# rookiepig/CrossScalePatchMatch

Hardware: AMD Instinct MI355X
Metric: Mpix/s disparity (GRD, use_cs=true) (higher is better)
Workload: dtype f64; 1 GPU; C3: 1242x375 max_dis=128 GRD scale_num=5 reg_lambda=0.3 wnd=35 iters=3 (BASELINE.json configs[2] when C3); cc_name=GRD, schedule=raster, sweep_cells=as cost_source, raster_sweep=persistent, rb_rounds=1, sweep_workgroups_per_cu=2, sweep_workgroup_waves=levels - 1 (coarsest level folded, CSPM_OPT_SWEEP_FOLD), early_exit=True, pairs_per_gpu=22, distinct_pairs_per_gpu=22, pairs_in_flight_per_gpu=2, use_pp=False, parallelism=1 rank(s), one per GPU, 2 independent pair stream(s) each, dispatch=every rank generates its own pairs (no collective in the timed region)

## Files before the change

crossscalepatchmatch_amd/capi.py:

```python
import ctypes as C
import os
import subprocess

import numpy as np

_HERE = os.path.dirname(os.path.abspath(__file__))
_SO = os.environ.get("CSPM_LIB") or os.path.join(_HERE, "libcspm_hip.so")

SCHED_RASTER, SCHED_REDBLACK = 0, 1
RNG_PER_PIXEL, RNG_ROW_SHARED = 0, 1
K_GRD, K_INIT, K_SPATIAL, K_VIEW, K_REFINE, K_MISC, K_POST = range(7)
K_NAMES = ["grd", "init", "spatial", "view", "refine", "misc", "post"]
MAX_LEVELS = 8
OPT_GRD_VOLUMES = 1
OPT_RASTER_LAUNCHES = 2
OPT_SWEEP_TIMEOUT_MS = 3
OPT_SWEEP_FALLBACKS = 4
OPT_SWEEP_PAIRS = 5
OPT_SWEEP_PAIRS_ACTIVE = 6
OPT_TABLE_VOLUMES = 7
OPT_TABLE_VOLUMES_ACTIVE = 8
OPT_SWEEP_PACKED = 10
OPT_SWEEP_PACKED_ACTIVE = 11
OPT_SWEEP_PACKED_BAD = 12
OPT_SWEEP_FLOW = 13
OPT_SWEEP_WG = 14
OPT_VOLUME_FALLBACKS = 9
OPT_VOLUME_RETRY_PAIRS = 15
OPT_VIEW_SORT = 17
OPT_SWEEP_FOLD = 18
OPT_FAULT_VOLUME_ALLOC = 16
CA_BOX, CA_GF, CA_BF = 0, 1, 2

SYMBOLS = [
    "cspm_device_count", "cspm_create", "cspm_destroy", "cspm_last_error", "cspm_set_stream", "cspm_get_stream", "cspm_synchronize",
    "cspm_set_images", "cspm_set_images_device", "cspm_build_cost_grd", "cspm_build_cost_cen", "cspm_build_cost_img", "cspm_cen_build_cv_host", "cspm_set_option", "cspm_get_option", "cspm_begin_cost", "cspm_upload_cost_slab",
    "cspm_finish_cost", "cspm_get_levels", "cspm_get_level_dims", "cspm_get_level_image", "cspm_get_cost_slab",
    "cspm_get_max_cost", "cspm_get_scale_weights", "cspm_grd_build_cv_host", "cspm_plane_cost_batch",
    "cspm_pm_default_params", "cspm_patchmatch", "cspm_pm_init", "cspm_pm_spatial", "cspm_pm_view", "cspm_pm_refine",
    "cspm_get_planes", "cspm_set_planes", "cspm_get_disparity_u8", "cspm_get_disparity_f64",
    "cspm_disparity_u8_device", "cspm_postprocess", "cspm_postprocess_device", "cspm_enable_timing", "cspm_reset_timing", "cspm_get_timing",
    "cspm_taps_per_view_pass", "cspm_row_engine_taps_per_view_pass", "cspm_fpm_begin", "cspm_fpm_candidates", "cspm_fpm_commit",
    "cspm_aggregate_cv_host", "cspm_local_stereo", "cspm_rescore_planes", "cspm_patchmatch_warm", "cspm_upsample_planes",
]


class CspmError(RuntimeError):
    pass


class PmParams(C.Structure):
    _fields_ = [("seed", C.c_uint64), ("schedule", C.c_int), ("rb_rounds", C.c_int), ("rb_neighbours", C.c_int),
                ("rng_mode", C.c_int), ("early_exit", C.c_int)]


def library_path():
    return _SO


def build_library(force=False):
    src_dir = os.path.join(_HERE, "csrc")
    srcs = [os.path.join(src_dir, f) for f in os.listdir(src_dir)] + [os.path.join(_HERE, "..", "include", "cspm.h")]
    if force or not os.path.exists(_SO) or os.path.getmtime(_SO) < max(os.path.getmtime(s) for s in srcs):
        subprocess.check_call(["make", "-C", src_dir, "-B"], stdout=subprocess.DEVNULL)
    return _SO


_lib = None


def load_library():
    global _lib
    if _lib is not None:
        return _lib
    if not os.path.exists(_SO):
        raise CspmError(f"{_SO} is missing: build it with `python -c 'import __graft_entry__ as g; g.build()'` "
                        "(hipcc --offload-arch=gfx950). There is no CPU fallback.")
    L = C.CDLL(_SO)
    vp, dp, ip, u8p = C.c_void_p, C.POINTER(C.c_double), C.POINTER(C.c_int), C.POINTER(C.c_uint8)
    llp = C.POINTER(C.c_longlong)
    pp = C.POINTER(PmParams)
    sig = {
        "cspm_device_count": (C.c_int, []),
        "cspm_create": (C.c_int, [C.POINTER(vp), C.c_int]),
        "cspm_destroy": (None, [vp]),
        "cspm_last_error": (C.c_char_p, [vp]),
        "cspm_set_stream": (C.c_int, [vp, vp]),
        "cspm_get_stream": (C.c_int, [vp, C.POINTER(vp)]),
        "cspm_synchronize": (C.c_int, [vp]),
        "cspm_set_images": (C.c_int, [vp, u8p, u8p, C.c_int, C.c_int, C.c_size_t]),
        "cspm_set_images_device": (C.c_int, [vp, vp, vp, C.c_int, C.c_int, C.c_size_t]),
        "cspm_build_cost_grd": (C.c_int, [vp, C.c_int, C.c_int, C.c_int, C.c_double]),
        "cspm_set_option": (C.c_int, [vp, C.c_int, C.c_longlong]),
        "cspm_get_option": (C.c_int, [vp, C.c_int, llp]),
        "cspm_build_cost_cen": (C.c_int, [vp, C.c_int, C.c_int, C.c_int, C.c_double]),
        "cspm_build_cost_img": (C.c_int, [vp, C.c_int, C.c_int, C.c_int, C.c_double]),
        "cspm_cen_build_cv_host": (C.c_int, [C.c_int, dp, dp, C.c_int, C.c_int, C.c_int, C.c_int, dp]),
        "cspm_begin_cost": (C.c_int, [vp, C.c_int, C.c_int, C.c_int, C.c_double]),
        "cspm_upload_cost_slab": (C.c_int, [vp, C.c_int, C.c_int, C.c_int, dp, C.c_size_t]),
        "cspm_finish_cost": (C.c_int, [vp]),
        "cspm_get_levels": (C.c_int, [vp]),
        "cspm_get_level_dims": (C.c_int, [vp, C.c_int, ip, ip, ip]),
        "cspm_get_level_image": (C.c_int, [vp, C.c_int, C.c_int, u8p]),
        "cspm_get_cost_slab": (C.c_int, [vp, C.c_int, C.c_int, C.c_int, dp]),
        "cspm_get_max_cost": (C.c_int, [vp, C.c_int, C.c_int, dp]),
        "cspm_get_scale_weights": (C.c_int, [vp, dp]),
        "cspm_grd_build_cv_host": (C.c_int, [C.c_int, dp, dp, C.c_int, C.c_int, C.c_int, C.c_int, dp]),
        "cspm_plane_cost_batch": (C.c_int, [vp, C.c_int, C.c_int, ip, dp, dp]),
        "cspm_pm_default_params": (C.c_int, [pp]),
        "cspm_patchmatch": (C.c_int, [vp, C.c_int, pp]),
        "cspm_pm_init": (C.c_int, [vp, pp]),
        "cspm_pm_spatial": (C.c_int, [vp, C.c_int, pp]),
        "cspm_pm_view": (C.c_int, [vp, C.c_int, pp]),
        "cspm_pm_refine": (C.c_int, [vp, C.c_int, pp]),
        "cspm_get_planes": (C.c_int, [vp, C.c_int, dp, dp]),
        "cspm_set_planes": (C.c_int, [vp, C.c_int, dp, dp]),
        "cspm_get_disparity_u8": (C.c_int, [vp, C.c_int, C.c_int, u8p, C.c_size_t]),
        "cspm_get_disparity_f64": (C.c_int, [vp, C.c_int, dp]),
        "cspm_disparity_u8_device": (C.c_int, [vp, C.c_int, C.c_int, vp]),
        "cspm_postprocess": (C.c_int, [vp, C.c_int, u8p, u8p, C.c_size_t]),
        "cspm_postprocess_device": (C.c_int, [vp, C.c_int, vp, vp]),
        "cspm_enable_timing": (C.c_int, [vp, C.c_int]),
        "cspm_reset_timing": (C.c_int, [vp]),
        "cspm_get_timing": (C.c_int, [vp, C.c_int, llp, dp, llp]),
        "cspm_fpm_begin": (C.c_int, [vp, C.c_int, C.c_int, C.c_int]),
        "cspm_fpm_candidates": (C.c_int, [vp, C.c_int, C.c_int, C.c_int, pp, ip, ip, ip, dp]),
        "cspm_fpm_commit": (C.c_int, [vp, dp]),
        "cspm_taps_per_view_pass": (C.c_longlong, [vp]),
        "cspm_row_engine_taps_per_view_pass": (C.c_longlong, [vp]),
        "cspm_aggregate_cv_host": (C.c_int, [C.c_int, C.c_int, dp, C.c_int, C.c_int, C.c_int, dp]),
        "cspm_local_stereo": (C.c_int, [vp, C.c_int]),
        "cspm_rescore_planes": (C.c_int, [vp]),
        "cspm_patchmatch_warm": (C.c_int, [vp, C.c_int, pp]),
        "cspm_upsample_planes": (C.c_int, [vp, vp]),
    }
    assert sorted(sig) == sorted(SYMBOLS)
    for name, (res, args) in sig.items():
        f = getattr(L, name)
        f.restype, f.argtypes = res, args
    _lib = L
    return L


def _dp(a):
    return a.ctypes.data_as(C.POINTER(C.c_double))


def _u8(a):
    return a.ctypes.data_as(C.POINTER(C.c_uint8))


class StereoContext:

    def __init__(self, device=0):
        self.L = load_library()
        self.p = C.c_void_p()
        rc = self.L.cspm_create(C.byref(self.p), device)
        if rc != 0:
            raise CspmError(f"cspm_create failed ({rc}): {self.L.cspm_last_error(None).decode()}")
        self.w = self.h = 0

    def close(self):
        if getattr(self, "p", None) and self.p:
            self.L.cspm_destroy(self.p)
            self.p = C.c_void_p()

    def __del__(self):
        try:
            self.close()
        except Exception:
            pass

    def _chk(self, rc):
        if rc != 0:
            raise CspmError(f"cspm error {rc}: {self.L.cspm_last_error(self.p).decode()}")

    def set_images(self, l_bgr, r_bgr):
        l = np.ascontiguousarray(l_bgr, dtype=np.uint8)
        r = np.ascontiguousarray(r_bgr, dtype=np.uint8)
        assert l.ndim == 3 and l.shape[2] == 3 and l.shape == r.shape
        self.h, self.w = l.shape[:2]
        self._chk(self.L.cspm_set_images(self.p, _u8(l), _u8(r), self.w, self.h, self.w * 3))

    def set_images_device(self, d_l_ptr, d_r_ptr, w, h, stride=None):
# ... 226 lines not shown
```

crossscalepatchmatch_amd/csrc/cspm_api.hip:

```cpp
#include <hip/hip_runtime.h>

#include <cfloat>
#include <cmath>
#include <cstdio>
#include <cstring>
#include <string>
#include <vector>

#include "cspm_kernels.h"
#include "cspm_ca.h"

using namespace cspm;

namespace {

thread_local std::string g_create_error;

struct TimingRec {
  int kclass;
  hipEvent_t a, b;
  long long evals;
};

}

struct DevGuard {
  int prev = -1;
  bool ok = true;
  explicit DevGuard(int dev) {
    if (hipGetDevice(&prev) != hipSuccess) prev = -1;
    if (prev != dev) ok = hipSetDevice(dev) == hipSuccess;
    else prev = -1;
  }
  ~DevGuard() {
    if (prev >= 0) (void)hipSetDevice(prev);
  }
};

struct CostKey {
  int W = 0, H = 0, max_dis = 0, wnd = 0, scale_num = -1, with_vol = 0, kind = -1, with_pairs = 0, with_cvol = 0, with_px8 = 0;
  bool operator==(const CostKey &o) const {
    return W == o.W && H == o.H && max_dis == o.max_dis && wnd == o.wnd && scale_num == o.scale_num && with_vol == o.with_vol && kind == o.kind &&
           with_pairs == o.with_pairs && with_cvol == o.with_cvol && with_px8 == o.with_px8;
  }
};
enum { kKindForeign = 0, kKindGrd = 1, kKindCen = 2, kKindImg = 3 };

struct cspm_ctx {
  int device = 0, ncu = 256;
  int sweep_wg_per_cu = 0;
  int sweep_bands = 1;
  int sweep_bands_built = 0;
  int refine_chunk = 64;
  hipStream_t own_stream = nullptr, stream = nullptr;
  std::string err;
  int W = 0, H = 0;
  uint32_t *img0[2] = {nullptr, nullptr};
  uint8_t *stage = nullptr;
  size_t stage_bytes = 0;
  bool cost_alloc = false, cost_ready = false;
  Cost cost{};
  int max_dis = 0, wnd = 0;
  double scale_wgt[CSPM_MAX_LEVELS] = {0};
  double host_max_cost[2 * CSPM_MAX_LEVELS] = {0};
  std::vector<void *> cost_allocs;
  CostKey cost_key;
  bool max_cost_fetched = false;
  int *d_early_ok = nullptr;
  uint8_t *cen_gray[2][CSPM_MAX_LEVELS] = {{nullptr}};
  double *d_lut = nullptr, *d_lut_a = nullptr, *d_maxcost = nullptr;
  bool is_grd = false;
  bool is_cen = false;
  bool is_img = false;
  const uint32_t *cen_code[2][CSPM_MAX_LEVELS] = {{nullptr}};
  long long opt_grd_volumes = 0;
  long long opt_sweep_pairs = 0;
  long long sweep_pairs_limit = 4LL << 30;
  bool sweep_pairs = false;
  long long opt_table_volumes = 1;
  long long table_volumes_limit = 48LL << 30;
  long long opt_sweep_packed = 0;
  bool sweep_packed = false;
  unsigned int *d_px8_bad = nullptr;
  double volumes_mem_fraction = 0.5;
  long long optional_volume_fallbacks = 0;
  bool optional_missing = false;
  long long optional_reuses = 0;
  long long volume_retry_pairs = 16;
  int fault_volume_alloc = 0;
  unsigned long long *d_maxkeys = nullptr;
  int row_claim = -1;
  unsigned int *d_rowq = nullptr;
  bool field_alloc = false;
  bool field_consistent = false;
  double *field_mem = nullptr;
  Field f[2]{};
  ViewCand vc{nullptr, nullptr, nullptr, nullptr};
  long long opt_sweep_fold = 0;
  long long opt_view_sort = 1;
  uint8_t *d_dis[2] = {nullptr, nullptr};
  uint8_t *d_valid[2] = {nullptr, nullptr};
  unsigned int *d_todo = nullptr;
  unsigned int *d_sweep_ctrl = nullptr, *d_sweep_start = nullptr;
  unsigned long long *d_sweep_gran = nullptr;
  unsigned int *d_sweep_ready = nullptr, *d_sweep_qctl = nullptr;
  unsigned long long *d_sweep_queue = nullptr;
  long long opt_sweep_flow = 0;
  unsigned int sweep_epoch = 0;
  long long opt_raster_launches = 0;
  long long sweep_timeout_ms = 3000;
  bool sweep_pending = false;
  int pm_runs_unchecked = 0;
  bool phases_unchecked = false;
  int last_iters = 0;
  cspm_pm_params last_params{};
  bool last_warm = false;
  double *warm_snap = nullptr;
  long long sweep_fallbacks = 0;
  struct OutReq { int post, view, dis_scale; void *o0, *o1; };
  std::vector<OutReq> out_reqs;
  void remember_output(const OutReq &q) {
    for (auto it = out_reqs.begin(); it != out_reqs.end(); ++it)
      if (it->post == q.post && it->o0 == q.o0 && it->o1 == q.o1 && (q.post || it->view == q.view)) { out_reqs.erase(it); break; }
    out_reqs.push_back(q);
  }
  FpmCand fpm{nullptr, nullptr, nullptr, nullptr};
  long long fpm_cap = 0;
  int fpm_phase = -1, fpm_iter = 0, fpm_step = 0, fpm_inc = 1;
  long long fpm_count = 0;
  cspm_pm_params fpm_params{};
  std::vector<void *> ca_allocs;
  long long ca_key[4] = {0, 0, 0, 0};
  double *ca_gn = nullptr, *ca_t = nullptr, *ca_s = nullptr, *ca_raw = nullptr, *ca_out = nullptr, *ca_best = nullptr;
  int *ca_bestd = nullptr;
  double *ca_vol[CSPM_MAX_LEVELS] = {nullptr};
  unsigned long long *ca_keys = nullptr;
  CaGuideT ca_gt{nullptr, nullptr, nullptr, nullptr};
  int ca_nb = 0;
  bool timing = false;
  std::vector<TimingRec> recs;
  std::vector<hipEvent_t> pool;
  double acc_ms[CSPM_K_COUNT] = {0};
  long long acc_launch[CSPM_K_COUNT] = {0}, acc_evals[CSPM_K_COUNT] = {0};
};

namespace {

int fail(cspm_ctx *c, int code, const std::string &msg) {
  if (c) c->err = msg;
  else g_create_error = msg;
  return code;
}

#define HIPCHK(ctx, expr)                                                                            \
  do {                                                                                               \
    hipError_t e_ = (expr);                                                                          \
    if (e_ != hipSuccess)                                                                            \
      return fail(ctx, CSPM_ERR_HIP, std::string(#expr) + ": " + hipGetErrorString(e_));             \
  } while (0)

template <class T>
int dalloc(cspm_ctx *c, T **p, size_t n, std::vector<void *> *track) {
  void *q = nullptr;
  hipError_t e = hipMalloc(&q, n * sizeof(T) ? n * sizeof(T) : sizeof(T));
  if (e != hipSuccess) return fail(c, CSPM_ERR_HIP, std::string("hipMalloc: ") + hipGetErrorString(e));
  *p = (T *)q;
  if (track) track->push_back(q);
  return CSPM_OK;
}

hipEvent_t get_event(cspm_ctx *c) {
  if (!c->pool.empty()) {
    hipEvent_t e = c->pool.back();
    c->pool.pop_back();
    return e;
  }
  hipEvent_t e;
  (void)hipEventCreate(&e);
  return e;
}

struct Timed {
  cspm_ctx *c;
  TimingRec r{};
  bool on;
  Timed(cspm_ctx *ctx, int kclass, long long evals) : c(ctx), on(ctx->timing) {
    if (!on) return;
    r.kclass = kclass;
    r.evals = evals;
    r.a = get_event(c);
    r.b = get_event(c);
    (void)hipEventRecord(r.a, c->stream);
  }
  ~Timed() {
    if (!on) return;
    (void)hipEventRecord(r.b, c->stream);
    c->recs.push_back(r);
  }
};

int drain_timing(cspm_ctx *c) {
  if (c->recs.empty()) return CSPM_OK;
  HIPCHK(c, hipStreamSynchronize(c->stream));
  for (auto &r : c->recs) {
    float ms = 0.f;
    (void)hipEventElapsedTime(&ms, r.a, r.b);
    c->acc_ms[r.kclass] += ms;
    c->acc_launch[r.kclass] += 1;
    c->acc_evals[r.kclass] += r.evals;
    c->pool.push_back(r.a);
    c->pool.push_back(r.b);
  }
  c->recs.clear();
  return CSPM_OK;
}

inline bool row_claimed_w(const cspm_ctx *c, int W, int views) {
  const long long items = row_items(W, c->H, views);
  if (items >= (1LL << 31)) return false;
  if (c->row_claim >= 0) return c->row_claim != 0;
  return items >= 2LL * c->ncu * 12;
}
inline unsigned row_grid_w(const cspm_ctx *c, int W, int views) {
  const bool claimed = row_claimed_w(c, W, views);
  long long per_xcd = (row_items_per_xcd(W, c->H, views, claimed) + kRowWaves - 1) / kRowWaves;
  if (claimed) per_xcd += per_xcd / 4 + 1;
  return (unsigned)(per_xcd * 8);
}
inline bool row_claimed(const cspm_ctx *c, int views) { return row_claimed_w(c, c->W, views); }
inline unsigned row_grid(const cspm_ctx *c, int views) { return row_grid_w(c, c->W, views); }
inline int row_cap(const cspm_ctx *c) { return strip_capacity(c->max_dis, c->cost.half); }
inline int row_ocap(const cspm_ctx *c) { return own_capacity(c->cost.half); }
inline size_t row_shmem(const cspm_ctx *c) { return sizeof(LutMem) + (size_t)kRowWaves * wave_lds_bytes(row_cap(c), row_ocap(c)); }

inline RowQueue next_row_queue(cspm_ctx *c, int views) {
  if (!row_claimed(c, views)) return RowQueue{nullptr};
  (void)hipMemsetAsync(c->d_rowq, 0, 8 * sizeof(unsigned int), c->stream);
  return RowQueue{c->d_rowq};
}

inline unsigned eval_grid(long long items) {
  long long nb = (items + (kEvalBlock / kWave) - 1) / (kEvalBlock / kWave);
  nb = (nb + 7) / 8 * 8;
  if (nb < 8) nb = 8;
  return (unsigned)nb;
}
inline unsigned ew_grid(long long n, int block = 256) { return (unsigned)((n + block - 1) / block); }
inline unsigned stride_grid(long long n, int block = 256) { return (unsigned)std::min<long long>((n + block - 1) / block, 256 * 16); }

void free_cost(cspm_ctx *c) {
  for (void *p : c->cost_allocs) (void)hipFree(p);
  c->cost_allocs.clear();
  c->cost_alloc = c->cost_ready = false;
  c->cost_key = CostKey{};
  memset(&c->cost, 0, sizeof c->cost);
}
void free_field(cspm_ctx *c) {
  if (c->field_mem) (void)hipFree(c->field_mem);
  if (c->warm_snap) (void)hipFree(c->warm_snap);
  c->warm_snap = nullptr;
  if (c->vc.cost) (void)hipFree(c->vc.cost);
  if (c->vc.c) (void)hipFree(c->vc.c);
  if (c->vc.cx) (void)hipFree(c->vc.cx);
  if (c->vc.perm) (void)hipFree(c->vc.perm);
  for (int v = 0; v < 2; ++v) {
    if (c->d_dis[v]) (void)hipFree(c->d_dis[v]);
    if (c->d_valid[v]) (void)hipFree(c->d_valid[v]);
    c->d_dis[v] = nullptr;
    c->d_valid[v] = nullptr;
  }
  if (c->d_todo) (void)hipFree(c->d_todo);
  c->d_todo = nullptr;
  if (c->d_rowq) (void)hipFree(c->d_rowq);
  c->d_rowq = nullptr;
  if (c->fpm.xy) (void)hipFree(c->fpm.xy);
  if (c->fpm.view) (void)hipFree(c->fpm.view);
  if (c->fpm.plane) (void)hipFree(c->fpm.plane);
  if (c->fpm.cost) (void)hipFree(c->fpm.cost);
  c->fpm = FpmCand{nullptr, nullptr, nullptr, nullptr};
  c->fpm_cap = 0;
  c->fpm_phase = -1;
  if (c->d_sweep_ctrl) (void)hipFree(c->d_sweep_ctrl);
  if (c->d_sweep_gran) (void)hipFree(c->d_sweep_gran);
  if (c->d_sweep_start) (void)hipFree(c->d_sweep_start);
  if (c->d_sweep_ready) (void)hipFree(c->d_sweep_ready);
  if (c->d_sweep_qctl) (void)hipFree(c->d_sweep_qctl);
  if (c->d_sweep_queue) (void)hipFree(c->d_sweep_queue);
  c->d_sweep_ready = c->d_sweep_qctl = nullptr;
  c->d_sweep_queue = nullptr;
  c->d_sweep_ctrl = c->d_sweep_start = nullptr;
  c->d_sweep_gran = nullptr;
  c->field_mem = nullptr;
  c->vc = ViewCand{nullptr, nullptr, nullptr, nullptr};
  c->field_alloc = false;
}
void free_images(cspm_ctx *c) {
  for (int v = 0; v < 2; ++v) {
    if (c->img0[v]) (void)hipFree(c->img0[v]);
    c->img0[v] = nullptr;
  }
  if (c->stage) (void)hipFree(c->stage);
  c->stage = nullptr;
  c->stage_bytes = 0;
  c->W = c->H = 0;
}

void small_inverse_row0(int S, const double A[CSPM_MAX_LEVELS][CSPM_MAX_LEVELS], double *w);
int scale_weights(int S, double lambda, double *w) {
  if (S < 1 || S > CSPM_MAX_LEVELS) return -1;
  double A[CSPM_MAX_LEVELS][CSPM_MAX_LEVELS] = {{0}}, B[CSPM_MAX_LEVELS][CSPM_MAX_LEVELS] = {{0}};
  for (int s = 0; s < S; ++s) {
    B[s][s] = 1.0;
    if (S == 1) { A[0][0] = 1 + lambda; break; }
    if (s == 0) { A[s][s] = 1 + lambda; A[s][s + 1] = -lambda; }
    else if (s == S - 1) { A[s][s] = 1 + lambda; A[s][s - 1] = -lambda; }
    else { A[s][s] = 1 + 2 * lambda; A[s][s - 1] = -lambda; A[s][s + 1] = -lambda; }
  }
  if (S <= 3) {
    small_inverse_row0(S, A, w);
    return 0;
  }
  const double eps = DBL_EPSILON * 100;
  for (int i = 0; i < S; ++i) {
    int k = i;
    for (int j = i + 1; j < S; ++j)
      if (std::fabs(A[j][i]) > std::fabs(A[k][i])) k = j;
    if (std::fabs(A[k][i]) < eps) return -2;
    if (k != i) {
      for (int j = i; j < S; ++j) std::swap(A[i][j], A[k][j]);
      for (int j = 0; j < S; ++j) std::swap(B[i][j], B[k][j]);
    }
    const double d = -1 / A[i][i];
    for (int j = i + 1; j < S; ++j) {
      const double alpha = A[j][i] * d;
      for (int q = i + 1; q < S; ++q) A[j][q] += alpha * A[i][q];
      for (int q = 0; q < S; ++q) B[j][q] += alpha * B[i][q];
    }
    A[i][i] = -d;
  }
  for (int i = S - 1; i >= 0; --i)
    for (int j = 0; j < S; ++j) {
      double s = B[i][j];
      for (int q = i + 1; q < S; ++q) s -= A[i][q] * B[q][j];
      B[i][j] = s * A[i][i];
    }
  for (int s = 0; s < S; ++s) w[s] = B[0][s];
  return 0;
}

void small_inverse_row0(int S, const double A[CSPM_MAX_LEVELS][CSPM_MAX_LEVELS], double *w) {
  if (S == 1) {
    w[0] = 1. / A[0][0];
  } else if (S == 2) {
    double d = A[0][0] * A[1][1] - A[0][1] * A[1][0];
    d = 1. / d;
    w[0] = A[1][1] * d;
    w[1] = -A[0][1] * d;
  } else {
    double d = A[0][0] * (A[1][1] * A[2][2] - A[1][2] * A[2][1]) - A[0][1] * (A[1][0] * A[2][2] - A[1][2] * A[2][0]) +
               A[0][2] * (A[1][0] * A[2][1] - A[1][1] * A[2][0]);
    d = 1. / d;
    w[0] = (A[1][1] * A[2][2] - A[1][2] * A[2][1]) * d;
    w[1] = (A[0][2] * A[2][1] - A[0][1] * A[2][2]) * d;
    w[2] = (A[0][1] * A[1][2] - A[0][2] * A[1][1]) * d;
  }
}

void launch_pyramid(cspm_ctx *c) {
  Cost &cd = c->cost;
  for (int s = 0; s < cd.levels; ++s) {
    Level &L = cd.lv[s];
    for (int v = 0; v < 2; ++v) {
      Timed t(c, CSPM_K_MISC, 0);
      uint32_t *img = const_cast<uint32_t *>(L.pix[v]);
      if (s == 0) {
        hipLaunchKernelGGL(k_pad_u32, dim3(ew_grid((long long)L.Wp * L.H)), dim3(256), 0, c->stream, c->img0[v], L.W, L.H, L.Wp, L.pad, img);
      } else {
        const Level &P = cd.lv[s - 1];
        hipLaunchKernelGGL(k_pyrdown, dim3(ew_grid((long long)L.Wp * L.H)), dim3(256), 0, c->stream, P.pix[v], P.W, P.H, P.Wp, P.pad,
                           img, L.W, L.H, L.Wp, L.pad);
      }
    }
  }
}

int alloc_cost(cspm_ctx *c, int max_dis, int wnd_size, int scale_num, double reg_lambda, bool with_vol, int kind, bool want_pairs = false,
// ... 240 lines not shown
  if ((rc = dalloc(c, &c->d_sweep_ctrl, 2 + kSweepMaxBands, nullptr))) return rc;
  HIPCHK(c, hipMemsetAsync(c->d_sweep_ctrl, 0, (2 + kSweepMaxBands) * sizeof(unsigned int), c->stream));
  if ((rc = dalloc(c, &c->d_sweep_gran, 2 * n * kGranPerPixel, nullptr))) return rc;
  HIPCHK(c, hipMemsetAsync(c->d_sweep_gran, 0, sizeof(unsigned long long) * 2 * n * kGranPerPixel, c->stream));
  c->sweep_epoch = 0;
  {
    const int nd = c->W + c->H - 1;
    const int nb = std::max(1, std::min(std::min(c->sweep_bands, kSweepMaxBands), c->H));
    std::vector<unsigned int> start((size_t)nb * (nd + 1), 0);
    for (int b = 0; b < nb; ++b) {
      const int y0 = (int)((long long)b * c->H / nb), y1 = (int)((long long)(b + 1) * c->H / nb);
      unsigned int *st = start.data() + (size_t)b * (nd + 1);
      for (int k = 0; k < nd; ++k) {
        const int cnt = std::min(y1 - 1, k) - std::max(y0, k - (c->W - 1)) + 1;
        st[k + 1] = st[k] + 2u * (unsigned)std::max(cnt, 0);
      }
    }
    if ((rc = dalloc(c, &c->d_sweep_start, start.size(), nullptr))) return rc;
    HIPCHK(c, hipMemcpy(c->d_sweep_start, start.data(), start.size() * sizeof(unsigned int), hipMemcpyHostToDevice));
    c->sweep_bands_built = nb;
  }
  c->field_alloc = true;
  return CSPM_OK;
}

int ensure_flow(cspm_ctx *c) {
  if (c->d_sweep_ready) return CSPM_OK;
  const size_t n = (size_t)c->W * c->H;
  int rc;
  if ((rc = dalloc(c, &c->d_sweep_ready, 2 * n, nullptr))) return rc;
  if ((rc = dalloc(c, &c->d_sweep_queue, 2 * n + 65536, nullptr))) return rc;
  HIPCHK(c, hipMemsetAsync(c->d_sweep_queue, 0, sizeof(unsigned long long) * (2 * n + 65536), c->stream));
  if ((rc = dalloc(c, &c->d_sweep_qctl, 4, nullptr))) return rc;
  return CSPM_OK;
}

Pm make_pm(cspm_ctx *c, const cspm_pm_params *p) {
  Pm pm{};
  pm.W = c->W; pm.H = c->H; pm.max_dis = c->max_dis;
  pm.seed = p->seed;
  pm.rng_row_shared = p->rng_mode == CSPM_RNG_ROW_SHARED;
  pm.trust_cost = c->field_consistent ? 1 : 0;
  pm.use_thresh = p->early_exit ? 1 : 0;
  pm.f[0] = c->f[0];
  pm.f[1] = c->f[1];
  return pm;
}

int run_patchmatch(cspm_ctx *c, int iter_num, const cspm_pm_params *p);
int run_warm_retry(cspm_ctx *c, int iter_num, const cspm_pm_params *p);
int enqueue_disp_u8(cspm_ctx *c, int view, int dis_scale, void *d_out);
int enqueue_postprocess_device(cspm_ctx *c, int dis_scale, void *d_l_out, void *d_r_out);

int check_sweep(cspm_ctx *c) {
  if (!c->sweep_pending) return CSPM_OK;
  unsigned int ctrl[2] = {0, 0}, px8_bad = 0;
  HIPCHK(c, hipMemcpyAsync(ctrl, c->d_sweep_ctrl, sizeof ctrl, hipMemcpyDeviceToHost, c->stream));
  const bool packed = c->sweep_packed && c->cost_alloc && c->d_px8_bad;
  if (packed) HIPCHK(c, hipMemcpyAsync(&px8_bad, c->d_px8_bad, sizeof px8_bad, hipMemcpyDeviceToHost, c->stream));
  HIPCHK(c, hipStreamSynchronize(c->stream));
  c->sweep_pending = false;
  if (packed && px8_bad) {
    c->pm_runs_unchecked = 0;
    c->phases_unchecked = false;
    c->out_reqs.clear();
    return fail(c, CSPM_ERR_HIP, "CSPM_OPT_SWEEP_PACKED: " + std::to_string(px8_bad) + " gradients could not be packed exactly; the raster sweep's planes are not valid");
  }
  const int runs = c->pm_runs_unchecked;
  const bool phases = c->phases_unchecked;
  c->pm_runs_unchecked = 0;
  c->phases_unchecked = false;
  const std::vector<cspm_ctx::OutReq> reqs = c->out_reqs;
  c->out_reqs.clear();
  if (ctrl[1]) {
    (void)hipMemsetAsync(c->d_sweep_ctrl, 0, 2 * sizeof(unsigned int), c->stream);
    if (runs == 1 && !phases && c->cost_ready) {
      const long long keep = c->opt_raster_launches;
      c->opt_raster_launches = 1;
      int rc = c->last_warm ? run_warm_retry(c, c->last_iters, &c->last_params) : run_patchmatch(c, c->last_iters, &c->last_params);
      c->opt_raster_launches = keep;
      c->pm_runs_unchecked = 0;
      for (const auto &q : reqs) {
        if (rc != CSPM_OK) break;
        rc = q.post ? enqueue_postprocess_device(c, q.dis_scale, q.o0, q.o1) : enqueue_disp_u8(c, q.view, q.dis_scale, q.o0);
      }
      if (rc == CSPM_OK) {
        HIPCHK(c, hipStreamSynchronize(c->stream));
        ++c->sweep_fallbacks;
        return CSPM_OK;
      }
      return rc;
    }
    return fail(c, CSPM_ERR_HIP, "raster sweep timed out waiting for a predecessor pixel (inter-workgroup hand-off)");
  }
  return CSPM_OK;
}

const cspm_pm_params kDefaultParams = {12345ULL, CSPM_SCHED_RASTER, 1, 4, CSPM_RNG_PER_PIXEL, 1};

int check_pm(cspm_ctx *c, const cspm_pm_params **p) {
  if (!c) return CSPM_ERR_ARG;
  if (!c->cost_ready) return fail(c, CSPM_ERR_STATE, "no plane cost built (cspm_build_cost_grd / cspm_finish_cost)");
  if (!*p) *p = &kDefaultParams;
  if ((*p)->schedule != CSPM_SCHED_RASTER && (*p)->schedule != CSPM_SCHED_REDBLACK) return fail(c, CSPM_ERR_ARG, "bad schedule");
  if ((*p)->rb_neighbours != 2 && (*p)->rb_neighbours != 4) return fail(c, CSPM_ERR_ARG, "rb_neighbours must be 2 or 4");
  if ((*p)->rb_rounds < 1) return fail(c, CSPM_ERR_ARG, "rb_rounds must be >= 1");
  return ensure_field(c);
}

template <class K>
inline void allow_lds(K kern, size_t shmem) {
  if (shmem > 64 * 1024) (void)hipFuncSetAttribute(reinterpret_cast<const void *>(kern), hipFuncAttributeMaxDynamicSharedMemorySize, 160 * 1024);
}
#define LAUNCH_ONE(K, grid, block, shmem, ...)                                \
  do {                                                                       \
    allow_lds(K, shmem);                                                     \
    hipLaunchKernelGGL(K, grid, block, shmem, c->stream, __VA_ARGS__);       \
  } while (0)
#define LAUNCH_CS(kern, grid, block, shmem, ...)                                                                  \
  do {                                                                                                            \
    const int src_ = c->cost.fused;                                                                               \
    if (c->cost.cs) {                                                                                             \
      if (src_ == kSrcGrd) LAUNCH_ONE((kern<true, kSrcGrd>), grid, block, shmem, __VA_ARGS__);                    \
      else if (src_ == kSrcCen) LAUNCH_ONE((kern<true, kSrcCen>), grid, block, shmem, __VA_ARGS__);               \
      else if (src_ == kSrcImg) LAUNCH_ONE((kern<true, kSrcImg>), grid, block, shmem, __VA_ARGS__);               \
      else LAUNCH_ONE((kern<true, kSrcVolume>), grid, block, shmem, __VA_ARGS__);                                 \
    } else {                                                                                                      \
      if (src_ == kSrcGrd) LAUNCH_ONE((kern<false, kSrcGrd>), grid, block, shmem, __VA_ARGS__);                   \
      else if (src_ == kSrcCen) LAUNCH_ONE((kern<false, kSrcCen>), grid, block, shmem, __VA_ARGS__);              \
      else if (src_ == kSrcImg) LAUNCH_ONE((kern<false, kSrcImg>), grid, block, shmem, __VA_ARGS__);              \
      else LAUNCH_ONE((kern<false, kSrcVolume>), grid, block, shmem, __VA_ARGS__);                                \
    }                                                                                                             \
  } while (0)

#define LAUNCH_SWEEP(kern, grid, block, shmem, ...)                                                              \
  do {                                                                                                            \
    if (c->sweep_pairs && c->cost.fused == kSrcGrd) {                                                             \
      if (c->cost.cs) LAUNCH_ONE((kern<true, kSrcVol2>), grid, block, shmem, __VA_ARGS__);                        \
      else LAUNCH_ONE((kern<false, kSrcVol2>), grid, block, shmem, __VA_ARGS__);                                  \
    } else if (c->sweep_packed && c->cost.fused == kSrcGrd) {                                                     \
      if (c->cost.cs) LAUNCH_ONE((kern<true, kSrcGrd8>), grid, block, shmem, __VA_ARGS__);                        \
      else LAUNCH_ONE((kern<false, kSrcGrd8>), grid, block, shmem, __VA_ARGS__);                                  \
    } else {                                                                                                      \
      LAUNCH_CS(kern, grid, block, shmem, __VA_ARGS__);                                                           \
    }                                                                                                             \
  } while (0)

int do_init(cspm_ctx *c, const cspm_pm_params *p) {
  const long long items = 2LL * c->W * c->H;
  Pm pm = make_pm(c, p);
  {
    Timed t(c, CSPM_K_INIT, items);
    const RowQueue rq = next_row_queue(c, 2);
    LAUNCH_CS(k_init, dim3(row_grid(c, 2)), dim3(kRowBlock), row_shmem(c), c->cost, pm, rq, row_cap(c), row_ocap(c));
  }
  HIPCHK(c, hipGetLastError());
  c->field_consistent = true;
  return CSPM_OK;
}

inline bool sweep_folded(const cspm_ctx *c) { return c->cost.cs && kSweepWpl == 1 && c->opt_sweep_fold != 0 && c->cost.levels >= 4; }
inline unsigned sweep_waves(const cspm_ctx *c) {
  if (sweep_folded(c)) return (unsigned)(c->cost.levels - 1);
  return c->cost.cs ? (unsigned)(c->cost.levels * kSweepWpl) : (unsigned)((c->cost.n + kChainRows - 1) / kChainRows);
}
inline size_t sweep_lds(const cspm_ctx *c) { return sweep_shared_bytes((int)sweep_waves(c) + (sweep_folded(c) ? 1 : 0)); }

int do_spatial(cspm_ctx *c, int iter, const cspm_pm_params *p) {
  Pm pm = make_pm(c, p);
  const int inc = (iter % 2 == 0) ? 1 : -1;
  if (p->schedule == CSPM_SCHED_REDBLACK) {
    const long long items = 2LL * ((c->W + 1) / 2) * c->H;
    for (int r = 0; r < p->rb_rounds; ++r)
      for (int hs = 0; hs < 2; ++hs) {
        Timed t(c, CSPM_K_SPATIAL, items * p->rb_neighbours);
        LAUNCH_CS(k_spatial_rb, dim3(eval_grid(items)), dim3(kEvalBlock), 0, c->cost, pm, (hs + iter) & 1, inc, p->rb_neighbours);
      }
  } else if (!c->opt_raster_launches) {
    Sweep sw{};
    sw.ctrl = c->d_sweep_ctrl;
    sw.gran[0] = c->d_sweep_gran;
    sw.gran[1] = c->d_sweep_gran + (size_t)c->W * c->H * kGranPerPixel;
    sw.start = c->d_sweep_start;
    sw.nbands = c->sweep_bands_built;
    sw.epoch = ++c->sweep_epoch;
    sw.total = 2u * (unsigned)c->W * (unsigned)c->H;
    sw.timeout_ticks = c->sweep_timeout_ms * 100000LL;
    sw.trace = nullptr;
#ifdef CSPM_SWEEP_TRACE
    {
      static long long *d_trace = nullptr;
      if (!d_trace) { (void)hipMalloc((void **)&d_trace, sizeof(long long) * kTraceSlots * (size_t)sw.total); (void)hipMemset(d_trace, 0, sizeof(long long) * kTraceSlots * (size_t)sw.total); }
      sw.trace = d_trace;
      if (const char *path = getenv("CSPM_SWEEP_TRACE_FILE")) {
        static int sweep_no = 0;
        const int dump_after = getenv("CSPM_SWEEP_TRACE_SWEEP") ? atoi(getenv("CSPM_SWEEP_TRACE_SWEEP")) : 1;
        if (sweep_no++ == dump_after) {
          std::vector<long long> h((size_t)kTraceSlots * sw.total);
          (void)hipStreamSynchronize(c->stream);
          (void)hipMemcpy(h.data(), d_trace, h.size() * sizeof(long long), hipMemcpyDeviceToHost);
          if (FILE *fp = fopen(path, "wb")) { fwrite(h.data(), sizeof(long long), h.size(), fp); fclose(fp); }
        }
      }
    }
#endif
    HIPCHK(c, hipMemsetAsync(c->d_sweep_ctrl + 2, 0, kSweepMaxBands * sizeof(unsigned int), c->stream));
    const bool flow = c->opt_sweep_flow != 0 && (long long)c->W * c->H < (1LL << 30);
    if (flow) {
      int frc = ensure_flow(c);
      if (frc) return frc;
      sw.ready[0] = c->d_sweep_ready;
      sw.ready[1] = c->d_sweep_ready + (size_t)c->W * c->H;
      sw.queue = c->d_sweep_queue;
      sw.qctl = c->d_sweep_qctl;
      HIPCHK(c, hipMemsetAsync(c->d_sweep_ready, 0, sizeof(unsigned int) * 2 * (size_t)c->W * c->H, c->stream));
      HIPCHK(c, hipMemsetAsync(c->d_sweep_qctl, 0, 4 * sizeof(unsigned int), c->stream));
    }
    int ncu = c->ncu;
    const bool wide = 2LL * std::min(c->W, c->H) >= 4LL * c->ncu && !sweep_folded(c);
    const int wg_per_cu = c->sweep_wg_per_cu > 0 ? c->sweep_wg_per_cu : (wide ? 3 : 2);
    unsigned grid = (unsigned)std::max<long long>(sw.nbands, std::min<long long>((long long)sw.total, (long long)ncu * wg_per_cu));
    grid = (grid + (unsigned)sw.nbands - 1) / (unsigned)sw.nbands * (unsigned)sw.nbands;
    const unsigned waves = sweep_waves(c);
    {
      Timed t(c, CSPM_K_SPATIAL, (long long)sw.total * 2);
      if (flow) LAUNCH_SWEEP(k_spatial_flow, dim3(grid), dim3(waves * kWave), sweep_lds(c), c->cost, pm, sw, inc);
      else LAUNCH_SWEEP(k_spatial_sweep, dim3(grid), dim3(waves * kWave), sweep_lds(c), c->cost, pm, sw, inc);
    }
    c->sweep_pending = true;
  } else {
    for (int k = 1; k <= c->W + c->H - 2; ++k) {
      const int ys_lo = std::max(0, k - (c->W - 1)), ys_hi = std::min(c->H - 1, k);
      const long long items = 2LL * (ys_hi - ys_lo + 1);
      Timed t(c, CSPM_K_SPATIAL, items * 2);
      LAUNCH_SWEEP(k_spatial_diag, dim3((unsigned)items), dim3(sweep_waves(c) * kWave), sweep_lds(c), c->cost, pm, k, inc);
    }
  }
  HIPCHK(c, hipGetLastError());
  return CSPM_OK;
}

int do_view(cspm_ctx *c, int iter, const cspm_pm_params *p) {
  Pm pm = make_pm(c, p);
  const long long items = (long long)c->W * c->H;
  const size_t shmem = (size_t)c->W * (sizeof(unsigned long long) + sizeof(unsigned int));
  if (shmem > 160 * 1024) return fail(c, CSPM_ERR_ARG, "image too wide for the view-propagation row resolver");
  ViewCand vc = c->vc;
  const size_t sort_shmem = (size_t)(c->W + 1 + 256) * sizeof(unsigned int);
  if (!c->opt_view_sort || sort_shmem > 160 * 1024) vc.perm = nullptr;
  for (int v = 0; v < 2; ++v) {
    if (vc.perm) {
      Timed t(c, CSPM_K_MISC, 0);
      LAUNCH_ONE(k_view_sort, dim3(c->H), dim3(256), sort_shmem, pm, v, vc);
    }
    {
      Timed t(c, CSPM_K_VIEW, items);
      const RowQueue rq = next_row_queue(c, 1);
      LAUNCH_CS(k_view_eval, dim3(row_grid(c, 1)), dim3(kRowBlock), row_shmem(c), c->cost, pm, rq, v, vc, row_cap(c), row_ocap(c));
    }
    {
      Timed t(c, CSPM_K_MISC, 0);
      LAUNCH_ONE(k_view_resolve, dim3(c->H), dim3(256), shmem, pm, v, iter % 2 == 0 ? 0 : 1, c->vc);
    }
  }
  HIPCHK(c, hipGetLastError());
  return CSPM_OK;
}

int do_refine(cspm_ctx *c, int iter, const cspm_pm_params *p) {
  Pm pm = make_pm(c, p);
  const long long items = 2LL * c->W * c->H;
  const double z_iter = c->max_dis / 2.0, n_iter = 1.0;
  int steps = 0;
  for (double z = z_iter; z >= 0.1; z /= 2.0) ++steps;
  double z = z_iter, nn = n_iter;
  for (int first = 0; first < steps; first += c->refine_chunk) {
    const int cnt = std::min(c->refine_chunk, steps - first);
    Timed t(c, CSPM_K_REFINE, items * cnt);
    const RowQueue rq = next_row_queue(c, 2);
    LAUNCH_CS(k_refine, dim3(row_grid(c, 2)), dim3(kRowBlock), row_shmem(c), c->cost, pm, rq, iter, first, cnt, z, nn, row_cap(c), row_ocap(c));
    for (int k = 0; k < cnt; ++k) { z /= 2.0; nn /= 2.0; }
  }
  HIPCHK(c, hipGetLastError());
  return CSPM_OK;
}

int run_iterations(cspm_ctx *c, int iter_num, const cspm_pm_params *p) {
  int rc;
  for (int i = 0; i < iter_num; ++i) {
    if ((rc = do_spatial(c, i, p))) return rc;
    if ((rc = do_view(c, i, p))) return rc;
    if ((rc = do_refine(c, i, p))) return rc;
  }
  return CSPM_OK;
}

int run_patchmatch(cspm_ctx *c, int iter_num, const cspm_pm_params *p) {
  int rc;
  if ((rc = do_init(c, p))) return rc;
  return run_iterations(c, iter_num, p);
}

int do_rescore(cspm_ctx *c) {
  const long long items = 2LL * c->W * c->H;
  Pm pm = make_pm(c, &kDefaultParams);
  {
    Timed t(c, CSPM_K_INIT, items);
    const RowQueue rq = next_row_queue(c, 2);
    LAUNCH_CS(k_rescore, dim3(row_grid(c, 2)), dim3(kRowBlock), row_shmem(c), c->cost, pm, rq, row_cap(c), row_ocap(c));
  }
  HIPCHK(c, hipGetLastError());
  c->field_consistent = true;
  return CSPM_OK;
}

int warm_snapshot(cspm_ctx *c, bool save) {
  const size_t bytes = sizeof(double) * 14 * (size_t)c->W * c->H;
  if (!c->warm_snap) {
    int rc = dalloc(c, &c->warm_snap, 14 * (size_t)c->W * c->H, nullptr);
    if (rc) return rc;
  }
  HIPCHK(c, hipMemcpyAsync(save ? c->warm_snap : c->field_mem, save ? c->field_mem : c->warm_snap, bytes, hipMemcpyDeviceToDevice, c->stream));
  return CSPM_OK;
}

int run_warm_retry(cspm_ctx *c, int iter_num, const cspm_pm_params *p) {
  int rc;
  if ((rc = warm_snapshot(c, false))) return rc;
  c->field_consistent = true;
  return run_iterations(c, iter_num, p);
}

int postprocess_enqueue(cspm_ctx *c, int dis_scale) {
  Pm pm{};
  pm.W = c->W; pm.H = c->H; pm.f[0] = c->f[0]; pm.f[1] = c->f[1];
  const long long n = (long long)c->W * c->H;
  const Level &L0 = c->cost.lv[0];
  Timed t(c, CSPM_K_POST, 0);
  for (int v = 0; v < 2; ++v)
    hipLaunchKernelGGL(k_plane_to_disp_u8, dim3(ew_grid(n)), dim3(256), 0, c->stream, pm, v, dis_scale, c->d_dis[v], (size_t)c->W);
  unsigned int *todo_cnt = c->d_todo + 2 * (size_t)n;
  HIPCHK(c, hipMemsetAsync(todo_cnt, 0, 2 * sizeof(unsigned int), c->stream));
  hipLaunchKernelGGL(k_lr_check, dim3(ew_grid(2 * n)), dim3(256), 0, c->stream, c->d_dis[0], c->d_dis[1], c->W, c->H, dis_scale, c->d_valid[0],
                     c->d_valid[1]);
  if (fill_rows_shmem(c->W) > 160 * 1024) return fail(c, CSPM_ERR_ARG, "image too wide for the row scan of FillInvalid");
  LAUNCH_ONE(k_fill_rows, dim3(2u * (unsigned)c->H), dim3(kFillBlock), fill_rows_shmem(c->W), pm, dis_scale, c->d_valid[0], c->d_valid[1], c->d_dis[0],
             c->d_dis[1], c->d_todo, todo_cnt);
  hipLaunchKernelGGL(k_weighted_median, dim3((unsigned)c->ncu * 8u), dim3(kMedianBlock), 0, c->stream, L0.pix[0], L0.pix[1], L0.Wp, L0.pad, c->W,
                     c->H, c->d_valid[0], c->d_valid[1], c->d_lut, c->d_dis[0], c->d_dis[1], c->d_todo, todo_cnt, 35 / 2);
  HIPCHK(c, hipGetLastError());
  return CSPM_OK;
}

int enqueue_disp_u8(cspm_ctx *c, int view, int dis_scale, void *d_out) {
  Pm pm{};
  pm.W = c->W; pm.H = c->H; pm.f[0] = c->f[0]; pm.f[1] = c->f[1];
  {
    Timed t(c, CSPM_K_MISC, 0);
    hipLaunchKernelGGL(k_plane_to_disp_u8, dim3(ew_grid((long long)c->W * c->H)), dim3(256), 0, c->stream, pm, view, dis_scale,
                       (uint8_t *)d_out, (size_t)c->W);
  }
  HIPCHK(c, hipGetLastError());
  return CSPM_OK;
}
int enqueue_postprocess_device(cspm_ctx *c, int dis_scale, void *d_l_out, void *d_r_out) {
  int rc = postprocess_enqueue(c, dis_scale);
  if (rc) return rc;
  void *outs[2] = {d_l_out, d_r_out};
  for (int v = 0; v < 2; ++v)
    HIPCHK(c, hipMemcpyAsync(outs[v], c->d_dis[v], (size_t)c->W * c->H, hipMemcpyDeviceToDevice, c->stream));
  return CSPM_OK;
}

constexpr int kCaRadiusBox = 3, kCaRadiusGf = 9;
inline int ca_min_size(int method) { return method == CSPM_CA_BOX ? 2 * kCaRadiusBox + 1 : (method == CSPM_CA_GF ? 2 * kCaRadiusGf + 1 : 17); }
inline const char *ca_name(int method) { return method == CSPM_CA_BOX ? "BOX" : (method == CSPM_CA_GF ? "GF" : "BF"); }

struct CaWork {
  double *gn, *t, *s;
  CaGuideT gt;
  int nb;
};
inline size_t ca_t_slabs(int nb) { return (size_t)std::max(9, 4 * nb); }

void ca_prepare_guide(cspm_ctx *c, int method, const CaWork &w, int W, int H) {
  if (method != CSPM_CA_GF) return;
  const size_t px = (size_t)W * H;
  Timed t(c, CSPM_K_MISC, 0);
  hipLaunchKernelGGL((k_ca_ywalk<9, CaInGuide>), dim3((W + kCaBlock - 1) / kCaBlock, 1), dim3(kCaBlock), 0, c->stream, CaInGuide{w.gn, px}, W, H,
                     kCaRadiusGf, w.t);
  hipLaunchKernelGGL((k_ca_xwalk<9, CaEpGuide>), dim3((H + kCaBlock - 1) / kCaBlock, 1), dim3(kCaBlock), 0, c->stream, (const double *)w.t, W, H,
                     kCaRadiusGf, CaEpGuide{w.gt, w.gn, W, H, kCaRadiusGf, (double)0.0001f});
}

void ca_filter(cspm_ctx *c, int method, const CaWork &w, int W, int H, const double *src, int n, double *dst) {
  const size_t px = (size_t)W * H;
  const dim3 gy((W + kCaBlock - 1) / kCaBlock, n), gx((H + kCaBlock - 1) / kCaBlock, n);
  Timed t(c, CSPM_K_MISC, 0);
  if (method == CSPM_CA_BOX) {
    hipLaunchKernelGGL((k_ca_ywalk<1, CaInPlain>), gy, dim3(kCaBlock), 0, c->stream, CaInPlain{src, 1, px}, W, H, kCaRadiusBox, w.t);
    hipLaunchKernelGGL((k_ca_xwalk<1, CaEpStore>), gx, dim3(kCaBlock), 0, c->stream, (const double *)w.t, W, H, kCaRadiusBox, CaEpStore{dst, W, px});
  } else if (method == CSPM_CA_GF) {
    hipLaunchKernelGGL((k_ca_ywalk<4, CaInGfP>), gy, dim3(kCaBlock), 0, c->stream, CaInGfP{src, w.gn, px}, W, H, kCaRadiusGf, w.t);
    hipLaunchKernelGGL((k_ca_xwalk<4, CaEpGfA>), gx, dim3(kCaBlock), 0, c->stream, (const double *)w.t, W, H, kCaRadiusGf, CaEpGfA{w.gt, w.s, W, H, kCaRadiusGf});
    hipLaunchKernelGGL((k_ca_ywalk<4, CaInPlain>), gy, dim3(kCaBlock), 0, c->stream, CaInPlain{w.s, 4, px}, W, H, kCaRadiusGf, w.t);
    hipLaunchKernelGGL((k_ca_xwalk<4, CaEpGfQ>), gx, dim3(kCaBlock), 0, c->stream, (const double *)w.t, W, H, kCaRadiusGf, CaEpGfQ{w.gt, dst, W, H, kCaRadiusGf});
  } else {
    hipLaunchKernelGGL(k_ca_bf, dim3(ew_grid((long long)px)), dim3(256), 0, c->stream, (const double *)w.gn, src, W, H, n, dst);
  }
}

int ca_alloc_work(cspm_ctx *c, size_t px, int nb, CaWork *w, std::vector<void *> *track) {
  int rc;
  double *gt;
  w->nb = nb;
  if ((rc = dalloc(c, &w->gn, 3 * px, track)) || (rc = dalloc(c, &gt, 16 * px, track)) || (rc = dalloc(c, &w->t, ca_t_slabs(nb) * px, track)) ||
      (rc = dalloc(c, &w->s, (size_t)4 * nb * px, track)))
    return rc;
  w->gt = CaGuideT{gt, gt + 3 * px, gt + 6 * px, gt + 15 * px};
  return CSPM_OK;
}

inline int ca_batch(size_t px) { return (int)std::max<long long>(2, std::min<long long>(128, (6LL << 30) / (80LL * (long long)px))); }

const double *ca_raw_cells(cspm_ctx *c, int v, int s, int d0, int n, double *scratch) {
  const Level &L = c->cost.lv[s];
  const size_t px = (size_t)L.W * L.H;
  if (L.vol[v]) return L.vol[v] + (size_t)d0 * px;
  Timed t(c, CSPM_K_MISC, 0);
  if (c->is_cen)
    hipLaunchKernelGGL(k_cen_volume, dim3(stride_grid((long long)px * n)), dim3(256), 0, c->stream, c->cen_code[0][s], c->cen_code[1][s], L.W, L.H, d0,
                       n, v, scratch, (unsigned long long *)nullptr);
  else
    hipLaunchKernelGGL((k_grd_volume<SrcU32, true>), dim3(stride_grid((long long)px * n)), dim3(256), 0, c->stream, SrcU32{L.pix[0], L.Wp, L.pad},
                       SrcU32{L.pix[1], L.Wp, L.pad}, L.grd[0], L.grd[1], L.Wp, L.pad, L.W, L.H, d0, n, v, scratch, (unsigned long long *)nullptr);
  return scratch;
}

int ca_ensure(cspm_ctx *c) {
  const Cost &cd = c->cost;
  const long long key[4] = {c->W, c->H, c->max_dis, cd.levels};
  if (c->ca_nb && std::equal(key, key + 4, c->ca_key)) return CSPM_OK;
  HIPCHK(c, hipStreamSynchronize(c->stream));
  for (void *p : c->ca_allocs) (void)hipFree(p);
  c->ca_allocs.clear();
  c->ca_nb = 0;
  const size_t px = (size_t)c->W * c->H;
  const int nb = ca_batch(px);
  CaWork w;
  int rc;
  if ((rc = ca_alloc_work(c, px, nb, &w, &c->ca_allocs))) return rc;
  if ((rc = dalloc(c, &c->ca_raw, (size_t)nb * px, &c->ca_allocs)) || (rc = dalloc(c, &c->ca_out, (size_t)nb * px, &c->ca_allocs)) ||
      (rc = dalloc(c, &c->ca_best, px, &c->ca_allocs)) || (rc = dalloc(c, &c->ca_bestd, px, &c->ca_allocs)) ||
      (rc = dalloc(c, &c->ca_keys, CSPM_MAX_LEVELS, &c->ca_allocs)))
    return rc;
  for (int s = 1; s < cd.levels; ++s)
    if ((rc = dalloc(c, &c->ca_vol[s], (size_t)(cd.lv[s].D + 1) * cd.lv[s].W * cd.lv[s].H, &c->ca_allocs))) return rc;
  c->ca_gn = w.gn;
  c->ca_t = w.t;
  c->ca_s = w.s;
  c->ca_gt = w.gt;
  c->ca_nb = nb;
  std::copy(key, key + 4, c->ca_key);
  return CSPM_OK;
}

int ca_local_view(cspm_ctx *c, int method, int v) {
  const Cost &cd = c->cost;
  const CaWork w{c->ca_gn, c->ca_t, c->ca_s, c->ca_gt, c->ca_nb};
  const int nb = c->ca_nb;
  HIPCHK(c, hipMemsetAsync(c->ca_keys, 0, sizeof(unsigned long long) * CSPM_MAX_LEVELS, c->stream));
  CaLevels lv{};
  lv.levels = cd.levels;
  lv.cs = cd.cs;
  lv.max_key = c->ca_keys;
  for (int s = cd.levels - 1; s >= 0; --s) {
    const Level &L = cd.lv[s];
    lv.W[s] = L.W; lv.H[s] = L.H; lv.D[s] = L.D; lv.wgt[s] = c->scale_wgt[s];
    const size_t px = (size_t)L.W * L.H;
    {
      Timed t(c, CSPM_K_MISC, 0);
      hipLaunchKernelGGL(k_ca_guide_u32, dim3(ew_grid((long long)px)), dim3(256), 0, c->stream, L.pix[v], L.W, L.H, L.Wp, L.pad, w.gn);
    }
    if (L.D >= 1) ca_prepare_guide(c, method, w, L.W, L.H);
    if (s > 0) {
      double *A = c->ca_vol[s];
      lv.vol[s] = A;
      const double *raw0 = ca_raw_cells(c, v, s, 0, 1, A);
      if (raw0 != A) HIPCHK(c, hipMemcpyAsync(A, raw0, sizeof(double) * px, hipMemcpyDeviceToDevice, c->stream));
      for (int d0 = 1; d0 <= L.D; d0 += nb) {
        const int n = std::min(nb, L.D + 1 - d0);
        ca_filter(c, method, w, L.W, L.H, ca_raw_cells(c, v, s, d0, n, c->ca_raw), n, A + (size_t)d0 * px);
      }
      Timed t(c, CSPM_K_MISC, 0);
      hipLaunchKernelGGL(k_ca_max, dim3(1024), dim3(256), 0, c->stream, (const double *)A, (long long)(L.D + 1) * (long long)px, c->ca_keys + s);
    } else {
      HIPCHK(c, hipMemsetAsync(c->ca_bestd, 0, sizeof(int) * px, c->stream));
      for (int d0 = 1; d0 <= L.D - 1;) {
        const int n = std::min(nb, L.D + 1 - d0);
        ca_filter(c, method, w, L.W, L.H, ca_raw_cells(c, v, 0, d0, n, c->ca_raw), n, c->ca_out);
        Timed t(c, CSPM_K_MISC, 0);
        hipLaunchKernelGGL(k_ca_wta, dim3(ew_grid((long long)px)), dim3(256), 0, c->stream, lv, (const double *)c->ca_out, d0, n, c->ca_best, c->ca_bestd);
        d0 += n - 1;
      }
      Timed t(c, CSPM_K_MISC, 0);
      hipLaunchKernelGGL(k_ca_planes, dim3(ew_grid((long long)px)), dim3(256), 0, c->stream, c->f[v], (long long)px, (const double *)c->ca_best,
                         (const int *)c->ca_bestd);
    }
  }
  HIPCHK(c, hipGetLastError());
  return CSPM_OK;
}

}

extern "C" {

int cspm_device_count(void) {
  int n = 0;
  if (hipGetDeviceCount(&n) != hipSuccess) return 0;
  return n;
}

int cspm_create(cspm_ctx **out, int device) {
  if (!out) return CSPM_ERR_ARG;
  *out = nullptr;
  int n = 0;
  hipError_t e = hipGetDeviceCount(&n);
  if (e != hipSuccess || n <= 0)
    return fail(nullptr, CSPM_ERR_HIP, std::string("no HIP device: ") + (e != hipSuccess ? hipGetErrorString(e) : "count=0"));
  if (device < 0 || device >= n) return fail(nullptr, CSPM_ERR_ARG, "device index out of range");
  DevGuard guard_(device);
  if (!guard_.ok) return fail(nullptr, CSPM_ERR_HIP, "hipSetDevice failed");
  hipDeviceProp_t prop;
  if ((e = hipGetDeviceProperties(&prop, device)) != hipSuccess) return fail(nullptr, CSPM_ERR_HIP, hipGetErrorString(e));
  if (std::string(prop.gcnArchName).rfind("gfx950", 0) != 0)
    return fail(nullptr, CSPM_ERR_HIP, std::string("libcspm_hip is built for gfx950 only, device is ") + prop.gcnArchName);
  cspm_ctx *c = new cspm_ctx();
  c->device = device;
  c->ncu = prop.multiProcessorCount > 0 ? prop.multiProcessorCount : 256;
  if (const char *e = getenv("CSPM_REFINE_CHUNK")) c->refine_chunk = std::max(1, atoi(e));
  if (const char *e = getenv("CSPM_SWEEP_WG")) c->sweep_wg_per_cu = std::max(1, atoi(e));
  if (const char *e = getenv("CSPM_ROW_CLAIM")) c->row_claim = atoi(e) < 0 ? -1 : (atoi(e) ? 1 : 0);
  if (const char *e = getenv("CSPM_SWEEP_BANDS")) c->sweep_bands = std::max(1, std::min(kSweepMaxBands, atoi(e)));
  if (const char *e = getenv("CSPM_SWEEP_PAIRS")) c->opt_sweep_pairs = atoi(e) ? 1 : 0;
  if (const char *e = getenv("CSPM_TABLE_VOLUMES")) c->opt_table_volumes = atoi(e) ? 1 : 0;
  if (const char *e = getenv("CSPM_TABLE_VOLUMES_MAX_MB")) c->table_volumes_limit = std::max(0LL, atoll(e)) << 20;
  if (const char *e = getenv("CSPM_SWEEP_PACKED")) c->opt_sweep_packed = atoi(e) ? 1 : 0;
  if (const char *e = getenv("CSPM_SWEEP_FLOW")) c->opt_sweep_flow = atoi(e) ? 1 : 0;
  if (const char *e = getenv("CSPM_VIEW_SORT")) c->opt_view_sort = atoi(e) ? 1 : 0;
  if (const char *e = getenv("CSPM_SWEEP_FOLD")) c->opt_sweep_fold = atoi(e) ? 1 : 0;
  if (const char *e = getenv("CSPM_VOLUMES_MEM_FRACTION")) c->volumes_mem_fraction = std::min(1.0, std::max(0.0, atof(e)));
  if (const char *e = getenv("CSPM_SWEEP_PAIRS_MAX_MB")) c->sweep_pairs_limit = std::max(0LL, atoll(e)) << 20;
  if (const char *e = getenv("CSPM_SWEEP_TIMEOUT_MS")) c->sweep_timeout_ms = std::min(3600000LL, std::max(0LL, atoll(e)));
  if ((e = hipStreamCreateWithFlags(&c->own_stream, hipStreamNonBlocking)) != hipSuccess) {
    delete c;
    return fail(nullptr, CSPM_ERR_HIP, hipGetErrorString(e));
  }
  c->stream = c->own_stream;
  *out = c;
  return CSPM_OK;
}

void cspm_destroy(cspm_ctx *c) {
  if (!c) return;
  DevGuard guard_(c->device);
  (void)hipStreamSynchronize(c->stream);
  for (auto &r : c->recs) { (void)hipEventDestroy(r.a); (void)hipEventDestroy(r.b); }
  for (auto e : c->pool) (void)hipEventDestroy(e);
  free_cost(c);
  free_field(c);
  free_images(c);
  for (void *p : c->ca_allocs) (void)hipFree(p);
  if (c->own_stream) (void)hipStreamDestroy(c->own_stream);
  delete c;
}

const char *cspm_last_error(const cspm_ctx *c) { return c ? c->err.c_str() : g_create_error.c_str(); }

int cspm_set_stream(cspm_ctx *c, void *s) {
  if (!c) return CSPM_ERR_ARG;
  DevGuard guard_(c->device);
  if (!guard_.ok) return fail(c, CSPM_ERR_HIP, "hipSetDevice failed");
  HIPCHK(c, hipStreamSynchronize(c->stream));
  c->stream = s ? (hipStream_t)s : c->own_stream;
  return CSPM_OK;
}

int cspm_get_stream(cspm_ctx *c, void **out) {
  if (!c || !out) return CSPM_ERR_ARG;
  *out = (void *)c->stream;
  return CSPM_OK;
}

int cspm_synchronize(cspm_ctx *c) {
  if (!c) return CSPM_ERR_ARG;
  DevGuard guard_(c->device);
  if (!guard_.ok) return fail(c, CSPM_ERR_HIP, "hipSetDevice failed");
  int rc = check_sweep(c);
  if (rc) return rc;
  HIPCHK(c, hipStreamSynchronize(c->stream));
  return CSPM_OK;
}

static int set_images_impl(cspm_ctx *c, const void *l, const void *r, int w, int h, size_t stride, bool on_device) {
  if (!c) return CSPM_ERR_ARG;
  if (!l || !r || w < 1 || h < 1 || stride < (size_t)w * 3) return fail(c, CSPM_ERR_ARG, "bad image arguments");
  DevGuard guard_(c->device);
  if (!guard_.ok) return fail(c, CSPM_ERR_HIP, "hipSetDevice failed");
  if (w != c->W || h != c->H) {
    HIPCHK(c, hipStreamSynchronize(c->stream));
    free_cost(c);
    free_field(c);
    free_images(c);
    int rc;
    for (int v = 0; v < 2; ++v)
      if ((rc = dalloc(c, &c->img0[v], (size_t)w * h, nullptr))) return rc;
    c->W = w; c->H = h;
  } else {
    c->cost_ready = false;
  }
  c->field_consistent = false;
  if (c->pm_runs_unchecked) c->phases_unchecked = true;
  const void *src[2] = {l, r};
  const size_t row = (size_t)w * 3;
  if (!on_device && c->stage_bytes < 2 * row * h) {
    if (c->stage) (void)hipFree(c->stage);
    c->stage = nullptr;
    c->stage_bytes = 0;
    HIPCHK(c, hipMalloc((void **)&c->stage, 2 * row * h));
    c->stage_bytes = 2 * row * h;
  }
  for (int v = 0; v < 2; ++v) {
    const uint8_t *d_src = (const uint8_t *)src[v];
    size_t d_stride = stride;
    if (!on_device) {
      uint8_t *dst = c->stage + (size_t)v * row * h;
      HIPCHK(c, hipMemcpy2DAsync(dst, row, src[v], stride, row, h, hipMemcpyHostToDevice, c->stream));
      d_src = dst;
      d_stride = row;
    }
    Timed t(c, CSPM_K_MISC, 0);
    hipLaunchKernelGGL(k_pack_bgr, dim3(ew_grid((long long)w * h)), dim3(256), 0, c->stream, d_src, d_stride, w, h, w, 0, c->img0[v]);
  }
  HIPCHK(c, hipGetLastError());
  if (!on_device) HIPCHK(c, hipStreamSynchronize(c->stream));
  return CSPM_OK;
}

int cspm_set_images(cspm_ctx *c, const uint8_t *l, const uint8_t *r, int w, int h, size_t stride) {
  return set_images_impl(c, l, r, w, h, stride, false);
}
int cspm_set_images_device(cspm_ctx *c, const void *l, const void *r, int w, int h, size_t stride) {
  return set_images_impl(c, l, r, w, h, stride, true);
}

int cspm_set_option(cspm_ctx *c, int key, long long value) {
  if (!c) return CSPM_ERR_ARG;
  switch (key) {
    case CSPM_OPT_GRD_VOLUMES: c->opt_grd_volumes = value ? 1 : 0; return CSPM_OK;
    case CSPM_OPT_RASTER_LAUNCHES: c->opt_raster_launches = value ? 1 : 0; return CSPM_OK;
    case CSPM_OPT_SWEEP_PAIRS: c->opt_sweep_pairs = value ? 1 : 0; return CSPM_OK;
    case CSPM_OPT_TABLE_VOLUMES: c->opt_table_volumes = value ? 1 : 0; return CSPM_OK;
    case CSPM_OPT_SWEEP_PACKED: c->opt_sweep_packed = value ? 1 : 0; return CSPM_OK;
    case CSPM_OPT_SWEEP_FLOW: c->opt_sweep_flow = value ? 1 : 0; return CSPM_OK;
    case CSPM_OPT_SWEEP_WG: c->sweep_wg_per_cu = value < 0 ? 0 : (value > 16 ? 16 : (int)value); return CSPM_OK;
    case CSPM_OPT_VIEW_SORT: c->opt_view_sort = value ? 1 : 0; return CSPM_OK;
    case CSPM_OPT_SWEEP_FOLD: c->opt_sweep_fold = value ? 1 : 0; return CSPM_OK;
    case CSPM_OPT_FAULT_VOLUME_ALLOC: c->fault_volume_alloc = value < 0 ? 0 : (int)value; return CSPM_OK;
    case CSPM_OPT_VOLUME_RETRY_PAIRS: c->volume_retry_pairs = value < 0 ? 0 : value; return CSPM_OK;
    case CSPM_OPT_SWEEP_TIMEOUT_MS:
      if (value < 0 || value > 3600000) return fail(c, CSPM_ERR_ARG, "sweep timeout out of range");
      c->sweep_timeout_ms = value;
      return CSPM_OK;
    default: return fail(c, CSPM_ERR_ARG, "unknown option");
  }
}

int cspm_get_option(cspm_ctx *c, int key, long long *value) {
  if (!c || !value) return CSPM_ERR_ARG;
  switch (key) {
    case CSPM_OPT_GRD_VOLUMES: *value = c->opt_grd_volumes; return CSPM_OK;
    case CSPM_OPT_RASTER_LAUNCHES: *value = c->opt_raster_launches; return CSPM_OK;
    case CSPM_OPT_SWEEP_TIMEOUT_MS: *value = c->sweep_timeout_ms; return CSPM_OK;
    case CSPM_OPT_SWEEP_FALLBACKS: *value = c->sweep_fallbacks; return CSPM_OK;
    case CSPM_OPT_SWEEP_PAIRS: *value = c->opt_sweep_pairs; return CSPM_OK;
    case CSPM_OPT_TABLE_VOLUMES: *value = c->opt_table_volumes; return CSPM_OK;
    case CSPM_OPT_TABLE_VOLUMES_ACTIVE: *value = (c->cost_alloc && c->cost.lv[0].cvol[0]) ? 1 : 0; return CSPM_OK;
    case CSPM_OPT_SWEEP_PAIRS_ACTIVE: *value = c->sweep_pairs ? 1 : 0; return CSPM_OK;
    case CSPM_OPT_VOLUME_FALLBACKS: *value = c->optional_volume_fallbacks; return CSPM_OK;
    case CSPM_OPT_VOLUME_RETRY_PAIRS: *value = c->volume_retry_pairs; return CSPM_OK;
    case CSPM_OPT_VIEW_SORT: *value = c->opt_view_sort; return CSPM_OK;
    case CSPM_OPT_SWEEP_FOLD: *value = c->opt_sweep_fold; return CSPM_OK;
    case CSPM_OPT_SWEEP_PACKED: *value = c->opt_sweep_packed; return CSPM_OK;
    case CSPM_OPT_SWEEP_FLOW: *value = c->opt_sweep_flow; return CSPM_OK;
    case CSPM_OPT_SWEEP_WG: *value = c->sweep_wg_per_cu; return CSPM_OK;
    case CSPM_OPT_SWEEP_PACKED_ACTIVE: *value = c->sweep_packed ? 1 : 0; return CSPM_OK;
    case CSPM_OPT_SWEEP_PACKED_BAD: {
      if (!c->cost_alloc || !c->d_px8_bad) { *value = 0; return CSPM_OK; }
      DevGuard guard_(c->device);
      unsigned int bad = 0;
      HIPCHK(c, hipMemcpyAsync(&bad, c->d_px8_bad, sizeof bad, hipMemcpyDeviceToHost, c->stream));
      HIPCHK(c, hipStreamSynchronize(c->stream));
      *value = bad;
      return CSPM_OK;
    }
    default: return fail(c, CSPM_ERR_ARG, "unknown option");
  }
}

int cspm_build_cost_grd(cspm_ctx *c, int max_dis, int wnd_size, int scale_num, double reg_lambda) {
  if (!c) return CSPM_ERR_ARG;
  DevGuard guard_(c->device);
  if (!guard_.ok) return fail(c, CSPM_ERR_HIP, "hipSetDevice failed");
  const bool with_vol = c->opt_grd_volumes != 0;
  int rc = alloc_cost(c, max_dis, wnd_size, scale_num, reg_lambda, with_vol, kKindGrd, !with_vol && c->opt_sweep_pairs != 0,
                      !with_vol && c->opt_table_volumes != 0);
  if (rc) return rc;
  Cost &cd = c->cost;
  for (int s = 0; s < cd.levels; ++s) {
    Level &L = cd.lv[s];
    const long long ppx = (long long)L.Wp * L.H;
    for (int v = 0; v < 2; ++v) {
      double *g = const_cast<double *>(L.grd[v]);
      Timed t(c, CSPM_K_GRD, 0);
      hipLaunchKernelGGL(k_gradient<SrcU32>, dim3(ew_grid(ppx)), dim3(256), 0, c->stream, SrcU32{L.pix[v], L.Wp, L.pad}, L.W, L.H,
                         L.Wp, L.pad, g);
      hipLaunchKernelGGL(k_make_aos, dim3(ew_grid(ppx)), dim3(256), 0, c->stream, L.pix[v], (const double *)g, ppx, (PixG *)L.px[v]);
      hipLaunchKernelGGL(k_make_px16, dim3(ew_grid(ppx)), dim3(256), 0, c->stream, L.pix[v], (const double *)g, L.Wp, L.H, v == 1 ? -1 : 1,
                         (uint4 *)L.px16[v]);
      if (L.px8[v])
        hipLaunchKernelGGL(k_make_px8, dim3(ew_grid(ppx)), dim3(256), 0, c->stream, L.pix[v], (const double *)g, ppx, (Pix8 *)L.px8[v], c->d_px8_bad);
    }
    const long long cells = (long long)L.W * L.H * (L.D + 1);
    for (int v = 0; v < 2; ++v) {
      Timed t(c, CSPM_K_GRD, 0);
      hipLaunchKernelGGL((k_grd_volume<SrcU32, true>), dim3(stride_grid(cells)), dim3(256), 0, c->stream, SrcU32{L.pix[0], L.Wp, L.pad},
                         SrcU32{L.pix[1], L.Wp, L.pad}, L.grd[0], L.grd[1], L.Wp, L.pad, L.W, L.H, 0, L.D + 1, v,
                         (double *)L.vol[v], c->d_maxkeys + v * CSPM_MAX_LEVELS + s, (double2 *)L.vol2[v], (double *)L.cvol[v], L.cvW, L.cvpad);
    }
  }
  HIPCHK(c, hipGetLastError());
  cd.fused = with_vol ? kSrcVolume : kSrcGrd;
  c->sweep_pairs = cd.lv[0].vol2[0] != nullptr;
  c->sweep_packed = !with_vol && cd.lv[0].px8[0] != nullptr;
  c->is_grd = true;
  return finish_cost(c, false);
}

int cspm_build_cost_cen(cspm_ctx *c, int max_dis, int wnd_size, int scale_num, double reg_lambda) {
  if (!c) return CSPM_ERR_ARG;
  DevGuard guard_(c->device);
  if (!guard_.ok) return fail(c, CSPM_ERR_HIP, "hipSetDevice failed");
  const bool with_vol = c->opt_grd_volumes != 0;
  int rc = alloc_cost(c, max_dis, wnd_size, scale_num, reg_lambda, with_vol, kKindCen);
  if (rc) return rc;
  Cost &cd = c->cost;
  for (int s = 0; s < cd.levels; ++s) {
    Level &L = cd.lv[s];
    const long long px = (long long)L.W * L.H, ppx = (long long)L.Wp * L.H;
    for (int v = 0; v < 2; ++v) {
      uint8_t *gray = c->cen_gray[v][s];
      uint32_t *code = const_cast<uint32_t *>(c->cen_code[v][s]);
      Timed t(c, CSPM_K_GRD, 0);
      hipLaunchKernelGGL(k_gray8<SrcU32>, dim3(ew_grid(px)), dim3(256), 0, c->stream, SrcU32{L.pix[v], L.Wp, L.pad}, L.W, L.H, gray);
      hipLaunchKernelGGL(k_census, dim3(ew_grid(px)), dim3(256), 0, c->stream, gray, L.W, L.H, code);
      hipLaunchKernelGGL(k_make_aos_cen, dim3(ew_grid(ppx)), dim3(256), 0, c->stream, L.pix[v], code, L.W, L.H, L.Wp, L.pad, (PixC *)L.pc[v]);
      hipLaunchKernelGGL(k_make_aos, dim3(ew_grid(ppx)), dim3(256), 0, c->stream, L.pix[v], (const double *)nullptr, ppx, (PixG *)L.px[v]);
    }
    for (int v = 0; v < 2; ++v) {
      Timed t(c, CSPM_K_GRD, 0);
      hipLaunchKernelGGL(k_cen_volume, dim3(stride_grid(px * (L.D + 1))), dim3(256), 0, c->stream, c->cen_code[0][s], c->cen_code[1][s], L.W, L.H,
                         0, L.D + 1, v, (double *)L.vol[v], c->d_maxkeys + v * CSPM_MAX_LEVELS + s);
    }
  }
  HIPCHK(c, hipGetLastError());
  cd.fused = with_vol ? kSrcVolume : kSrcCen;
  c->is_cen = true;
  return finish_cost(c, false);
}

int cspm_build_cost_img(cspm_ctx *c, int max_dis, int wnd_size, int scale_num, double reg_lambda) {
  if (!c) return CSPM_ERR_ARG;
  DevGuard guard_(c->device);
  if (!guard_.ok) return fail(c, CSPM_ERR_HIP, "hipSetDevice failed");
  int rc = alloc_cost(c, max_dis, wnd_size, scale_num, reg_lambda, false, kKindImg);
  if (rc) return rc;
  Cost &cd = c->cost;
  for (int s = 0; s < cd.levels; ++s) {
    Level &L = cd.lv[s];
    const long long px = (long long)L.W * L.H, ppx = (long long)L.Wp * L.H;
    for (int v = 0; v < 2; ++v) {
      uint8_t *gray = c->cen_gray[v][s];
      Timed t(c, CSPM_K_GRD, 0);
      hipLaunchKernelGGL(k_gray8_u8, dim3(ew_grid(px)), dim3(256), 0, c->stream, L.pix[v], L.W, L.H, L.Wp, L.pad, gray);
      hipLaunchKernelGGL(k_make_aos_img, dim3(ew_grid(ppx)), dim3(256), 0, c->stream, L.pix[v], (const uint8_t *)gray, L.W, L.H, L.Wp, L.pad,
                         (PixG *)L.px[v]);
    }
  }
  HIPCHK(c, hipGetLastError());
  cd.fused = kSrcImg;
  c->is_img = true;
  const double alpha = 0.1, tau_clr = 10.0, tau_grd = 2.0;
  return finish_cost(c, false, alpha * tau_clr + (1 - alpha) * tau_grd);
}

int cspm_cen_build_cv_host(int device, const double *l_rgb, const double *r_rgb, int w, int h, int maxDis, int right_view, double *vol_out) {
  if (!l_rgb || !r_rgb || !vol_out || w < 1 || h < 1 || maxDis < 1) return fail(nullptr, CSPM_ERR_ARG, "bad arguments");
  cspm_ctx *c = nullptr;
  int rc = cspm_create(&c, device);
  if (rc) return rc;
  const size_t px = (size_t)w * h;
  double *d[2] = {nullptr, nullptr}, *vol = nullptr;
  uint8_t *gray[2];
  uint32_t *code[2];
  std::vector<void *> tmp;
  auto done = [&](int code_) {
    if (code_) g_create_error = c->err;
    for (void *p : tmp) (void)hipFree(p);
    cspm_destroy(c);
    return code_;
  };
  const double *src[2] = {l_rgb, r_rgb};
  for (int v = 0; v < 2; ++v) {
    if ((rc = dalloc(c, &d[v], px * 3, &tmp)) || (rc = dalloc(c, &gray[v], px, &tmp)) || (rc = dalloc(c, &code[v], px * 3, &tmp))) return done(rc);
    if (hipMemcpyAsync(d[v], src[v], sizeof(double) * px * 3, hipMemcpyHostToDevice, c->stream) != hipSuccess) return done(fail(c, CSPM_ERR_HIP, "upload failed"));
    hipLaunchKernelGGL(k_gray8<SrcF64>, dim3(ew_grid((long long)px)), dim3(256), 0, c->stream, SrcF64{d[v], w}, w, h, gray[v]);
    hipLaunchKernelGGL(k_census, dim3(ew_grid((long long)px)), dim3(256), 0, c->stream, gray[v], w, h, code[v]);
  }
  if ((rc = dalloc(c, &vol, px * maxDis, &tmp))) return done(rc);
  hipLaunchKernelGGL(k_cen_volume, dim3(stride_grid((long long)px * maxDis)), dim3(256), 0, c->stream, code[0], code[1], w, h, 0, maxDis, right_view,
                     vol, (unsigned long long *)nullptr);
  if (hipMemcpyAsync(vol_out, vol, sizeof(double) * px * maxDis, hipMemcpyDeviceToHost, c->stream) != hipSuccess ||
      hipStreamSynchronize(c->stream) != hipSuccess || hipGetLastError() != hipSuccess)
    return done(fail(c, CSPM_ERR_HIP, "census volume kernel failed"));
  return done(CSPM_OK);
}

int cspm_begin_cost(cspm_ctx *c, int max_dis, int wnd_size, int scale_num, double reg_lambda) {
  if (!c) return CSPM_ERR_ARG;
  DevGuard guard_(c->device);
  if (!guard_.ok) return fail(c, CSPM_ERR_HIP, "hipSetDevice failed");
  int rc = alloc_cost(c, max_dis, wnd_size, scale_num, reg_lambda, true, kKindForeign);
  if (rc) return rc;
  for (int s = 0; s < c->cost.levels; ++s)
// ... 509 lines not shown
    for (int y = 0; y < c->H; ++y) {
      const int cy = y >> s;
      sy += std::min(cy + cd.half, L.H - 1) - std::max(cy - cd.half, 0) + 1;
    }
    total += sy * lanes_per_row * cd.n;
  }
  return total;
}

#ifdef CSPM_COUNT_ALIVE
int cspm_debug_alive(unsigned long long *out16, int reset) {
  unsigned long long z[16] = {0};
  if (hipMemcpyFromSymbol(out16, HIP_SYMBOL(cspm::g_alive), sizeof z) != hipSuccess) return CSPM_ERR_HIP;
  if (reset && hipMemcpyToSymbol(HIP_SYMBOL(cspm::g_alive), z, sizeof z) != hipSuccess) return CSPM_ERR_HIP;
  return CSPM_OK;
}
int cspm_debug_alive_hist(unsigned long long *out120, int reset) {
  static unsigned long long z[120];
  if (hipMemcpyFromSymbol(out120, HIP_SYMBOL(cspm::g_alive_hist), sizeof z) != hipSuccess) return CSPM_ERR_HIP;
  if (reset && hipMemcpyToSymbol(HIP_SYMBOL(cspm::g_alive_hist), z, sizeof z) != hipSuccess) return CSPM_ERR_HIP;
  return CSPM_OK;
}
#endif

int cspm_fpm_begin(cspm_ctx *c, int w, int h, int max_dis) {
  if (!c) return CSPM_ERR_ARG;
  if (w < 1 || h < 1 || max_dis < 1) return fail(c, CSPM_ERR_ARG, "bad w / h / max_dis");
  DevGuard guard_(c->device);
  if (!guard_.ok) return fail(c, CSPM_ERR_HIP, "hipSetDevice failed");
  if (w != c->W || h != c->H) {
    HIPCHK(c, hipStreamSynchronize(c->stream));
    free_cost(c);
    free_field(c);
    free_images(c);
    c->W = w; c->H = h;
  }
  if (c->cost_alloc && c->max_dis != max_dis) {
    HIPCHK(c, hipStreamSynchronize(c->stream));
    free_cost(c);
  }
  c->max_dis = max_dis;
  c->field_consistent = false;
  c->phases_unchecked = true;
  int rc = ensure_field(c);
  if (rc) return rc;
  const long long need = std::max(2LL * w * h, 4LL * std::min(w, h));
  if (c->fpm_cap < need) {
    if ((rc = dalloc(c, &c->fpm.xy, (size_t)need * 2, nullptr)) || (rc = dalloc(c, &c->fpm.view, (size_t)need, nullptr)) ||
        (rc = dalloc(c, &c->fpm.plane, (size_t)need * 6, nullptr)) || (rc = dalloc(c, &c->fpm.cost, (size_t)need, nullptr)))
      return rc;
    c->fpm_cap = need;
  }
  c->fpm_phase = -1;
  return CSPM_OK;
}

int cspm_fpm_candidates(cspm_ctx *c, int phase, int iter, int step, const cspm_pm_params *p, int *n_out, int *xy_out, int *view_out,
                        double *plane_out) {
  if (!c || !n_out || !xy_out || !view_out || !plane_out) return CSPM_ERR_ARG;
  if (!c->fpm_cap) return fail(c, CSPM_ERR_STATE, "cspm_fpm_begin first");
  if (!p) p = &kDefaultParams;
  if (p->schedule != CSPM_SCHED_RASTER) return fail(c, CSPM_ERR_ARG, "a foreign IPlaneCost runs the reference's raster schedule only");
  DevGuard guard_(c->device);
  if (!guard_.ok) return fail(c, CSPM_ERR_HIP, "hipSetDevice failed");
  Pm pm = make_pm(c, p);
  const long long n = (long long)c->W * c->H;
  long long count = 0;
  int inc = 1;
  switch (phase) {
    case CSPM_FPM_INIT:
    case CSPM_FPM_REFINE: {
      if (phase == CSPM_FPM_REFINE && (step < 0 || step > 64)) return fail(c, CSPM_ERR_ARG, "refinement step out of range");
      double z = c->max_dis / 2.0, nn = 1.0;
      for (int k = 0; k < step && k < 64; ++k) { z /= 2.0; nn /= 2.0; }
      if (phase == CSPM_FPM_REFINE && z < 0.1) return fail(c, CSPM_ERR_ARG, "refinement step out of range");
      count = 2 * n;
      hipLaunchKernelGGL(k_fpm_point_cand, dim3(ew_grid(count)), dim3(256), 0, c->stream, pm, c->fpm, phase == CSPM_FPM_REFINE ? 1 : 0, iter, step, z, nn);
      break;
    }
    case CSPM_FPM_VIEW:
      if (step < 0 || step > 1) return fail(c, CSPM_ERR_ARG, "view propagation: step = target view, 0 or 1");
      count = n;
      hipLaunchKernelGGL(k_fpm_view_cand, dim3(ew_grid(count)), dim3(256), 0, c->stream, pm, c->fpm, step);
      break;
    case CSPM_FPM_SPATIAL: {
      if (step < 0 || step > c->W + c->H - 2) return fail(c, CSPM_ERR_ARG, "spatial propagation: step = anti-diagonal, 0 .. w+h-2");
      inc = (iter % 2 == 0) ? 1 : -1;
      const int cnt = std::min(c->H - 1, step) - std::max(0, step - (c->W - 1)) + 1;
      count = 4LL * cnt;
      hipLaunchKernelGGL(k_fpm_diag_cand, dim3(ew_grid(2LL * cnt)), dim3(256), 0, c->stream, pm, c->fpm, step, inc);
      break;
    }
    default: return fail(c, CSPM_ERR_ARG, "unknown phase");
  }
  HIPCHK(c, hipGetLastError());
  HIPCHK(c, hipMemcpyAsync(xy_out, c->fpm.xy, sizeof(int) * 2 * count, hipMemcpyDeviceToHost, c->stream));
  HIPCHK(c, hipMemcpyAsync(view_out, c->fpm.view, sizeof(int) * count, hipMemcpyDeviceToHost, c->stream));
  HIPCHK(c, hipMemcpyAsync(plane_out, c->fpm.plane, sizeof(double) * 6 * count, hipMemcpyDeviceToHost, c->stream));
  HIPCHK(c, hipStreamSynchronize(c->stream));
  c->fpm_phase = phase; c->fpm_iter = iter; c->fpm_step = step; c->fpm_inc = inc; c->fpm_count = count; c->fpm_params = *p;
  *n_out = (int)count;
  return CSPM_OK;
}

int cspm_fpm_commit(cspm_ctx *c, const double *cost) {
  if (!c || !cost) return CSPM_ERR_ARG;
  if (c->fpm_phase < 0) return fail(c, CSPM_ERR_STATE, "no candidate batch pending (cspm_fpm_candidates)");
  DevGuard guard_(c->device);
  if (!guard_.ok) return fail(c, CSPM_ERR_HIP, "hipSetDevice failed");
  Pm pm = make_pm(c, &c->fpm_params);
  const long long count = c->fpm_count;
  HIPCHK(c, hipMemcpyAsync(c->fpm.cost, cost, sizeof(double) * count, hipMemcpyHostToDevice, c->stream));
  switch (c->fpm_phase) {
    case CSPM_FPM_INIT:
    case CSPM_FPM_REFINE:
      hipLaunchKernelGGL(k_fpm_point_commit, dim3(ew_grid(count)), dim3(256), 0, c->stream, pm, c->fpm, c->fpm_phase == CSPM_FPM_REFINE ? 1 : 0);
      break;
    case CSPM_FPM_VIEW: {
      const size_t shmem = (size_t)c->W * (sizeof(unsigned long long) + sizeof(unsigned int));
      if (shmem > 160 * 1024) return fail(c, CSPM_ERR_ARG, "image too wide for the view-propagation row resolver");
      hipLaunchKernelGGL(k_fpm_view_commit, dim3(ew_grid(count)), dim3(256), 0, c->stream, pm, c->fpm, c->vc);
      LAUNCH_ONE(k_view_resolve, dim3(c->H), dim3(256), shmem, pm, c->fpm_step, c->fpm_iter % 2 == 0 ? 0 : 1, c->vc);
      break;
    }
    case CSPM_FPM_SPATIAL:
      hipLaunchKernelGGL(k_fpm_diag_commit, dim3(ew_grid(count / 2)), dim3(256), 0, c->stream, pm, c->fpm, c->fpm_step, c->fpm_inc);
      break;
  }
  HIPCHK(c, hipGetLastError());
  HIPCHK(c, hipStreamSynchronize(c->stream));
  c->fpm_phase = -1;
  return CSPM_OK;
}

#ifdef CSPM_ROW_STATS
int cspm_debug_unionstat(unsigned long long *out64, int reset) {
  static unsigned long long z[64];
  if (hipMemcpyFromSymbol(out64, HIP_SYMBOL(cspm::g_unionstat), sizeof z) != hipSuccess) return CSPM_ERR_HIP;
  if (reset && hipMemcpyToSymbol(HIP_SYMBOL(cspm::g_unionstat), z, sizeof z) != hipSuccess) return CSPM_ERR_HIP;
  return CSPM_OK;
}
int cspm_debug_rowtime(unsigned long long *out64, int reset) {
  static unsigned long long z[64];
  if (hipMemcpyFromSymbol(out64, HIP_SYMBOL(cspm::g_rowtime), sizeof z) != hipSuccess) return CSPM_ERR_HIP;
  if (reset && hipMemcpyToSymbol(HIP_SYMBOL(cspm::g_rowtime), z, sizeof z) != hipSuccess) return CSPM_ERR_HIP;
  return CSPM_OK;
}
int cspm_debug_rangestats(unsigned long long *out1024, int reset) {
  static unsigned long long z[16 * 8 * 8];
  if (hipMemcpyFromSymbol(out1024, HIP_SYMBOL(cspm::g_rangestat), sizeof z) != hipSuccess) return CSPM_ERR_HIP;
  if (reset && hipMemcpyToSymbol(HIP_SYMBOL(cspm::g_rangestat), z, sizeof z) != hipSuccess) return CSPM_ERR_HIP;
  return CSPM_OK;
}
int cspm_debug_rowstats(unsigned long long *out1024, int reset) {
  static unsigned long long z[16 * 8 * 8];
  if (hipMemcpyFromSymbol(out1024, HIP_SYMBOL(cspm::g_rowstat), sizeof z) != hipSuccess) return CSPM_ERR_HIP;
  if (reset && hipMemcpyToSymbol(HIP_SYMBOL(cspm::g_rowstat), z, sizeof z) != hipSuccess) return CSPM_ERR_HIP;
  return CSPM_OK;
}
#endif

}
```

crossscalepatchmatch_amd/csrc/cspm_device.h:

```cpp
#pragma once
#include <hip/hip_runtime.h>
#include <stdint.h>

#include "../../include/cspm.h"

#pragma clang fp contract(off)

namespace cspm {

constexpr double kDoubleEps = 0.00000001;
constexpr double kDoubleMax = 1.7976931348623157e308;
constexpr int kLutSize = 768;
constexpr int kLutZero = 767;
constexpr int kWave = 64;
constexpr int kEvalBlock = 256;
constexpr uint32_t kBorderPix = 0x00030303u;

struct __attribute__((packed, aligned(4))) PixG {
  double g;
  uint32_t pix;
};
static_assert(sizeof(PixG) == 12, "PixG must be 12 bytes");

struct __attribute__((aligned(16))) PixC {
  uint32_t code[3];
  uint32_t pix;
};
static_assert(sizeof(PixC) == 16, "PixC must be 16 bytes");

enum { kSrcVolume = 0, kSrcGrd = 1, kSrcCen = 2,
       kSrcImg = 3 };
enum { kSrcVol2 = 4 };

enum { kSrcGrd8 = 5 };

struct __attribute__((aligned(8))) Pix8 {
  uint32_t lo, hi;
};
static_assert(sizeof(Pix8) == 8, "Pix8 must be 8 bytes");
constexpr double kPix8Scale = 134217728.0;
constexpr double kPix8Bias = 34359738368.0;
__host__ __device__ inline bool pix8_encode(uint32_t pix, double g, Pix8 *out) {
  const double t = g * kPix8Scale + kPix8Bias;
  const bool ok = t >= 0.0 && t < 68719476736.0 && t == (double)(unsigned long long)t && (pix >> 24) == 0u;
  const unsigned long long u = ok ? (unsigned long long)t : 0ull;
  out->lo = (uint32_t)u;
  out->hi = (pix << 8) | (uint32_t)(u >> 32);
  return ok;
}

struct Level {
  int W, H, D;
  int Wp, pad;
  const PixG *px[2];
  const uint4 *px16[2];
  const Pix8 *px8[2];
  const PixC *pc[2];
  const uint32_t *pix[2];
  const double *grd[2];
  const double *vol[2];
  const double *cvol[2];
  int cvW, cvpad;
  const double2 *vol2[2];
  double wgt;
};

struct Cost {
  int cs;
  int fused;
  int levels;
  int half;
  int n;
  int T;
  const int *early_ok;
  const double *lut;
  const double *lut_a;
  const double *max_cost;
  Level lv[CSPM_MAX_LEVELS];
};

struct Field {
  double *nx, *ny, *nz;
  double *a, *b, *c;
  double *cost;
};

struct Pm {
  int W, H, max_dis;
  uint64_t seed;
  int rng_row_shared;
  int use_thresh;
  int trust_cost;
  Field f[2];
};

__device__ __forceinline__ int round2int(double d) {
  d = d + 6755399441055744.0;
  return __double2loint(d);
}
__device__ __forceinline__ int handle_border(int loc, int size) {
  if (loc < 0) return loc + size;
  if (loc >= size) return loc - size;
  return loc;
}

__device__ __forceinline__ void plane_param(double nx, double ny, double nz, double px, double py, double pz,
                                            double &a, double &b, double &c) {
  double denom = fmax(fabs(nz), kDoubleEps);
  if (nz < 0.0) denom = -denom;
  a = -nx / denom;
  b = -ny / denom;
  double s = nx * px;
  s += ny * py;
  s += nz * pz;
  c = s / denom;
}

constexpr uint64_t kGold = 0x9E3779B97F4A7C15ULL;
__host__ __device__ __forceinline__ uint64_t mix64(uint64_t z) {
  z ^= z >> 30; z *= 0xBF58476D1CE4E5B9ULL;
  z ^= z >> 27; z *= 0x94D049BB133111EBULL;
  z ^= z >> 31;
  return z;
}
__host__ __device__ __forceinline__ uint32_t stream_id(int phase, int iter, int step, int view) {
  return (uint32_t)((((phase * 16 + iter) * 32 + step) * 2) + view);
}
struct Rng {
  uint64_t base;
  __device__ __forceinline__ Rng(uint64_t seed, uint32_t stream, uint64_t pix) {
    uint64_t k = mix64(seed + kGold * ((uint64_t)stream + 1));
    base = mix64(k ^ (kGold * (pix + 1)));
  }
  __device__ __forceinline__ double u01(uint32_t draw) const {
    uint64_t r = mix64(base + kGold * ((uint64_t)draw + 1));
    return (double)(r >> 11) * (1.0 / 9007199254740992.0);
  }
  __device__ __forceinline__ double uniform(uint32_t draw, double a, double b) const { return u01(draw) * (b - a) + a; }
};

__device__ __forceinline__ unsigned long long f64_key(double v) {
  unsigned long long b = (unsigned long long)__double_as_longlong(v);
  return (b >> 63) ? ~b : (b | 0x8000000000000000ULL);
}
__host__ __device__ __forceinline__ double key_f64(unsigned long long k) {
  unsigned long long b = (k >> 63) ? (k & 0x7FFFFFFFFFFFFFFFULL) : ~k;
  union { unsigned long long u; double d; } x;
  x.u = b;
  return x.d;
}

}
```

crossscalepatchmatch_amd/csrc/cspm_rows.h:

```cpp
#pragma once
#include "cspm_tap.h"

#pragma clang fp contract(off)

namespace cspm {

#ifndef CSPM_ROW_WAVES
#define CSPM_ROW_WAVES 4
#endif
constexpr int kRowWaves = CSPM_ROW_WAVES;
#ifndef CSPM_ROW_MINW
#define CSPM_ROW_MINW 3
#endif
#ifndef CSPM_VIEW_MINW
#define CSPM_VIEW_MINW CSPM_ROW_MINW
#endif
#ifndef CSPM_INIT_MINW
#define CSPM_INIT_MINW CSPM_ROW_MINW
#endif
#ifndef CSPM_ROW_EXIT
#define CSPM_ROW_EXIT 1
#endif
#ifndef CSPM_CELL_BUMP
#define CSPM_CELL_BUMP 1
#endif
#ifndef CSPM_ROW_BUMP
#define CSPM_ROW_BUMP 1
#endif
#ifndef CSPM_EDGE_ALLV
#define CSPM_EDGE_ALLV 1
#endif
#ifndef CSPM_TABLE_DMA
#define CSPM_TABLE_DMA 1
#endif
#ifndef CSPM_TABLE_CLUSTERS
#define CSPM_TABLE_CLUSTERS 1
#endif
#ifndef CSPM_TABLE_DMA_SINGLE
#define CSPM_TABLE_DMA_SINGLE 1
#endif
#ifndef CSPM_PREFER_WTAB
#define CSPM_PREFER_WTAB 0
#endif
#ifndef CSPM_WTAB_MAXC
#define CSPM_WTAB_MAXC 64
#endif
#ifndef CSPM_CELL_SUB
#define CSPM_CELL_SUB 4
#endif
#ifndef CSPM_OWN_SINGLE
#define CSPM_OWN_SINGLE 1
#endif
#ifndef CSPM_CELL_PITCH_IMM
#define CSPM_CELL_PITCH_IMM 1
#endif
#ifndef CSPM_CELL_PAD
#define CSPM_CELL_PAD 1
#endif
#ifndef CSPM_RANGE_MODE
#define CSPM_RANGE_MODE 1
#endif
#ifndef CSPM_CELL_MODE
#define CSPM_CELL_MODE 1
#endif
constexpr int kRowBlock = kRowWaves * kWave;
#ifdef CSPM_ROW_STATS
__device__ unsigned long long g_rowstat[16 * 8 * 8];
__device__ unsigned long long g_rangestat[16 * 8 * 8];
__device__ unsigned long long g_rowtime[8 * 8];
__device__ unsigned long long g_unionstat[8 * 8];
#define ROWTIME_NOW() __builtin_readcyclecounter()
#define ROWTIME_ADD(slot, v) do { rowtime_acc[(slot) & 3] += (unsigned long long)(v); rowtime_base = (slot) & 4; } while (0)
#define ROWTIME_FLUSH() do { if (lane == 0 && rowtime_acc[3]) for (int k_ = 0; k_ < 4; ++k_) atomicAdd(&g_rowtime[s * 8 + rowtime_base + k_], rowtime_acc[k_]); } while (0)
#else
#define ROWTIME_NOW() 0ull
#define ROWTIME_ADD(slot, v) do { } while (0)
#define ROWTIME_FLUSH() do { } while (0)
#endif

constexpr int kStripRegs = 6;
constexpr int kOwnRegs = 2;
__host__ __device__ inline int strip_capacity(int max_dis, int half) {
  const int want = kWave + 2 * half + max_dis + 2;
  return want <= kStripRegs * kWave ? want : kStripRegs * kWave;
}
__host__ __device__ inline int own_capacity(int half) { return kWave + 2 * half + 2; }
__host__ __device__ inline int strip_set_bytes(int cap, int ocap) { return (cap * 16 + ocap * 12 + 15) / 16 * 16; }
__host__ __device__ inline int wave_lds_bytes(int cap, int ocap) {
  const int dbl = 2 * strip_set_bytes(cap, ocap), single = (cap + ocap) * 16;
  return dbl > single ? dbl : single;
}

__device__ __forceinline__ void dma_b128(const char *sbase, unsigned voff, unsigned lds_dst) {
  unsigned keep;
  asm volatile("s_mov_b32 %0, m0\n\ts_mov_b32 m0, %3\n\ts_nop 0\n\tglobal_load_lds_dwordx4 %1, %2\n\ts_mov_b32 m0, %0"
               : "=&s"(keep) : "v"(voff), "s"(sbase), "s"(lds_dst) : "memory");
}
__device__ __forceinline__ void dma_b32(const char *sbase, unsigned voff, unsigned lds_dst) {
  unsigned keep;
  asm volatile("s_mov_b32 %0, m0\n\ts_mov_b32 m0, %3\n\ts_nop 0\n\tglobal_load_lds_dword %1, %2\n\ts_mov_b32 m0, %0"
               : "=&s"(keep) : "v"(voff), "s"(sbase), "s"(lds_dst) : "memory");
}
__device__ __forceinline__ void dma_wait() { asm volatile("s_waitcnt vmcnt(0) lgkmcnt(0)" ::: "memory"); }
__device__ __forceinline__ const char *uniform_ptr(const char *p) {
  const uintptr_t v = (uintptr_t)p;
  const unsigned lo = __builtin_amdgcn_readfirstlane((unsigned)v), hi = __builtin_amdgcn_readfirstlane((unsigned)(v >> 32));
  return (const char *)(((uintptr_t)hi << 32) | lo);
}

template <int SRC> struct StripReg { typedef u32x3 type; };
template <> struct StripReg<kSrcCen> { typedef uint4 type; };
template <int SRC>
__device__ __forceinline__ typename StripReg<SRC>::type ld_strip(const char *row, int byte_off) {
  if constexpr (SRC == kSrcCen) return *reinterpret_cast<const uint4 *>(row + (size_t)(unsigned)byte_off);
  else return *reinterpret_cast<const u32x3_a4 *>(row + (size_t)(unsigned)byte_off);
}

__device__ __forceinline__ double lds_ld_single(int adr) { return *(volatile __attribute__((address_space(3))) const double *)(uintptr_t)(unsigned)adr; }
template <int SRC, int VIEW>
__device__ __forceinline__ void rd_cells(int adr, uint4 &o0, uint4 &o1) {
  constexpr bool down = VIEW == 0 && SRC != kSrcImg;
  constexpr int a0 = down ? 16 : 0, a1 = down ? 0 : 16;
  if constexpr (SRC == kSrcCen) {
    o0 = lds_ld<uint4>(adr + a0);
    o1 = lds_ld<uint4>(adr + a1);
  } else {
    const uint4 s0 = lds_ld<uint4>(adr + a0);
    const uint2 g1 = lds_ld<uint2>(adr + a1);
    o0 = uint4{s0.x, s0.y, s0.z, 0u};
    o1 = uint4{g1.x, g1.y, s0.w, 0u};
  }
}
template <int SRC> struct StageReg { uint4 v; };
template <int SRC, int VIEW>
__device__ __forceinline__ StageReg<SRC> ld_stage(const char *row, int byte_off) {
  constexpr int E = elem_size<SRC>();
  StageReg<SRC> r;
  if constexpr (SRC == kSrcCen) {
    r.v = *reinterpret_cast<const uint4 *>(row + (size_t)(unsigned)byte_off);
  } else {
    const u32x3 e = *reinterpret_cast<const u32x3_a4 *>(row + (size_t)(unsigned)byte_off);
    const uint32_t nb = *reinterpret_cast<const uint32_t *>(row + (size_t)(unsigned)(byte_off + ((VIEW == 0 && SRC != kSrcImg) ? -E : E) + 8));
    r.v = uint4{e.x, e.y, e.z, nb};
  }
  return r;
}
template <int SRC>
__device__ __forceinline__ uint4 rd_own(int adr_g, int adr_p, int j) {
  if constexpr (SRC == kSrcCen) {
    return lds_ld<uint4>(adr_g + j * 16);
  } else {
    const uint32_t pix = lds_ld<uint32_t>(adr_p + j * 4);
    uint2 g{0u, 0u};
    if constexpr (SRC == kSrcGrd || SRC == kSrcImg) {
#if CSPM_OWN_SINGLE
      const u32x2 v = *(volatile __attribute__((address_space(3))) const u32x2 *)(uintptr_t)(unsigned)(adr_g + j * 8);
      g = uint2{v[0], v[1]};
#else
      g = lds_ld<uint2>(adr_g + j * 8);
#endif
    }
    return uint4{g.x, g.y, pix, 0u};
  }
}
template <int SRC>
__device__ __forceinline__ void wr_own(char *ostrip, int ocap, int idx, const typename StripReg<SRC>::type &e) {
  if constexpr (SRC == kSrcCen) {
    *reinterpret_cast<uint4 *>(ostrip + idx * 16) = e;
  } else {
    if constexpr (SRC == kSrcGrd || SRC == kSrcImg) *reinterpret_cast<uint2 *>(ostrip + idx * 8) = uint2{e.x, e.y};
    *reinterpret_cast<uint32_t *>(ostrip + ocap * 8 + idx * 4) = e.z;
  }
}
template <int K>
__device__ __forceinline__ int mad_const(int f, int base) {
  int r;
  asm("v_mad_i32_i24 %0, %1, %2, %3" : "=v"(r) : "v"(f), "n"(K), "v"(base));
  return r;
}

struct RowLevel {
  int W, n, half, Dm1;
  bool has_valid;
  double maxc;
  const double *vol;
  size_t slab;
};

struct RowTree {
  double p0, p1, p2, p3, p4, p5;
  __device__ __forceinline__ void push(int idx, double R) {
    double t = R;
    if ((idx & 1) == 0) { p0 = t; return; }
    t = p0 + t;
    if ((idx & 2) == 0) { p1 = t; return; }
    t = p1 + t;
    if ((idx & 4) == 0) { p2 = t; return; }
    t = p2 + t;
    if ((idx & 8) == 0) { p3 = t; return; }
    t = p3 + t;
    if ((idx & 16) == 0) { p4 = t; return; }
    t = p4 + t;
    p5 = t;
  }
  __device__ __forceinline__ double total(int count) const {
    double t = 0.0;
    bool have = false;
    if (count & 1) { t = p0; have = true; }
    if (count & 2) { t = have ? p1 + t : p1; have = true; }
    if (count & 4) { t = have ? p2 + t : p2; have = true; }
    if (count & 8) { t = have ? p3 + t : p3; have = true; }
    if (count & 16) { t = have ? p4 + t : p4; have = true; }
    if (count & 32) { t = have ? p5 + t : p5; }
    return t;
  }
};

struct RowSrc {
  int adr_o, adr_g, adr_p;
  int adr_g2, adr_g3;
  const char *own_row, *oth_row;
  int lane_off;
  int img_base, fx_lo, fx_hi;
};

#ifndef CSPM_ROW_SUB
#define CSPM_ROW_SUB 2
#endif
template <int SRC, int VIEW, bool EDGE, bool STAGED, bool ALLV, int J0, int J1>
__device__ __forceinline__ void tap_batch(const RowLevel &A, const Luts &lut, const RowSrc &R, int g0, int adr_o, int adr_g, int adr_g2, int adr_g3, int adr_p, int off_g,
                                          uint32_t Ip, double pa, double Gg, double qxg_d, int e_rel, int e_span, int qy, int cx_lane,
                                          double S[kRowMod]) {
  constexpr int E = elem_size<SRC>();
  constexpr int dirS = VIEW == 0 ? -16 : 16, dirE = VIEW == 0 ? -E : E;
  constexpr int N = J1 - J0;
  const int lutzero = kLutZero;
  uint4 P[N], o0[N], o1[N];
  double fr[N], wgt[N], tmp[N];
  bool valid[N], in_img[N];
  if constexpr (STAGED && CSPM_OWN_SINGLE && (SRC == kSrcGrd || SRC == kSrcImg)) {
#pragma unroll
    for (int k = 0; k < N; ++k) P[k].z = lds_ld<uint32_t>(adr_p + (J0 + k) * 4);
#pragma unroll
    for (int k = 0; k < N; ++k) {
      const u32x2 v = *(volatile __attribute__((address_space(3))) const u32x2 *)(uintptr_t)(unsigned)(adr_g + (J0 + k) * 8);
      P[k].x = v[0]; P[k].y = v[1]; P[k].w = 0u;
    }
  } else {
#pragma unroll
    for (int k = 0; k < N; ++k)
      P[k] = STAGED ? rd_own<SRC>(CSPM_OWN_SINGLE || k == 0 ? adr_g : k == 1 ? adr_g2 : adr_g3, adr_p, J0 + k) : ld_elem<SRC>(R.own_row, off_g + (J0 + k) * E);
  }
#pragma unroll
  for (int k = 0; k < N; ++k) {
    const int j = J0 + k;
    const double q_disp = tap_disp(pa, (double)j, Gg);
    in_img[k] = true;
    if (EDGE) in_img[k] = (unsigned)(e_rel + j) <= (unsigned)e_span;
    if constexpr (SRC == kSrcImg) {
      const ImgSplit g = split_img(q_disp, VIEW == 0 ? -q_disp : q_disp, qxg_d + (double)j, A.Dm1, A.has_valid);
      fr[k] = g.fw;
      valid[k] = ALLV ? true : g.valid;
      const int fxc = min(max(g.fx, R.fx_lo), R.fx_hi);
      if (STAGED) {
        rd_cells<SRC, VIEW>(fxc * 16 + R.img_base, o0[k], o1[k]);
      } else {
        o0[k] = ld_elem<SRC>(R.oth_row, fxc * E + R.img_base);
        o1[k] = ld_elem<SRC>(R.oth_row, fxc * E + R.img_base + E);
      }
      continue;
    }
    const DispSplit d = ALLV ? split_disp_valid(q_disp) : split_disp(q_disp, A.Dm1, A.has_valid);
    fr[k] = d.fr;
    valid[k] = d.valid;
    if (SRC == kSrcVolume) {
      const int qx = in_img[k] ? cx_lane - A.half + g0 + j : cx_lane;
      const double *v = A.vol + (size_t)d.f * A.slab + (size_t)qy * A.W + qx;
      tmp[k] = lerp_cells(d.fr, v[0], v[A.slab]);
    } else if (STAGED) {
      rd_cells<SRC, VIEW>(mad_const<dirS>(d.f, adr_o) + j * 16, o0[k], o1[k]);
    } else {
      const int of = mad_const<dirE>(d.f, off_g);
      o0[k] = ld_elem<SRC>(R.oth_row, of + j * E);
      o1[k] = ld_elem<SRC>(R.oth_row, of + j * E + dirE);
    }
  }
#pragma unroll
  for (int k = 0; k < N; ++k) {
    int sad = (int)__builtin_amdgcn_sad_u8(Ip, pix_of<SRC>(P[k]), 0u);
    if (EDGE) sad = in_img[k] ? sad : lutzero;
    wgt[k] = lut.w[sad];
  }
  if constexpr (SRC == kSrcImg) {
#pragma unroll
    for (int k = 0; k < N; ++k)
      tmp[k] = img_cell(pix_of<SRC>(P[k]), g_of(P[k]), pix_of<SRC>(o0[k]), g_of(o0[k]), pix_of<SRC>(o1[k]), g_of(o1[k]), fr[k]);
  } else if (SRC != kSrcVolume) {
#pragma unroll
    for (int k = 0; k < N; ++k) {
      double c0, c1;
      cell_pair_of<SRC>(lut.a, P[k], o0[k], o1[k], c0, c1);
      tmp[k] = lerp_cells(fr[k], c0, c1);
    }
  }
#pragma unroll
  for (int k = 0; k < N; ++k) {
    const double maxc = A.maxc;
    const double t = (ALLV || valid[k]) ? tmp[k] : maxc;
    S[J0 + k] = __builtin_fma(wgt[k], t, S[J0 + k]);
  }
}

template <int SRC, int VIEW, bool EDGE, bool STAGED, bool ALLV, int CNT>
__device__ __forceinline__ void tap_group(const RowLevel &A, const Luts &lut, const RowSrc &R, int g0, int ga, uint32_t Ip, double pa, double rowterm,
                                          double &qxg_d, int e_rel, int e_span, int qy, int cx_lane, double S[kRowMod]) {
  constexpr int E = elem_size<SRC>();
  constexpr int SUB = CSPM_ROW_SUB;
  const double Gg = group_disp(pa, qxg_d, rowterm);
  const double qxg = qxg_d;
  qxg_d += (double)kRowMod;
  const int adr_o = R.adr_o + ga * 16, adr_g = R.adr_g + ga * (SRC == kSrcCen ? 16 : 8), adr_p = R.adr_p + ga * 4, off_g = R.lane_off + ga * E;
  const int adr_g2 = R.adr_g2 + ga * (SRC == kSrcCen ? 16 : 8), adr_g3 = R.adr_g3 + ga * (SRC == kSrcCen ? 16 : 8);
  tap_batch<SRC, VIEW, EDGE, STAGED, ALLV, 0, (CNT < SUB ? CNT : SUB)>(A, lut, R, g0, adr_o, adr_g, adr_g2, adr_g3, adr_p, off_g, Ip, pa, Gg, qxg, e_rel, e_span, qy,
                                                                  cx_lane, S);
  if constexpr (CNT > SUB)
    tap_batch<SRC, VIEW, EDGE, STAGED, ALLV, SUB, (CNT < 2 * SUB ? CNT : 2 * SUB)>(A, lut, R, g0, adr_o, adr_g, adr_g2, adr_g3, adr_p, off_g, Ip, pa, Gg, qxg, e_rel,
                                                                              e_span, qy, cx_lane, S);
  if constexpr (CNT > 2 * SUB)
    tap_batch<SRC, VIEW, EDGE, STAGED, ALLV, 2 * SUB, CNT>(A, lut, R, g0, adr_o, adr_g, adr_g2, adr_g3, adr_p, off_g, Ip, pa, Gg, qxg, e_rel, e_span, qy, cx_lane, S);
}

template <int SRC, int VIEW, bool EDGE, bool STAGED, bool ALLV = false>
__device__ __forceinline__ double row_taps(const RowLevel &A, const Luts &lut, const RowSrc &R, uint32_t Ip, double pa, double rowterm,
                                           double qx0_d, int e_lo, int e_span, int qy, int cx_lane) {
  double S[kRowMod];
#pragma unroll
  for (int j = 0; j < kRowMod; ++j) S[j] = 0.0;
  double qx_d = qx0_d;
  const int full = A.n / kRowMod * kRowMod;
  int g0 = 0;
  if constexpr (CSPM_ROW_BUMP && STAGED && SRC == kSrcGrd) {
    RowSrc Rg = R;
    for (; g0 < full; g0 += kRowMod) {
      tap_group<SRC, VIEW, EDGE, STAGED, ALLV, kRowMod>(A, lut, Rg, g0, 0, Ip, pa, rowterm, qx_d, g0 - e_lo, e_span, qy, cx_lane, S);
      Rg.adr_o += kRowMod * 16; Rg.adr_g += kRowMod * 8; Rg.adr_p += kRowMod * 4;
      asm("" : "+v"(Rg.adr_o), "+v"(Rg.adr_g), "+v"(Rg.adr_p));
    }
  } else {
    for (; g0 < full; g0 += kRowMod)
      tap_group<SRC, VIEW, EDGE, STAGED, ALLV, kRowMod>(A, lut, R, g0, g0, Ip, pa, rowterm, qx_d, g0 - e_lo, e_span, qy, cx_lane, S);
  }
  switch (A.n - full) {
#define CSPM_TAIL(K) case K: tap_group<SRC, VIEW, EDGE, STAGED, ALLV, K>(A, lut, R, g0, g0, Ip, pa, rowterm, qx_d, g0 - e_lo, e_span, qy, cx_lane, S); break;
    CSPM_TAIL(1) CSPM_TAIL(2) CSPM_TAIL(3) CSPM_TAIL(4) CSPM_TAIL(5) CSPM_TAIL(6)
#undef CSPM_TAIL
    default: break;
  }
  double Rsum = S[0];
#pragma unroll
  for (int j = 1; j < kRowMod; ++j) Rsum = Rsum + S[j];
  return Rsum;
}

struct CellRow {
  int adr_c;
  int stride;
  int adr_w;
  int adr_p;
  uint32_t Ip;
};
template <bool ALLV, bool WTAB, int J0, int J1, int STRIDE = 0>
__device__ __forceinline__ void cell_batch(const RowLevel &A, const Luts &lut, const CellRow &C, int adr_c, int adr_c1, int adr_w, int adr_p, int g8,
                                           double pa, double Gg, double S[kRowMod]) {
  constexpr int N = J1 - J0;
  double c0[N], c1[N], w[N], fr[N];
  bool valid[N];
  uint32_t pq[N];
  if constexpr (!WTAB) {
#pragma unroll
    for (int k = 0; k < N; ++k) pq[k] = lds_ld<uint32_t>(adr_p + (J0 + k) * 4);
  }
#pragma unroll
  for (int k = 0; k < N; ++k) {
    const int j = J0 + k;
    const double q_disp = tap_disp(pa, (double)j, Gg);
    const DispSplit d = ALLV ? split_disp_valid(q_disp) : split_disp(q_disp, A.Dm1, A.has_valid);
    fr[k] = d.fr;
    valid[k] = d.valid;
    int a0;
    asm("v_mad_i32_i24 %0, %1, %2, %3" : "=v"(a0) : "v"(d.f), "s"(C.stride), "v"(adr_c));
    c0[k] = lds_ld<double>(a0 + j * 8);
    if constexpr (STRIDE > 0) {
      c1[k] = lds_ld_single(a0 + STRIDE + j * 8);
    } else {
      int a1;
      asm("v_mad_i32_i24 %0, %1, %2, %3" : "=v"(a1) : "v"(d.f), "s"(C.stride), "v"(adr_c1));
      c1[k] = lds_ld<double>(a1 + j * 8);
    }
    if constexpr (WTAB) w[k] = lds_ld_single(adr_w + j * 8);
  }
  if constexpr (!WTAB) {
#pragma unroll
    for (int k = 0; k < N; ++k) w[k] = lut.w[(int)__builtin_amdgcn_sad_u8(C.Ip, pq[k], 0u)];
  }
#pragma unroll
  for (int k = 0; k < N; ++k) {
    const double tmp = lerp_cells(fr[k], c0[k], c1[k]);
    const double maxc = A.maxc;
    const double t = (ALLV || valid[k]) ? tmp : maxc;
    S[J0 + k] = __builtin_fma(w[k], t, S[J0 + k]);
  }
}
template <bool ALLV, bool WTAB, int CNT, int STRIDE = 0>
__device__ __forceinline__ void cell_group(const RowLevel &A, const Luts &lut, const CellRow &C, int g0, double pa, double rowterm, double &qxg_d,
                                           double S[kRowMod]) {
  const double Gg = group_disp(pa, qxg_d, rowterm);
  qxg_d += (double)kRowMod;
  const int g8 = g0 * 8, adr_c = C.adr_c + g8, adr_c1 = C.adr_c + C.stride + g8, adr_w = C.adr_w + g8, adr_p = C.adr_p + g0 * 4;
  constexpr int SUB = CSPM_CELL_SUB;
  cell_batch<ALLV, WTAB, 0, (CNT < SUB ? CNT : SUB), STRIDE>(A, lut, C, adr_c, adr_c1, adr_w, adr_p, g8, pa, Gg, S);
  if constexpr (CNT > SUB) cell_batch<ALLV, WTAB, SUB, CNT, STRIDE>(A, lut, C, adr_c, adr_c1, adr_w, adr_p, g8, pa, Gg, S);
}
template <bool ALLV, bool WTAB, bool PITCH_IMM = false>
__device__ __forceinline__ double cell_row_taps(const RowLevel &A, const Luts &lut, const CellRow &C, double pa, double rowterm, double qx0_d) {
  double S[kRowMod];
#pragma unroll
  for (int j = 0; j < kRowMod; ++j) S[j] = 0.0;
  double qx_d = qx0_d;
  const int full = A.n / kRowMod * kRowMod;
  int g0 = 0;
  bool done = false;
  if constexpr (PITCH_IMM && CSPM_CELL_PITCH_IMM) {
    done = true;
    switch (C.stride) {
#if CSPM_CELL_BUMP
#define CSPM_PITCH(P)                                                                    \
  case P * 8: {                                                                          \
    CellRow Cg = C;                                                                      \
    for (; g0 < full; g0 += kRowMod) {                                                   \
      cell_group<ALLV, WTAB, kRowMod, P * 8>(A, lut, Cg, 0, pa, rowterm, qx_d, S);       \
      Cg.adr_c += kRowMod * 8;                                                           \
      if constexpr (WTAB) { Cg.adr_w += kRowMod * 8; asm("" : "+v"(Cg.adr_c), "+v"(Cg.adr_w)); } \
      else { Cg.adr_p += kRowMod * 4; asm("" : "+v"(Cg.adr_c), "+v"(Cg.adr_p)); }       \
    }                                                                                    \
  } break;
#else
#define CSPM_PITCH(P) case P * 8: for (; g0 < full; g0 += kRowMod) cell_group<ALLV, WTAB, kRowMod, P * 8>(A, lut, C, g0, pa, rowterm, qx_d, S); break;
#endif
      CSPM_PITCH(128) CSPM_PITCH(100) CSPM_PITCH(80) CSPM_PITCH(68) CSPM_PITCH(52) CSPM_PITCH(44) CSPM_PITCH(40)
#undef CSPM_PITCH
      default: done = false; break;
    }
  }
  if (!done)
    for (; g0 < full; g0 += kRowMod) cell_group<ALLV, WTAB, kRowMod>(A, lut, C, g0, pa, rowterm, qx_d, S);
  switch (A.n - full) {
#define CSPM_TAIL(K) case K: cell_group<ALLV, WTAB, K>(A, lut, C, g0, pa, rowterm, qx_d, S); break;
    CSPM_TAIL(1) CSPM_TAIL(2) CSPM_TAIL(3) CSPM_TAIL(4) CSPM_TAIL(5) CSPM_TAIL(6)
#undef CSPM_TAIL
    default: break;
  }
  double Rsum = S[0];
#pragma unroll
  for (int j = 1; j < kRowMod; ++j) Rsum = Rsum + S[j];
  return Rsum;
}

struct RowCtx {
#ifdef CSPM_ROW_STATS
  int stat_slot;
#endif
#ifdef CSPM_COUNT_ALIVE
  int tag;
#endif
  int y;
  int lane;
  char *strip;
  char *ostrip;
  int cap, ocap;
};
__device__ __forceinline__ RowCtx make_row_ctx(unsigned char *smem, int y, int cap, int ocap) {
  const int wave = __builtin_amdgcn_readfirstlane((int)(threadIdx.x >> 6));
  char *base = reinterpret_cast<char *>(smem + sizeof(LutMem)) + (size_t)wave * (size_t)wave_lds_bytes(cap, ocap);
  return RowCtx{
#ifdef CSPM_ROW_STATS
      0,
#endif
#ifdef CSPM_COUNT_ALIVE
      2,
#endif
      y, (int)(threadIdx.x & 63), base, base + (size_t)cap * 16, cap, ocap};
}

#ifndef CSPM_LEVEL_INLINE
#define CSPM_LEVEL_INLINE __forceinline__
#endif
template <int SRC, int VIEW>
__device__ CSPM_LEVEL_INLINE double level_rows(const Cost &cd, const Luts &lut, const RowCtx &ctx, int s, int cx, int cy, double a, double b,
                                             double c, bool exit_on, double need, bool dead_in) {
  constexpr int E = elem_size<SRC>();
  const int lane = ctx.lane;
#ifdef CSPM_ROW_STATS
  unsigned long long rowtime_acc[4] = {0, 0, 0, 0};
  int rowtime_base = 0;
#endif
  const Level &L = cd.lv[s];
  RowLevel A;
  A.W = L.W; A.n = cd.n; A.half = cd.half; A.Dm1 = L.D - 1;
  A.has_valid = L.D >= 2;
  A.maxc = cd.max_cost[VIEW * CSPM_MAX_LEVELS + s];
  A.vol = L.vol[VIEW];
  A.slab = (size_t)L.W * (size_t)L.H;
  const char *px, *opx;
  if (SRC == kSrcCen) {
    px = reinterpret_cast<const char *>(L.pc[VIEW]); opx = reinterpret_cast<const char *>(L.pc[1 - VIEW]);
  } else {
    px = reinterpret_cast<const char *>(L.px[VIEW]); opx = reinterpret_cast<const char *>(L.px[1 - VIEW]);
  }
  int cmin = wave_min_i32(cx), cmax = wave_max_i32(cx);
  cmin = __builtin_amdgcn_readfirstlane(cmin);
  cmax = __builtin_amdgcn_readfirstlane(cmax);
  const bool edge = (cmin - A.half < 0) | (cmax + A.half >= A.W);
  const int D = L.D;
  const int s_lo = VIEW == 0 ? L.pad + cmin - A.half - D : L.pad + cmin - A.half;
  const int s_hi = VIEW == 0 ? L.pad + cmax + A.half : L.pad + cmax + A.half + D + 1;
  const int s_len = SRC == kSrcVolume ? 0 : s_hi - s_lo + 1;
  const int o_lo = L.pad + cmin - A.half, o_len = cmax - cmin + 2 * A.half + 1;
  const bool staged = s_len <= ctx.cap && o_len <= ctx.ocap;
  RowSrc R;
  const int strip_a = lds_addr(ctx.strip), ostrip_a = lds_addr(ctx.ostrip);
  R.adr_o = strip_a + (L.pad + cx - A.half - s_lo) * 16 - ((VIEW == 0 && SRC != kSrcImg) ? 16 : 0);
  R.adr_g = ostrip_a + (cx - cmin) * (SRC == kSrcCen ? 16 : 8);
  R.adr_p = ostrip_a + ctx.ocap * 8 + (cx - cmin) * 4;
  R.adr_g2 = R.adr_g3 = R.adr_g;
  asm volatile("" : "+v"(R.adr_g2));
  asm volatile("" : "+v"(R.adr_g3));
  R.lane_off = (L.pad + cx - A.half) * E;
  R.img_base = staged ? strip_a + (L.pad - s_lo) * 16 : L.pad * E;
  R.fx_lo = staged ? s_lo - L.pad : -L.pad;
  R.fx_hi = staged ? s_hi - 1 - L.pad : L.W + L.pad - 2;
  const uint32_t Ip = SRC == kSrcCen ? L.pc[VIEW][cy * L.Wp + L.pad + cx].pix : L.px[VIEW][cy * L.Wp + L.pad + cx].pix;
  const double qx0_d = (double)(cx - A.half);
  const int e_lo = max(0, A.half - cx);
  const int e_span = min(A.n - 1, A.W - 1 - cx + A.half) - e_lo;
  RowTree tree;
  const int dy_lo = max(0, A.half - cy), dy_hi = min(A.n - 1, L.H - 1 - cy + A.half);
  for (int dy = 0; dy < dy_lo; ++dy) tree.push(dy, 0.0);
  double partial = 0.0;
  auto all_rejected = [&](double Rsum) -> bool {
#if CSPM_ROW_EXIT
    if (!exit_on) return false;
    partial = partial + Rsum;
    return __builtin_amdgcn_ballot_w64(!(dead_in | (partial >= need))) == 0ull;
#else
    return false;
#endif
  };
  if constexpr (SRC == kSrcGrd) {
    const int ncent = cmax - cmin + 1, NQ = o_len;
    const int lds_room = wave_lds_bytes(ctx.cap, ctx.ocap) - 64;
    const int own_bytes = (NQ * 8 + 15) / 16 * 16 + (NQ * 4 + 15) / 16 * 16, wtab_bytes = ncent * A.n * 8 + ncent * 4;
    const int NQP = ncent >= 48 ? (NQ + 31) / 32 * 32 : ncent >= 24 ? (NQ + 15) / 32 * 32 + 16 : NQ;
    int d_base = 1, ND = D, pitch = NQ;
    bool cells_on = false, wtab = true, allv_level = false, tdma = false;
    int nd_a = 0, b_lo = 0;
    bool lane_b = false;
    int tbuf = 2;
    const int p2 = (NQ * 4 + 15) / 16 * 16;
    if (CSPM_CELL_MODE && staged && D >= 2) {
      const bool full_fits = (NQ + D) * 16 + own_bytes + NQ * D * 8 + wtab_bytes <= lds_room;
      const bool have_cvol = CSPM_TABLE_DMA && L.cvol[VIEW] != nullptr;
      bool range_ok = false;
      int f_lo = 1, f_hi = 1;
      int fl_lane = 1, fh_lane = 1;
      if ((!full_fits || have_cvol) && CSPM_RANGE_MODE && D < 512 && dy_lo <= dy_hi) {
        const int jl = (A.n - 1) % kRowMod;
        const double rt0 = b * (double)(cy - A.half + dy_lo) + c, rt1 = b * (double)(cy - A.half + dy_hi) + c;
        const double q00 = tap_disp(a, 0.0, group_disp(a, qx0_d, rt0)), q01 = tap_disp(a, (double)jl, group_disp(a, qx0_d + (double)(A.n - 1 - jl), rt0));
        const double q10 = tap_disp(a, 0.0, group_disp(a, qx0_d, rt1)), q11 = tap_disp(a, (double)jl, group_disp(a, qx0_d + (double)(A.n - 1 - jl), rt1));
        const double qmin = __builtin_fmin(__builtin_fmin(q00, q01), __builtin_fmin(q10, q11));
        const double qmax = __builtin_fmax(__builtin_fmax(q00, q01), __builtin_fmax(q10, q11));
        const bool safe = (qmin >= 1.0 + 0x1p-20) & (qmax <= (double)D - 0x1p-20);
        f_lo = fl_lane = safe ? (int)(qmin - 0x1p-20) : 1;
        f_hi = fh_lane = safe ? min((int)(qmax + 0x1p-20) + 1, D) : 1;
        f_lo = wave_min_i32(f_lo);
        f_hi = wave_max_i32(f_hi);
        range_ok = __builtin_amdgcn_ballot_w64(!safe) == 0ull;
      }
      const int nd = f_hi - f_lo + 1;
      if (have_cvol) {
        const int NQE = (NQ + 3) & ~3, NQD = NQP > NQE ? NQP : NQE;
        auto span32 = [&](int n_) { return (unsigned long long)n_ * (unsigned long long)L.H * (unsigned long long)L.cvW * 8ull < (1ull << 32); };
        auto fits = [&](int nb, int n_, int pit, bool wt) { return nb * n_ * pit * 8 + 2 * p2 + (wt ? wtab_bytes : 0) <= lds_room && n_ * (pit / 2) <= 12 * kWave && span32(n_); };
        for (int nb = 2; nb >= 1 && !tdma; --nb) {
          if (range_ok) {
            if (!CSPM_PREFER_WTAB && CSPM_CELL_PAD && !edge && ncent <= CSPM_WTAB_MAXC && fits(nb, nd, NQD, false)) { tdma = true; pitch = NQD; wtab = false; }
            else if (!CSPM_PREFER_WTAB && !edge && ncent <= CSPM_WTAB_MAXC && fits(nb, nd, NQE, false)) { tdma = true; pitch = NQE; wtab = false; }
            else if (CSPM_CELL_PAD && fits(nb, nd, NQD, true)) { tdma = true; pitch = NQD; }
            else if (CSPM_CELL_PAD && !edge && fits(nb, nd, NQD, false)) { tdma = true; pitch = NQD; wtab = false; }
            else if (fits(nb, nd, NQE, true)) { tdma = true; pitch = NQE; }
            else if (!edge && fits(nb, nd, NQE, false)) { tdma = true; pitch = NQE; wtab = false; }
            if (tdma) { cells_on = true; d_base = f_lo; ND = nd; allv_level = true; tbuf = nb; }
          }
          if (!tdma && full_fits) {
            if (CSPM_CELL_PAD && fits(nb, D, NQD, true)) { tdma = true; pitch = NQD; }
            else if (fits(nb, D, NQE, true)) { tdma = true; pitch = NQE; }
            if (tdma) { cells_on = true; tbuf = nb; }
          }
          if (!CSPM_TABLE_DMA_SINGLE) break;
        }
        if (CSPM_TABLE_CLUSTERS && !tdma && range_ok && nd > 2) {
          const int cut = (f_lo + f_hi + 1) / 2;
          const bool in_a = fh_lane < cut, in_b = fl_lane >= cut;
          if (__builtin_amdgcn_ballot_w64(!(in_a | in_b)) == 0ull) {
            int a_hi = in_a ? fh_lane : f_lo, bl = in_b ? fl_lane : f_hi;
            a_hi = wave_max_i32(a_hi);
            bl = wave_min_i32(bl);
            const int na = a_hi - f_lo + 1, nb_ = f_hi - bl + 1, nt = na + nb_;
            const bool span_ok = span32(f_hi - f_lo + 1);
            if (nt < nd && span_ok) {
              for (int nb = 2; nb >= 1 && !tdma; --nb) {
                if (CSPM_CELL_PAD && fits(nb, nt, NQD, true)) { tdma = true; pitch = NQD; }
                else if (CSPM_CELL_PAD && !edge && fits(nb, nt, NQD, false)) { tdma = true; pitch = NQD; wtab = false; }
                else if (fits(nb, nt, NQE, true)) { tdma = true; pitch = NQE; }
                else if (!edge && fits(nb, nt, NQE, false)) { tdma = true; pitch = NQE; wtab = false; }
                if (tdma) { cells_on = true; d_base = f_lo; ND = nt; allv_level = true; tbuf = nb; nd_a = na; b_lo = bl; lane_b = in_b; }
                if (!CSPM_TABLE_DMA_SINGLE) break;
              }
            }
          }
        }
      }
      if (!tdma) {
        if (full_fits) {
          cells_on = true;
          if (CSPM_CELL_PAD && (NQ + D) * 16 + own_bytes + NQP * D * 8 + wtab_bytes <= lds_room) pitch = NQP;
        } else if (range_ok && (NQ + nd) <= kStripRegs * kWave) {
          const int strip_bytes = (NQ + nd) * 16 + own_bytes;
          if (CSPM_CELL_PAD && strip_bytes + NQP * nd * 8 + wtab_bytes <= lds_room) { cells_on = true; pitch = NQP; }
          else if (CSPM_CELL_PAD && !edge && strip_bytes + p2 + NQP * nd * 8 <= lds_room) { cells_on = true; wtab = false; pitch = NQP; }
          else if (strip_bytes + NQ * nd * 8 + wtab_bytes <= lds_room) { cells_on = true; }
          else if (!edge && strip_bytes + p2 + NQ * nd * 8 <= lds_room) { cells_on = true; wtab = false; }
          if (cells_on) { d_base = f_lo; ND = nd; allv_level = true; }
        }
      }
#ifdef CSPM_ROW_STATS
      if (range_ok && !cells_on && D <= 128) {
        unsigned m[4] = {0u, 0u, 0u, 0u};
        for (int d = fl_lane; d <= fh_lane; ++d) m[(d >> 5) & 3] |= 1u << (d & 31);
        for (int off = 1; off < kWave; off <<= 1)
          for (int k = 0; k < 4; ++k) m[k] |= (unsigned)__shfl_xor((int)m[k], off, kWave);
        const int un = __popc(m[0]) + __popc(m[1]) + __popc(m[2]) + __popc(m[3]);
        if (lane == 0) atomicAdd(&g_unionstat[s * 8 + (un <= 8 ? 0 : un <= 11 ? 1 : un <= 16 ? 2 : un <= 24 ? 3 : 4)], 1ull);
      }
      if (lane == 0) {
        unsigned long long *g = &g_rangestat[(ctx.stat_slot * 8 + s) * 8];
        if (cells_on && !allv_level) atomicAdd(&g[7], 1ull);
        else {
          atomicAdd(&g[0], 1ull);
          if (!range_ok) atomicAdd(&g[1], 1ull);
          else if (cells_on) { atomicAdd(&g[wtab ? 2 : 3], 1ull); atomicAdd(&g[5], (unsigned long long)nd); }
          else { atomicAdd(&g[4], 1ull); atomicAdd(&g[6], (unsigned long long)nd); }
        }
      }
#endif
    }
    auto build_wtab = [&](int adr_pix, int adr_ipc, int adr_wgt) {
      const int gcol0 = cmin - A.half;
      for (int j0 = 0; j0 < A.n; j0 += kWave) {
        const int j = j0 + lane;
        const bool jon = j < A.n;
        const int js = jon ? j : 0;
        int adr_p = adr_pix + js * 4, adr_o = adr_wgt + js * 8;
        int col = gcol0 + js;
        constexpr int U = 4;
        for (int c0 = 0; c0 < ncent; c0 += U) {
          uint32_t ic[U], pq[U];
#pragma unroll
          for (int u = 0; u < U; ++u) {
            ic[u] = lds_ld<uint32_t>(adr_ipc + (c0 + u) * 4);
            pq[u] = lds_ld<uint32_t>(adr_p + u * 4);
          }
          double w[U];
#pragma unroll
          for (int u = 0; u < U; ++u) {
            int sad = (int)__builtin_amdgcn_sad_u8(ic[u], pq[u], 0u);
            sad = ((unsigned)(col + u) < (unsigned)A.W) ? sad : kLutZero;
            w[u] = lut.w[sad];
          }
          int ao = adr_o;
#pragma unroll
          for (int u = 0; u < U; ++u) {
            if (jon && c0 + u < ncent) *(__attribute__((address_space(3))) double *)(uintptr_t)(unsigned)ao = w[u];
            ao += A.n * 8;
          }
          adr_p += U * 4; adr_o = ao; col += U;
        }
      }
    };
    if (cells_on && tdma) {
      const int tbytes = ND * pitch * 8, ppr = pitch / 2, used = (NQ + 1) / 2, npiece = ND * ppr;
      const int off_p = tbuf * tbytes, off_w = off_p + 2 * p2, off_i = off_w + ncent * A.n * 8;
      const unsigned lds0 = (unsigned)__builtin_amdgcn_readfirstlane(strip_a);
      const unsigned inv = ((1u << 20) + (unsigned)ppr - 1u) / (unsigned)ppr;
      const size_t Wp = (size_t)L.Wp;
      const unsigned rowB = (unsigned)L.cvW * 8u, slabB = (unsigned)L.H * rowB;
      const char *cv = uniform_ptr(reinterpret_cast<const char *>(L.cvol[VIEW]) + (size_t)d_base * slabB + (size_t)(cy - A.half + dy_lo) * rowB +
                                   (size_t)(L.cvpad + cmin - A.half) * 8);
      const char *gp = uniform_ptr(reinterpret_cast<const char *>(L.pix[VIEW]) + ((size_t)(cy - A.half + dy_lo) * Wp + o_lo) * 4);
      const int p_p16 = (NQ * 4 + 15) / 16;
      auto issue_tab = [&](int tb) {
        const unsigned dst = lds0 + (unsigned)(tb * tbytes);
        for (int i = 0; i * kWave < npiece; ++i) {
          const unsigned e = (unsigned)(lane + i * kWave);
          const unsigned k = (e * inv) >> 20, pc = e - k * (unsigned)ppr;
          const unsigned dk = (nd_a > 0 && (int)k >= nd_a) ? k + (unsigned)(b_lo - d_base - nd_a) : k;
          if (e < (unsigned)npiece && pc < (unsigned)used) dma_b128(cv, dk * slabB + pc * 16u, dst + (unsigned)i * 1024u);
        }
        cv += rowB;
      };
      auto issue_pix = [&](int pb) {
        if (lane < p_p16) dma_b128(gp, (unsigned)lane * 16u, lds0 + (unsigned)(off_p + pb * p2));
        gp += Wp * 4;
      };
      dma_wait();
      issue_pix(0);
      issue_tab(0);
      const int ipc_a = strip_a + off_i;
      if (wtab) *(__attribute__((address_space(3))) uint32_t *)(uintptr_t)(unsigned)(ipc_a + (cx - cmin) * 4) = Ip;
      CellRow C;
      C.stride = pitch * 8;
      C.adr_w = strip_a + off_w + (cx - cmin) * A.n * 8;
      C.Ip = Ip;
      const int adr_c0 = strip_a + (cx - cmin) * 8 - (lane_b ? b_lo - nd_a : d_base) * C.stride;
      int par = 0;
      for (int dy = dy_lo; dy <= dy_hi; ++dy) {
        const int qy = cy - A.half + dy;
        [[maybe_unused]] const unsigned long long rt0 = ROWTIME_NOW();
        dma_wait();
        [[maybe_unused]] const unsigned long long rt1 = ROWTIME_NOW();
        if (dy < dy_hi) {
          issue_pix(par ^ 1);
          if (tbuf == 2) issue_tab(par ^ 1);
        }
        C.adr_c = adr_c0 + (tbuf == 2 ? par * tbytes : 0);
        C.adr_p = strip_a + off_p + par * p2 + (cx - cmin) * 4;
        if (wtab) build_wtab(strip_a + off_p + par * p2, ipc_a, strip_a + off_w);
        const double rowterm = b * (double)qy + c;
        double Rsum;
        if (wtab) {
          bool allv = allv_level;
          if (!allv_level) {
            const int jl = (A.n - 1) % kRowMod;
            const double q_first = tap_disp(a, 0.0, group_disp(a, qx0_d, rowterm));
            const double q_last = tap_disp(a, (double)jl, group_disp(a, qx0_d + (double)(A.n - 1 - jl), rowterm));
            const double lo = 1.0 + 0x1p-20, hi = (double)L.D - 0x1p-20;
            const bool safe = (L.D < 512) & (q_first >= lo) & (q_first <= hi) & (q_last >= lo) & (q_last <= hi);
            allv = __builtin_amdgcn_ballot_w64(!safe) == 0ull;
          }
          Rsum = allv ? cell_row_taps<true, true, true>(A, lut, C, a, rowterm, qx0_d) : cell_row_taps<false, true, true>(A, lut, C, a, rowterm, qx0_d);
        } else {
          Rsum = cell_row_taps<true, false, true>(A, lut, C, a, rowterm, qx0_d);
        }
        tree.push(dy, Rsum);
#ifdef CSPM_ROW_STATS
        {
          asm volatile("s_waitcnt lgkmcnt(0)" ::: "memory");
          const unsigned long long rt3 = ROWTIME_NOW();
          ROWTIME_ADD(0, rt3 - rt0); ROWTIME_ADD(1, rt1 - rt0); ROWTIME_ADD(3, 1);
        }
#endif
        if (all_rejected(Rsum)) { dma_wait(); ROWTIME_FLUSH(); return __builtin_inf(); }
        if (tbuf == 1 && dy < dy_hi) {
          asm volatile("s_waitcnt lgkmcnt(0)" ::: "memory");
          issue_tab(0);
        }
        par ^= 1;
      }
      ROWTIME_FLUSH();
      return tree.total(dy_hi + 1);
    }
    if (cells_on) {
      const int c_lo = VIEW == 0 ? L.pad + cmin - A.half - (d_base + ND - 1) : L.pad + cmin - A.half + (d_base - 1);
      const int c_len = NQ + ND;
      const int p_bytes = (NQ * 4 + 15) / 16 * 16;
      const int off_g = c_len * 16, off_p = off_g + (NQ * 8 + 15) / 16 * 16, off_c = off_p + (wtab ? 1 : 2) * p_bytes;
      const int off_w = off_c + pitch * ND * 8, off_i = off_w + ncent * A.n * 8;
      const unsigned lds0 = (unsigned)__builtin_amdgcn_readfirstlane(strip_a);
      const size_t Wp = (size_t)L.Wp;
      const char *g16 = uniform_ptr(reinterpret_cast<const char *>(L.px16[1 - VIEW]) + ((size_t)(cy - A.half + dy_lo) * Wp + c_lo) * 16);
      const char *gg = uniform_ptr(reinterpret_cast<const char *>(L.grd[VIEW]) + ((size_t)(cy - A.half + dy_lo) * Wp + o_lo) * 8);
      const char *gp = uniform_ptr(reinterpret_cast<const char *>(L.pix[VIEW]) + ((size_t)(cy - A.half + dy_lo) * Wp + o_lo) * 4);
      const int g_p16 = (NQ * 8 + 15) / 16, p_p16 = (NQ * 4 + 15) / 16;
      auto issue = [&](int par) {
#pragma unroll
        for (int k = 0; k < kStripRegs; ++k)
          if (k * kWave < c_len) {
            if (lane + k * kWave < c_len) dma_b128(g16, (unsigned)(lane + k * kWave) * 16u, lds0 + (unsigned)k * 1024u);
          }
        if (lane < g_p16) dma_b128(gg, (unsigned)lane * 16u, lds0 + (unsigned)off_g);
        if (lane < p_p16) dma_b128(gp, (unsigned)lane * 16u, lds0 + (unsigned)(off_p + par * p_bytes));
        g16 += Wp * 16; gg += Wp * 8; gp += Wp * 4;
      };
      dma_wait();
      issue(0);
      int par = 0;
      const int ipc_a = strip_a + off_i;
      if (wtab) *(__attribute__((address_space(3))) uint32_t *)(uintptr_t)(unsigned)(ipc_a + (cx - cmin) * 4) = Ip;
      CellRow C;
      C.stride = pitch * 8;
      C.adr_c = strip_a + off_c + (cx - cmin) * 8 - d_base * C.stride;
      C.adr_w = strip_a + off_w + (cx - cmin) * A.n * 8;
      C.Ip = Ip;
      for (int dy = dy_lo; dy <= dy_hi; ++dy) {
        const int qy = cy - A.half + dy;
        [[maybe_unused]] const unsigned long long rt0 = ROWTIME_NOW();
        dma_wait();
        [[maybe_unused]] const unsigned long long rt1 = ROWTIME_NOW();
        for (int q0 = 0; q0 < NQ; q0 += kWave) {
          const int q = q0 + lane;
          const bool qon = q < NQ;
          const int qs = qon ? q : 0;
          const uint2 gq2 = lds_ld<uint2>(strip_a + off_g + qs * 8);
          const uint32_t pq = lds_ld<uint32_t>(strip_a + off_p + par * p_bytes + qs * 4);
          const double gq = __hiloint2double((int)gq2.y, (int)gq2.x);
          int adr_s = strip_a + (VIEW == 0 ? qs + ND - 1 : qs + 1) * 16;
          int adr_t = strip_a + off_c + qs * 8;
          constexpr int U = 4;
          for (int d0 = 0; d0 < ND; d0 += U) {
            uint4 o[U];
#pragma unroll
            for (int u = 0; u < U; ++u) o[u] = lds_ld<uint4>(adr_s + (VIEW == 0 ? -16 : 16) * u);
            double cell[U];
#pragma unroll
            for (int u = 0; u < U; ++u) cell[u] = grd_cell(lut.a, pq, gq, o[u].z, __hiloint2double((int)o[u].y, (int)o[u].x));
            int at = adr_t;
#pragma unroll
            for (int u = 0; u < U; ++u) {
              if (qon && d0 + u < ND) *(__attribute__((address_space(3))) double *)(uintptr_t)(unsigned)at = cell[u];
              at += C.stride;
            }
            adr_s += (VIEW == 0 ? -16 : 16) * U;
            adr_t = at;
          }
        }
        if (wtab) build_wtab(strip_a + off_p, ipc_a, strip_a + off_w);
        const double rowterm = b * (double)qy + c;
        double Rsum;
        dma_wait();
        [[maybe_unused]] const unsigned long long rt2 = ROWTIME_NOW();
        C.adr_p = strip_a + off_p + par * p_bytes + (cx - cmin) * 4;
        if (!wtab) par ^= 1;
        if (dy < dy_hi) issue(par);
        if (wtab) {
          bool allv = allv_level;
          if (!allv_level) {
            const int jl = (A.n - 1) % kRowMod;
            const double q_first = tap_disp(a, 0.0, group_disp(a, qx0_d, rowterm));
            const double q_last = tap_disp(a, (double)jl, group_disp(a, qx0_d + (double)(A.n - 1 - jl), rowterm));
            const double lo = 1.0 + 0x1p-20, hi = (double)L.D - 0x1p-20;
            const bool safe = (L.D < 512) & (q_first >= lo) & (q_first <= hi) & (q_last >= lo) & (q_last <= hi);
            allv = __builtin_amdgcn_ballot_w64(!safe) == 0ull;
          }
          Rsum = allv ? cell_row_taps<true, true>(A, lut, C, a, rowterm, qx0_d) : cell_row_taps<false, true>(A, lut, C, a, rowterm, qx0_d);
        } else {
          Rsum = cell_row_taps<true, false>(A, lut, C, a, rowterm, qx0_d);
        }
        tree.push(dy, Rsum);
#ifdef CSPM_ROW_STATS
        {
          asm volatile("s_waitcnt lgkmcnt(0)" ::: "memory");
          const unsigned long long rt3 = ROWTIME_NOW();
          ROWTIME_ADD(0, rt3 - rt0); ROWTIME_ADD(1, rt1 - rt0); ROWTIME_ADD(2, rt2 - rt1); ROWTIME_ADD(3, 1);
        }
#endif
        if (all_rejected(Rsum)) { dma_wait(); ROWTIME_FLUSH(); return __builtin_inf(); }
      }
      ROWTIME_FLUSH();
      return tree.total(dy_hi + 1);
    }
  }
  if constexpr (SRC == kSrcGrd) {
    if (staged) {
      const int set = strip_set_bytes(ctx.cap, ctx.ocap);
      const unsigned lds0 = (unsigned)__builtin_amdgcn_readfirstlane(strip_a);
      const size_t Wp = (size_t)L.Wp;
      const char *g16 = uniform_ptr(reinterpret_cast<const char *>(L.px16[1 - VIEW]) + ((size_t)(cy - A.half + dy_lo) * Wp + s_lo) * 16);
      const char *gg = uniform_ptr(reinterpret_cast<const char *>(L.grd[VIEW]) + ((size_t)(cy - A.half + dy_lo) * Wp + o_lo) * 8);
      const char *gp = uniform_ptr(reinterpret_cast<const char *>(L.pix[VIEW]) + ((size_t)(cy - A.half + dy_lo) * Wp + o_lo) * 4);
      const int g_p16 = (o_len * 8 + 15) / 16, p_p16 = (o_len * 4 + 15) / 16;
      auto issue = [&](unsigned dst) {
#pragma unroll
        for (int k = 0; k < kStripRegs; ++k)
          if (k * kWave < s_len) {
            if (lane + k * kWave < s_len) dma_b128(g16, (unsigned)(lane + k * kWave) * 16u, dst + (unsigned)k * 1024u);
          }
        if (lane < g_p16) dma_b128(gg, (unsigned)lane * 16u, dst + (unsigned)(ctx.cap * 16));
        if (lane < p_p16) dma_b128(gp, (unsigned)lane * 16u, dst + (unsigned)(ctx.cap * 16 + ctx.ocap * 8));
        g16 += Wp * 16; gg += Wp * 8; gp += Wp * 4;
      };
      dma_wait();
      issue(lds0);
      int par = 0;
      for (int dy = dy_lo; dy <= dy_hi; ++dy) {
        const int qy = cy - A.half + dy;
        [[maybe_unused]] const unsigned long long rt0 = ROWTIME_NOW();
        dma_wait();
        [[maybe_unused]] const unsigned long long rt1 = ROWTIME_NOW();
        if (dy < dy_hi) issue(lds0 + (unsigned)(par ? 0 : set));
        RowSrc Rr = R;
        const int boff = par ? set : 0;
        Rr.adr_o += boff; Rr.adr_g += boff; Rr.adr_g2 += boff; Rr.adr_g3 += boff; Rr.adr_p += boff; Rr.img_base += boff;
        const double rowterm = b * (double)qy + c;
        double Rsum;
        const int jl = (A.n - 1) % kRowMod;
        const double q_first = tap_disp(a, 0.0, group_disp(a, qx0_d, rowterm));
        const double q_last = tap_disp(a, (double)jl, group_disp(a, qx0_d + (double)(A.n - 1 - jl), rowterm));
        const double lo = 1.0 + 0x1p-20, hi = (double)L.D - 0x1p-20;
        const bool safe = (L.D >= 2) & (L.D < 512) & (q_first >= lo) & (q_first <= hi) & (q_last >= lo) & (q_last <= hi);
        const bool allv = __builtin_amdgcn_ballot_w64(!safe) == 0ull;
        if (!edge) {
          Rsum = allv ? row_taps<SRC, VIEW, false, true, true>(A, lut, Rr, Ip, a, rowterm, qx0_d, e_lo, e_span, qy, cx)
                      : row_taps<SRC, VIEW, false, true>(A, lut, Rr, Ip, a, rowterm, qx0_d, e_lo, e_span, qy, cx);
        } else {
          Rsum = (CSPM_EDGE_ALLV && allv) ? row_taps<SRC, VIEW, true, true, true>(A, lut, Rr, Ip, a, rowterm, qx0_d, e_lo, e_span, qy, cx)
                                          : row_taps<SRC, VIEW, true, true>(A, lut, Rr, Ip, a, rowterm, qx0_d, e_lo, e_span, qy, cx);
        }
        tree.push(dy, Rsum);
#ifdef CSPM_ROW_STATS
        {
          asm volatile("s_waitcnt lgkmcnt(0)" ::: "memory");
          const unsigned long long rt3 = ROWTIME_NOW();
          ROWTIME_ADD(4, rt3 - rt0); ROWTIME_ADD(5, rt1 - rt0); ROWTIME_ADD(7, 1);
        }
#endif
        if (all_rejected(Rsum)) { dma_wait(); ROWTIME_FLUSH(); return __builtin_inf(); }
        par ^= 1;
      }
      ROWTIME_FLUSH();
      return tree.total(dy_hi + 1);
    }
  }
  StageReg<SRC> pre[kStripRegs];
  typename StripReg<SRC>::type opre[kOwnRegs];
  const size_t row_stride = (size_t)L.Wp * E;
  R.own_row = px + (size_t)(cy - A.half + dy_lo) * row_stride;
  R.oth_row = opx + (size_t)(cy - A.half + dy_lo) * row_stride;
  const int pre_off = (s_lo + lane) * E, opre_off = (o_lo + lane) * E;
  auto fetch = [&](const char *own_row, const char *oth_row) {
#pragma unroll
    for (int k = 0; k < kStripRegs; ++k)
      if (lane + k * kWave < s_len) pre[k] = ld_stage<SRC, VIEW>(oth_row, pre_off + k * kWave * E);
#pragma unroll
    for (int k = 0; k < kOwnRegs; ++k)
      if (lane + k * kWave < o_len) opre[k] = ld_strip<SRC>(own_row, opre_off + k * kWave * E);
  };
  auto commit = [&]() {
#pragma unroll
    for (int k = 0; k < kStripRegs; ++k)
      if (lane + k * kWave < s_len) *reinterpret_cast<uint4 *>(ctx.strip + (lane + k * kWave) * 16) = pre[k].v;
#pragma unroll
    for (int k = 0; k < kOwnRegs; ++k)
      if (lane + k * kWave < o_len) wr_own<SRC>(ctx.ostrip, ctx.ocap, lane + k * kWave, opre[k]);
  };
  if (staged) {
    fetch(R.own_row, R.oth_row);
    wave_lds_fence();
    commit();
  }
  for (int dy = dy_lo; dy <= dy_hi; ++dy) {
    const int qy = cy - A.half + dy;
    const bool more = dy < dy_hi;
    if (staged) {
      wave_lds_fence();
      if (more) fetch(R.own_row + row_stride, R.oth_row + row_stride);
    }
    const double rowterm = b * (double)qy + c;
    double Rsum;
#ifdef CSPM_ROW_STATS
    {
      const int jl = (A.n - 1) % kRowMod;
      const double q_first = tap_disp(a, 0.0, group_disp(a, qx0_d, rowterm));
      const double q_last = tap_disp(a, (double)jl, group_disp(a, qx0_d + (double)(A.n - 1 - jl), rowterm));
      const double lo = 1.0 + 0x1p-20, hi = (double)L.D - 0x1p-20;
      const bool safe = (L.D >= 2) & (q_first >= lo) & (q_first <= hi) & (q_last >= lo) & (q_last <= hi);
      int f_lo = safe ? (int)fmin(q_first, q_last) : 0, f_hi = safe ? (int)fmax(q_first, q_last) + 1 : 0;
      for (int off = 1; off < kWave; off <<= 1) {
        f_lo = min(f_lo, __shfl_xor(f_lo, off, kWave));
        f_hi = max(f_hi, __shfl_xor(f_hi, off, kWave));
      }
      const int nd = f_hi - f_lo + 1;
      int bucket = nd <= 4 ? 0 : nd <= 8 ? 1 : nd <= 16 ? 2 : nd <= 32 ? 3 : 4;
      if (__builtin_amdgcn_ballot_w64(!safe) != 0ull) bucket = 5;
      if (!staged) bucket = 6;
      if (lane == 0) atomicAdd(&g_rowstat[(ctx.stat_slot * 8 + s) * 8 + bucket], 1ull);
    }
#endif
    if (staged && !edge) {
      const int jl = (A.n - 1) % kRowMod;
      const double q_first = tap_disp(a, 0.0, group_disp(a, qx0_d, rowterm));
      const double q_last = tap_disp(a, (double)jl, group_disp(a, qx0_d + (double)(A.n - 1 - jl), rowterm));
      const double lo = 1.0 + 0x1p-20, hi = (double)L.D - 0x1p-20;
      const bool safe = (L.D >= 2) & (L.D < 512) & (q_first >= lo) & (q_first <= hi) & (q_last >= lo) & (q_last <= hi);
      Rsum = __builtin_amdgcn_ballot_w64(!safe) == 0ull ? row_taps<SRC, VIEW, false, true, true>(A, lut, R, Ip, a, rowterm, qx0_d, e_lo, e_span, qy, cx)
                                                        : row_taps<SRC, VIEW, false, true>(A, lut, R, Ip, a, rowterm, qx0_d, e_lo, e_span, qy, cx);
    } else if (staged) {
      Rsum = row_taps<SRC, VIEW, true, true>(A, lut, R, Ip, a, rowterm, qx0_d, e_lo, e_span, qy, cx);
    } else {
      Rsum = row_taps<SRC, VIEW, true, false>(A, lut, R, Ip, a, rowterm, qx0_d, e_lo, e_span, qy, cx);
    }
    tree.push(dy, Rsum);
    if (all_rejected(Rsum)) return __builtin_inf();
    if (staged && more) {
      wave_lds_fence();
      commit();
    }
    R.own_row += row_stride;
    R.oth_row += row_stride;
  }
// ... 346 lines not shown
```

crossscalepatchmatch_amd/csrc/cspm_tap.h:

```cpp
#pragma once
#include "cspm_device.h"

#pragma clang fp contract(off)

namespace cspm {

constexpr int kRowMod = 7;
constexpr int kChainRows = 9;
constexpr int kMaxWnd = 45;
constexpr int kMaxPasses = (kMaxWnd + kChainRows - 1) / kChainRows;

struct Luts {
  const double *w;
  const double *a;
};

__device__ __forceinline__ void wave_lds_fence() {
  __builtin_amdgcn_fence(__ATOMIC_RELEASE, "wavefront");
  __builtin_amdgcn_wave_barrier();
  __builtin_amdgcn_fence(__ATOMIC_ACQUIRE, "wavefront");
}

typedef uint32_t u32x3 __attribute__((ext_vector_type(3)));
typedef u32x3 u32x3_a4 __attribute__((aligned(4)));
template <int SRC>
__device__ __forceinline__ uint4 ld_elem(const char *base, int byte_off) {
  if (SRC == kSrcCen) return *reinterpret_cast<const uint4 *>(base + (size_t)(unsigned)byte_off);
  const u32x3 v = *reinterpret_cast<const u32x3_a4 *>(base + (size_t)(unsigned)byte_off);
  return uint4{v.x, v.y, v.z, 0u};
}
template <int SRC> constexpr int elem_size() { return SRC == kSrcCen ? 16 : SRC == kSrcGrd8 ? 8 : 12; }
template <int SRC>
__device__ __forceinline__ uint32_t pix_of(const uint4 &v) { return SRC == kSrcCen ? v.w : v.z; }
typedef uint32_t u32x2 __attribute__((ext_vector_type(2)));
typedef uint32_t u32x4 __attribute__((ext_vector_type(4)));
typedef u32x4 u32x4_a8 __attribute__((aligned(8)));
__device__ __forceinline__ uint2 ld_pix8(const char *base, int byte_off) {
  const u32x2 v = *reinterpret_cast<const u32x2 *>(base + (size_t)(unsigned)byte_off);
  return uint2{v.x, v.y};
}
__device__ __forceinline__ uint4 ld_pix8_pair(const char *base, int byte_off) {
  const u32x4 v = *reinterpret_cast<const u32x4_a8 *>(base + (size_t)(unsigned)byte_off);
  return uint4{v.x, v.y, v.z, v.w};
}
__device__ __forceinline__ uint32_t pix8_colour(uint32_t hi) { return hi >> 8; }
__device__ __forceinline__ double pix8_x(uint32_t lo, uint32_t hi) { return __hiloint2double((int)((hi & 0xFu) | 0x43300000u), (int)lo); }
__device__ __forceinline__ double g_of(const uint4 &v) { return __hiloint2double((int)v.y, (int)v.x); }

constexpr unsigned kClrSat = 31;
__device__ __forceinline__ double grd_cell(const double *lut_a, uint32_t Iq, double Gq, uint32_t Io, double Go) {
  const unsigned sad = min(__builtin_amdgcn_sad_u8(Iq, Io, 0u), kClrSat);
  const double grdDiff = __builtin_fmin(fabs(Gq - Go), 2.0);
  return __builtin_fma(1 - 0.1, grdDiff, lut_a[sad]);
}
__device__ __forceinline__ double grd8_cell(const double *lut_a, uint32_t Iq, double Xq, uint32_t Io, double Xo) {
  const unsigned sad = min(__builtin_amdgcn_sad_u8(Iq, Io, 0u), kClrSat);
  const double dX = __builtin_fmin(fabs(Xq - Xo), 268435456.0);
  return __builtin_fma((1 - 0.1) * 0x1p-27, dX, lut_a[sad]);
}
__device__ __forceinline__ double cen_cell(const uint4 &q, const uint4 &o) {
  const int eighty = 80;
  const int ham = __popc(q.x ^ o.x) + __popc(q.y ^ o.y) + __popc(q.z ^ o.z);
  const int cnt = ((int)o.w < 0) ? eighty : ham;
  return (double)cnt;
}
template <int SRC>
__device__ __forceinline__ double cell_of(const double *lut_a, const uint4 &own, const uint4 &other) {
  if (SRC == kSrcCen) return cen_cell(own, other);
  return grd_cell(lut_a, pix_of<SRC>(own), g_of(own), pix_of<SRC>(other), g_of(other));
}

typedef __attribute__((address_space(3))) const char lds_cchar;
__device__ __forceinline__ int lds_addr(const void *p) { return (int)(uintptr_t)(lds_cchar *)p; }
template <class T> struct LdsVec { typedef T type; };
template <> struct LdsVec<uint2> { typedef u32x2 type; };
template <> struct LdsVec<uint4> { typedef u32x4 type; };
template <class T>
__device__ __forceinline__ T lds_ld(int adr) {
  typedef typename LdsVec<T>::type V;
  const V v = *(__attribute__((address_space(3))) const V *)(uintptr_t)(unsigned)adr;
  if constexpr (sizeof(T) == 16) return T{v[0], v[1], v[2], v[3]};
  else if constexpr (__is_floating_point(T)) return v;
  else if constexpr (sizeof(T) == 8) return T{v[0], v[1]};
  else return v;
}
#ifndef CSPM_PAIR_SAD
#define CSPM_PAIR_SAD 1
#endif
typedef unsigned short u16x2_t __attribute__((ext_vector_type(2)));
template <int SRC>
__device__ __forceinline__ void cell_pair_of(const double *lut_a, const uint4 &own, const uint4 &o0, const uint4 &o1, double &c0, double &c1) {
  if constexpr (SRC == kSrcCen || !CSPM_PAIR_SAD) {
    c0 = cell_of<SRC>(lut_a, own, o0);
    c1 = cell_of<SRC>(lut_a, own, o1);
  } else {
    const uint32_t Iq = pix_of<SRC>(own);
    const double Gq = g_of(own);
    uint32_t t = __builtin_amdgcn_sad_u8(Iq, pix_of<SRC>(o0), 0u);
    t = __builtin_amdgcn_sad_hi_u8(Iq, pix_of<SRC>(o1), t);
    const u16x2_t lim = {(unsigned short)kClrSat, (unsigned short)kClrSat};
    t = __builtin_bit_cast(uint32_t, __builtin_elementwise_min(__builtin_bit_cast(u16x2_t, t), lim));
    const int base = lds_addr(lut_a);
    int adr0;
    asm("v_mad_u32_u16 %0, %1, 8, %2" : "=v"(adr0) : "v"(t), "s"(base));
    int adr1;
    asm("v_mad_u32_u16 %0, %1, 8, %2 op_sel:[1,0,0,0]" : "=v"(adr1) : "v"(t), "s"(base));
    const double a0 = lds_ld<double>(adr0), a1 = lds_ld<double>(adr1);
    c0 = __builtin_fma(1 - 0.1, __builtin_fmin(fabs(Gq - g_of(o0)), 2.0), a0);
    c1 = __builtin_fma(1 - 0.1, __builtin_fmin(fabs(Gq - g_of(o1)), 2.0), a1);
  }
}
__device__ __forceinline__ int cvt_i32_sat(double x) {
  int r;
  asm("v_cvt_i32_f64 %0, %1" : "=v"(r) : "v"(x));
  return r;
}
__device__ __forceinline__ int med3_i32(int x, int lo, int hi) {
  int r;
  asm("v_med3_i32 %0, %1, %2, %3" : "=v"(r) : "v"(x), "v"(lo), "v"(hi));
  return r;
}

struct DispSplit {
  bool valid;
  int f;
  double fr;
};
__device__ __forceinline__ DispSplit split_disp(double q_disp, int Dm1, bool level_has_valid) {
  DispSplit s;
  const int f0 = cvt_i32_sat(q_disp);
  s.f = med3_i32(f0, 1, Dm1);
  s.valid = (s.f == f0) & level_has_valid;
  s.fr = __builtin_amdgcn_fract(q_disp);
  return s;
}
__device__ __forceinline__ DispSplit split_disp_valid(double q_disp) {
  DispSplit s;
  s.f = cvt_i32_sat(q_disp);
  s.valid = true;
  s.fr = __builtin_amdgcn_fract(q_disp);
  return s;
}
__device__ __forceinline__ double lerp_cells(double fr, double c0, double c1) { return __builtin_fma(fr, c1 - c0, c0); }
__device__ __forceinline__ double tap_value(const DispSplit &s, double c0, double c1, double maxc) {
  const double tmp = lerp_cells(s.fr, c0, c1);
  return s.valid ? tmp : maxc;
}
__device__ __forceinline__ double group_disp(double a, double qx_group, double q_disp_y) { return __builtin_fma(a, qx_group, q_disp_y); }
__device__ __forceinline__ double tap_disp(double a, double j, double G) { return __builtin_fma(a, j, G); }

struct ImgSplit {
  bool valid;
  int fx;
  double fw;
};
__device__ __forceinline__ ImgSplit split_img(double q_disp, double signed_disp, double qx_d, int Dm1, bool level_has_valid) {
  ImgSplit s;
  const int f0 = cvt_i32_sat(q_disp);
  s.valid = (med3_i32(f0, 1, Dm1) == f0) & level_has_valid;
  const double other_x = qx_d + signed_disp;
  s.fx = cvt_i32_sat(other_x);
  s.fw = (double)(int)((unsigned)s.fx + 1u) - other_x;
  return s;
}
__device__ __forceinline__ double img_cell(uint32_t Iq, double Gq, uint32_t If, double Gf, uint32_t Ic, double Gc, double fw) {
  double t[3];
#pragma unroll
  for (int k = 0; k < 3; ++k) {
    const int q = (int)((Iq >> (8 * k)) & 255u), c = (int)((Ic >> (8 * k)) & 255u), f = (int)((If >> (8 * k)) & 255u);
    t[k] = fabs((double)(q - c) + fw * (double)(c - f));
  }
  double clr = t[0] + t[1];
  clr = clr + t[2];
  clr *= 0.33333333333333;
  const double grd = fabs((Gq - Gc) + fw * (Gc - Gf));
  return 0.1 * __builtin_fmin(clr, 10.0) + (1 - 0.1) * __builtin_fmin(grd, 2.0);
}

__device__ __forceinline__ void require_full_exec() {
#ifdef CSPM_DEBUG_EXEC
  if (__builtin_amdgcn_read_exec() != ~0ull) __builtin_trap();
#endif
}
template <int CTRL>
__device__ __forceinline__ double dpp_f64(double v) {
  int lo = __double2loint(v), hi = __double2hiint(v);
  lo = __builtin_amdgcn_update_dpp(lo, lo, CTRL, 0xF, 0xF, false);
  hi = __builtin_amdgcn_update_dpp(hi, hi, CTRL, 0xF, 0xF, false);
  return __hiloint2double(hi, lo);
}
__device__ __forceinline__ double readlane_f64(double v, int l) {
  return __hiloint2double(__builtin_amdgcn_readlane(__double2hiint(v), l), __builtin_amdgcn_readlane(__double2loint(v), l));
}
__device__ __forceinline__ double wave_tree_sum(double v) {
  require_full_exec();
  v = v + dpp_f64<0xB1>(v);
  v = v + dpp_f64<0x4E>(v);
  v = v + dpp_f64<0x141>(v);
  v = v + dpp_f64<0x140>(v);
  const double r0 = readlane_f64(v, 0), r1 = readlane_f64(v, 16), r2 = readlane_f64(v, 32), r3 = readlane_f64(v, 48);
  const double a = r0 + r1, b = r2 + r3;
  return a + b;
}

template <int CTRL>
__device__ __forceinline__ int dpp_i32(int v) { return __builtin_amdgcn_update_dpp(v, v, CTRL, 0xF, 0xF, false); }
__device__ __forceinline__ int wave_min_i32(int v) {
  require_full_exec();
  v = min(v, dpp_i32<0xB1>(v));
  v = min(v, dpp_i32<0x4E>(v));
  v = min(v, dpp_i32<0x141>(v));
  v = min(v, dpp_i32<0x140>(v));
  return __builtin_amdgcn_readfirstlane(min(min(__builtin_amdgcn_readlane(v, 0), __builtin_amdgcn_readlane(v, 16)), min(__builtin_amdgcn_readlane(v, 32), __builtin_amdgcn_readlane(v, 48))));
}
__device__ __forceinline__ int wave_max_i32(int v) {
  require_full_exec();
  v = max(v, dpp_i32<0xB1>(v));
  v = max(v, dpp_i32<0x4E>(v));
  v = max(v, dpp_i32<0x141>(v));
  v = max(v, dpp_i32<0x140>(v));
  return __builtin_amdgcn_readfirstlane(max(max(__builtin_amdgcn_readlane(v, 0), __builtin_amdgcn_readlane(v, 16)), max(__builtin_amdgcn_readlane(v, 32), __builtin_amdgcn_readlane(v, 48))));
}

struct LutMem {
  double w[kLutSize];
  double a[kClrSat + 1];
};
__device__ __forceinline__ Luts load_luts(const Cost &cd, LutMem &m) {
  for (int i = threadIdx.x; i < kLutSize; i += blockDim.x) m.w[i] = i == kLutZero ? 0.0 : cd.lut[i];
  if (threadIdx.x <= kClrSat) m.a[threadIdx.x] = cd.lut_a[threadIdx.x];
  __syncthreads();
  return Luts{m.w, m.a};
}

__device__ __forceinline__ long long xcd_block() {
  const long long per = (long long)gridDim.x / 8;
  return (long long)(blockIdx.x % 8) * per + blockIdx.x / 8;
}

__device__ __forceinline__ void store_plane(const Field &f, long long i, double nx, double ny, double nz, double a, double b,
                                            double c, double cost) {
  f.nx[i] = nx; f.ny[i] = ny; f.nz[i] = nz;
  f.a[i] = a; f.b[i] = b; f.c[i] = c;
  f.cost[i] = cost;
}

struct Cand { double nx, ny, nz, a, b, c; };

}
```

include/cspm.h:

```cpp
#ifndef CSPM_H
#define CSPM_H

#include <stddef.h>
#include <stdint.h>

#ifdef __cplusplus
extern "C" {
#endif

#define CSPM_OK 0
#define CSPM_ERR_ARG (-1)
#define CSPM_ERR_HIP (-2)
#define CSPM_ERR_STATE (-3)

#define CSPM_MAX_LEVELS 8

typedef struct cspm_ctx cspm_ctx;

#define CSPM_SCHED_RASTER 0
#define CSPM_SCHED_REDBLACK 1

#define CSPM_RNG_PER_PIXEL 0
#define CSPM_RNG_ROW_SHARED 1

typedef struct cspm_pm_params {
  uint64_t seed;
  int schedule;
  int rb_rounds;
  int rb_neighbours;
  int rng_mode;
  int early_exit;
} cspm_pm_params;

int cspm_device_count(void);
int cspm_create(cspm_ctx **out, int device);
void cspm_destroy(cspm_ctx *ctx);
const char *cspm_last_error(const cspm_ctx *ctx);
int cspm_set_stream(cspm_ctx *ctx, void *hip_stream);
int cspm_get_stream(cspm_ctx *ctx, void **hip_stream_out);
int cspm_synchronize(cspm_ctx *ctx);

int cspm_set_images(cspm_ctx *ctx, const uint8_t *l_bgr, const uint8_t *r_bgr, int w, int h, size_t stride);
int cspm_set_images_device(cspm_ctx *ctx, const void *d_l_bgr, const void *d_r_bgr, int w, int h, size_t stride);

int cspm_build_cost_grd(cspm_ctx *ctx, int max_dis, int wnd_size, int scale_num, double reg_lambda);
#define CSPM_OPT_GRD_VOLUMES 1
#define CSPM_OPT_RASTER_LAUNCHES 2
#define CSPM_OPT_SWEEP_TIMEOUT_MS 3
#define CSPM_OPT_SWEEP_FALLBACKS 4
#define CSPM_OPT_SWEEP_PAIRS 5
#define CSPM_OPT_SWEEP_PAIRS_ACTIVE 6
#define CSPM_OPT_TABLE_VOLUMES 7
#define CSPM_OPT_TABLE_VOLUMES_ACTIVE 8
#define CSPM_OPT_VOLUME_FALLBACKS 9
#define CSPM_OPT_SWEEP_FLOW 13
#define CSPM_OPT_SWEEP_WG 14
#define CSPM_OPT_VOLUME_RETRY_PAIRS 15
#define CSPM_OPT_VIEW_SORT 17
#define CSPM_OPT_SWEEP_FOLD 18
#define CSPM_OPT_FAULT_VOLUME_ALLOC 16
#define CSPM_OPT_SWEEP_PACKED 10
#define CSPM_OPT_SWEEP_PACKED_ACTIVE 11
#define CSPM_OPT_SWEEP_PACKED_BAD 12
int cspm_get_option(cspm_ctx *ctx, int key, long long *value);
int cspm_set_option(cspm_ctx *ctx, int key, long long value);
int cspm_build_cost_cen(cspm_ctx *ctx, int max_dis, int wnd_size, int scale_num, double reg_lambda);
int cspm_build_cost_img(cspm_ctx *ctx, int max_dis, int wnd_size, int scale_num, double reg_lambda);
int cspm_begin_cost(cspm_ctx *ctx, int max_dis, int wnd_size, int scale_num, double reg_lambda);
int cspm_upload_cost_slab(cspm_ctx *ctx, int view, int level, int d, const double *slab, size_t stride_elems);
int cspm_finish_cost(cspm_ctx *ctx);
int cspm_get_levels(const cspm_ctx *ctx);
int cspm_get_level_dims(const cspm_ctx *ctx, int level, int *w, int *h, int *max_disp);
int cspm_get_level_image(cspm_ctx *ctx, int view, int level, uint8_t *bgr_out);
int cspm_get_cost_slab(cspm_ctx *ctx, int view, int level, int d, double *slab_out);
int cspm_get_max_cost(cspm_ctx *ctx, int view, int level, double *out);
int cspm_get_scale_weights(const cspm_ctx *ctx, double *out );

int cspm_grd_build_cv_host(int device, const double *l_rgb, const double *r_rgb, int w, int h, int maxDis,
                           int right_view, double *vol_out);

int cspm_cen_build_cv_host(int device, const double *l_rgb, const double *r_rgb, int w, int h, int maxDis,
                           int right_view, double *vol_out);

int cspm_plane_cost_batch(cspm_ctx *ctx, int view, int n, const int *xy, const double *norm_param, double *cost_out);

int cspm_pm_default_params(cspm_pm_params *p);
int cspm_patchmatch(cspm_ctx *ctx, int iter_num, const cspm_pm_params *p);
int cspm_pm_init(cspm_ctx *ctx, const cspm_pm_params *p);
int cspm_pm_spatial(cspm_ctx *ctx, int iter, const cspm_pm_params *p);
int cspm_pm_view(cspm_ctx *ctx, int iter, const cspm_pm_params *p);
int cspm_pm_refine(cspm_ctx *ctx, int iter, const cspm_pm_params *p);
int cspm_get_planes(cspm_ctx *ctx, int view, double *norm_param_out, double *min_cost_out);
int cspm_set_planes(cspm_ctx *ctx, int view, const double *norm_param, const double *min_cost);
int cspm_rescore_planes(cspm_ctx *ctx);
int cspm_patchmatch_warm(cspm_ctx *ctx, int iter_num, const cspm_pm_params *p);
int cspm_upsample_planes(cspm_ctx *dst, cspm_ctx *src);
int cspm_get_disparity_u8(cspm_ctx *ctx, int view, int dis_scale, uint8_t *out, size_t stride);
int cspm_get_disparity_f64(cspm_ctx *ctx, int view, double *out);
int cspm_disparity_u8_device(cspm_ctx *ctx, int view, int dis_scale, void *d_out);
int cspm_postprocess(cspm_ctx *ctx, int dis_scale, uint8_t *l_out, uint8_t *r_out, size_t stride);
int cspm_postprocess_device(cspm_ctx *ctx, int dis_scale, void *d_l_out, void *d_r_out);

#define CSPM_FPM_INIT 0
#define CSPM_FPM_SPATIAL 1
#define CSPM_FPM_VIEW 2
#define CSPM_FPM_REFINE 3
int cspm_fpm_begin(cspm_ctx *ctx, int w, int h, int max_dis);
int cspm_fpm_candidates(cspm_ctx *ctx, int phase, int iter, int step, const cspm_pm_params *p, int *n_out, int *xy_out, int *view_out,
                        double *plane_out);
int cspm_fpm_commit(cspm_ctx *ctx, const double *cost);

#define CSPM_CA_BOX 0
#define CSPM_CA_GF 1
#define CSPM_CA_BF 2
int cspm_aggregate_cv_host(int device, int method, const double *guide, int w, int h, int n_slices, double *vol);
int cspm_local_stereo(cspm_ctx *ctx, int method);

#define CSPM_K_GRD 0
#define CSPM_K_INIT 1
#define CSPM_K_SPATIAL 2
#define CSPM_K_VIEW 3
#define CSPM_K_REFINE 4
#define CSPM_K_MISC 5
#define CSPM_K_POST 6
#define CSPM_K_COUNT 7
int cspm_enable_timing(cspm_ctx *ctx, int on);
int cspm_reset_timing(cspm_ctx *ctx);
int cspm_get_timing(cspm_ctx *ctx, int kclass, long long *launches, double *total_ms, long long *evals);
long long cspm_taps_per_view_pass(const cspm_ctx *ctx);
long long cspm_row_engine_taps_per_view_pass(const cspm_ctx *ctx);

#ifdef __cplusplus
}
#endif
#endif
```

Measured before the change: 3.362 Mpix/s.

## Qualify more row passes for range-limited cost tables via abstain and clamped ranges

Widens which row-engine passes can use the compact disparity-range cost table. Dead lanes may abstain by taking a neutral plane, and partially out-of-range planes are admitted with per-lane clamping of the disparity index through a new split_disp_in. Per-row validity checks are now also applied on the non-wtab path. The intent is to avoid the general full-D fallback staging more often. The cost is extra wave reductions, extra per-row checks and new clamping logic, plus optional atomic counters.

```diff
diff --git a/crossscalepatchmatch_amd/capi.py b/crossscalepatchmatch_amd/capi.py
--- a/crossscalepatchmatch_amd/capi.py
+++ b/crossscalepatchmatch_amd/capi.py
@@ -30,6 +30,13 @@
 OPT_VIEW_SORT = 17
 OPT_SWEEP_FOLD = 18
 OPT_FAULT_VOLUME_ALLOC = 16
+OPT_TABLE_QUALIFY = 19
+OPT_QUALIFY_COUNTS = 20
+OPT_QUALIFY_PASSES = 21
+OPT_QUALIFY_RANGE = 22
+OPT_QUALIFY_CLAMPED = 23
+OPT_QUALIFY_ABSTAINED = 24
+OPT_QUALIFY_GENERAL = 25
 CA_BOX, CA_GF, CA_BF = 0, 1, 2
 
 SYMBOLS = [
diff --git a/crossscalepatchmatch_amd/csrc/cspm_api.hip b/crossscalepatchmatch_amd/csrc/cspm_api.hip
--- a/crossscalepatchmatch_amd/csrc/cspm_api.hip
+++ b/crossscalepatchmatch_amd/csrc/cspm_api.hip
@@ -97,6 +97,9 @@
   Field f[2]{};
   ViewCand vc{nullptr, nullptr, nullptr, nullptr};
   long long opt_sweep_fold = 0;
+  long long opt_table_qualify = 3;
+  unsigned long long *d_qcount = nullptr;
+  bool qcount_on = false;
   long long opt_view_sort = 1;
   uint8_t *d_dis[2] = {nullptr, nullptr};
   uint8_t *d_valid[2] = {nullptr, nullptr};
@@ -232,6 +235,13 @@
 inline int row_cap(const cspm_ctx *c) { return strip_capacity(c->max_dis, c->cost.half); }
 inline int row_ocap(const cspm_ctx *c) { return own_capacity(c->cost.half); }
 inline size_t row_shmem(const cspm_ctx *c) { return sizeof(LutMem) + (size_t)kRowWaves * wave_lds_bytes(row_cap(c), row_ocap(c)); }
+
+inline Cost row_cost(const cspm_ctx *c) {
+  Cost cd = c->cost;
+  cd.qualify = (int)c->opt_table_qualify;
+  cd.qcount = c->qcount_on ? c->d_qcount : nullptr;
+  return cd;
+}
 
 inline RowQueue next_row_queue(cspm_ctx *c, int views) {
   if (!row_claimed(c, views)) return RowQueue{nullptr};
@@ -778,7 +788,7 @@
   {
     Timed t(c, CSPM_K_INIT, items);
     const RowQueue rq = next_row_queue(c, 2);
-    LAUNCH_CS(k_init, dim3(row_grid(c, 2)), dim3(kRowBlock), row_shmem(c), c->cost, pm, rq, row_cap(c), row_ocap(c));
+    LAUNCH_CS(k_init, dim3(row_grid(c, 2)), dim3(kRowBlock), row_shmem(c), row_cost(c), pm, rq, row_cap(c), row_ocap(c));
   }
   HIPCHK(c, hipGetLastError());
   c->field_consistent = true;
@@ -882,7 +892,7 @@
     {
       Timed t(c, CSPM_K_VIEW, items);
       const RowQueue rq = next_row_queue(c, 1);
-      LAUNCH_CS(k_view_eval, dim3(row_grid(c, 1)), dim3(kRowBlock), row_shmem(c), c->cost, pm, rq, v, vc, row_cap(c), row_ocap(c));
+      LAUNCH_CS(k_view_eval, dim3(row_grid(c, 1)), dim3(kRowBlock), row_shmem(c), row_cost(c), pm, rq, v, vc, row_cap(c), row_ocap(c));
     }
     {
       Timed t(c, CSPM_K_MISC, 0);
@@ -904,7 +914,7 @@
     const int cnt = std::min(c->refine_chunk, steps - first);
     Timed t(c, CSPM_K_REFINE, items * cnt);
     const RowQueue rq = next_row_queue(c, 2);
-    LAUNCH_CS(k_refine, dim3(row_grid(c, 2)), dim3(kRowBlock), row_shmem(c), c->cost, pm, rq, iter, first, cnt, z, nn, row_cap(c), row_ocap(c));
+    LAUNCH_CS(k_refine, dim3(row_grid(c, 2)), dim3(kRowBlock), row_shmem(c), row_cost(c), pm, rq, iter, first, cnt, z, nn, row_cap(c), row_ocap(c));
     for (int k = 0; k < cnt; ++k) { z /= 2.0; nn /= 2.0; }
   }
   HIPCHK(c, hipGetLastError());
@@ -933,7 +943,7 @@
   {
     Timed t(c, CSPM_K_INIT, items);
     const RowQueue rq = next_row_queue(c, 2);
-    LAUNCH_CS(k_rescore, dim3(row_grid(c, 2)), dim3(kRowBlock), row_shmem(c), c->cost, pm, rq, row_cap(c), row_ocap(c));
+    LAUNCH_CS(k_rescore, dim3(row_grid(c, 2)), dim3(kRowBlock), row_shmem(c), row_cost(c), pm, rq, row_cap(c), row_ocap(c));
   }
   HIPCHK(c, hipGetLastError());
   c->field_consistent = true;
@@ -1174,6 +1184,7 @@
   if (const char *e = getenv("CSPM_TABLE_VOLUMES_MAX_MB")) c->table_volumes_limit = std::max(0LL, atoll(e)) << 20;
   if (const char *e = getenv("CSPM_SWEEP_PACKED")) c->opt_sweep_packed = atoi(e) ? 1 : 0;
   if (const char *e = getenv("CSPM_SWEEP_FLOW")) c->opt_sweep_flow = atoi(e) ? 1 : 0;
+  if (const char *e = getenv("CSPM_TABLE_QUALIFY")) c->opt_table_qualify = atoi(e) & 3;
   if (const char *e = getenv("CSPM_VIEW_SORT")) c->opt_view_sort = atoi(e) ? 1 : 0;
   if (const char *e = getenv("CSPM_SWEEP_FOLD")) c->opt_sweep_fold = atoi(e) ? 1 : 0;
   if (const char *e = getenv("CSPM_VOLUMES_MEM_FRACTION")) c->volumes_mem_fraction = std::min(1.0, std::max(0.0, atof(e)));
@@ -1198,6 +1209,7 @@
   free_field(c);
   free_images(c);
   for (void *p : c->ca_allocs) (void)hipFree(p);
+  if (c->d_qcount) (void)hipFree(c->d_qcount);
   if (c->own_stream) (void)hipStreamDestroy(c->own_stream);
   delete c;
 }
@@ -1292,6 +1304,21 @@
     case CSPM_OPT_SWEEP_FLOW: c->opt_sweep_flow = value ? 1 : 0; return CSPM_OK;
     case CSPM_OPT_SWEEP_WG: c->sweep_wg_per_cu = value < 0 ? 0 : (value > 16 ? 16 : (int)value); return CSPM_OK;
     case CSPM_OPT_VIEW_SORT: c->opt_view_sort = value ? 1 : 0; return CSPM_OK;
+    case CSPM_OPT_TABLE_QUALIFY:
+      if (value < 0 || value > 3) return fail(c, CSPM_ERR_ARG, "table qualification: 0 .. 3");
+      c->opt_table_qualify = value;
+      return CSPM_OK;
+    case CSPM_OPT_QUALIFY_COUNTS: {
+      DevGuard guard_(c->device);
+      if (!guard_.ok) return fail(c, CSPM_ERR_HIP, "hipSetDevice failed");
+      if (value && !c->d_qcount) {
+        int rc = dalloc(c, &c->d_qcount, 8, nullptr);
+        if (rc) return rc;
+      }
+      if (value) HIPCHK(c, hipMemsetAsync(c->d_qcount, 0, 8 * sizeof(unsigned long long), c->stream));
+      c->qcount_on = value != 0;
+      return CSPM_OK;
+    }
     case CSPM_OPT_SWEEP_FOLD: c->opt_sweep_fold = value ? 1 : 0; return CSPM_OK;
     case CSPM_OPT_FAULT_VOLUME_ALLOC: c->fault_volume_alloc = value < 0 ? 0 : (int)value; return CSPM_OK;
     case CSPM_OPT_VOLUME_RETRY_PAIRS: c->volume_retry_pairs = value < 0 ? 0 : value; return CSPM_OK;
@@ -1317,6 +1344,21 @@
     case CSPM_OPT_VOLUME_FALLBACKS: *value = c->optional_volume_fallbacks; return CSPM_OK;
     case CSPM_OPT_VOLUME_RETRY_PAIRS: *value = c->volume_retry_pairs; return CSPM_OK;
     case CSPM_OPT_VIEW_SORT: *value = c->opt_view_sort; return CSPM_OK;
+    case CSPM_OPT_TABLE_QUALIFY: *value = c->opt_table_qualify; return CSPM_OK;
+    case CSPM_OPT_QUALIFY_PASSES:
+    case CSPM_OPT_QUALIFY_RANGE:
+    case CSPM_OPT_QUALIFY_CLAMPED:
+    case CSPM_OPT_QUALIFY_ABSTAINED:
+    case CSPM_OPT_QUALIFY_GENERAL: {
+      *value = 0;
+      if (!c->d_qcount) return CSPM_OK;
+      DevGuard guard_(c->device);
+      unsigned long long n[8];
+      HIPCHK(c, hipMemcpyAsync(n, c->d_qcount, sizeof n, hipMemcpyDeviceToHost, c->stream));
+      HIPCHK(c, hipStreamSynchronize(c->stream));
+      *value = (long long)n[key - CSPM_OPT_QUALIFY_PASSES];
+      return CSPM_OK;
+    }
     case CSPM_OPT_SWEEP_FOLD: *value = c->opt_sweep_fold; return CSPM_OK;
     case CSPM_OPT_SWEEP_PACKED: *value = c->opt_sweep_packed; return CSPM_OK;
     case CSPM_OPT_SWEEP_FLOW: *value = c->opt_sweep_flow; return CSPM_OK;
@@ -2132,6 +2174,12 @@
   if (reset && hipMemcpyToSymbol(HIP_SYMBOL(cspm::g_rangestat), z, sizeof z) != hipSuccess) return CSPM_ERR_HIP;
   return CSPM_OK;
 }
+int cspm_debug_qualstats(unsigned long long *out1024, int reset) {
+  static unsigned long long z[16 * 8 * 8];
+  if (hipMemcpyFromSymbol(out1024, HIP_SYMBOL(cspm::g_qualstat), sizeof z) != hipSuccess) return CSPM_ERR_HIP;
+  if (reset && hipMemcpyToSymbol(HIP_SYMBOL(cspm::g_qualstat), z, sizeof z) != hipSuccess) return CSPM_ERR_HIP;
+  return CSPM_OK;
+}
 int cspm_debug_rowstats(unsigned long long *out1024, int reset) {
   static unsigned long long z[16 * 8 * 8];
   if (hipMemcpyFromSymbol(out1024, HIP_SYMBOL(cspm::g_rowstat), sizeof z) != hipSuccess) return CSPM_ERR_HIP;
diff --git a/crossscalepatchmatch_amd/csrc/cspm_device.h b/crossscalepatchmatch_amd/csrc/cspm_device.h
--- a/crossscalepatchmatch_amd/csrc/cspm_device.h
+++ b/crossscalepatchmatch_amd/csrc/cspm_device.h
@@ -76,6 +76,8 @@
   const double *lut;
   const double *lut_a;
   const double *max_cost;
+  int qualify;
+  unsigned long long *qcount;
   Level lv[CSPM_MAX_LEVELS];
 };
 
diff --git a/crossscalepatchmatch_amd/csrc/cspm_rows.h b/crossscalepatchmatch_amd/csrc/cspm_rows.h
--- a/crossscalepatchmatch_amd/csrc/cspm_rows.h
+++ b/crossscalepatchmatch_amd/csrc/cspm_rows.h
@@ -60,15 +60,24 @@
 #ifndef CSPM_RANGE_MODE
 #define CSPM_RANGE_MODE 1
 #endif
+#ifndef CSPM_TABLE_QUALIFY
+#define CSPM_TABLE_QUALIFY 3
+#endif
 #ifndef CSPM_CELL_MODE
 #define CSPM_CELL_MODE 1
 #endif
 constexpr int kRowBlock = kRowWaves * kWave;
+#ifdef CSPM_ROW_STATS
+constexpr bool kRowStats = true;
+#else
+constexpr bool kRowStats = false;
+#endif
 #ifdef CSPM_ROW_STATS
 __device__ unsigned long long g_rowstat[16 * 8 * 8];
 __device__ unsigned long long g_rangestat[16 * 8 * 8];
 __device__ unsigned long long g_rowtime[8 * 8];
 __device__ unsigned long long g_unionstat[8 * 8];
+__device__ unsigned long long g_qualstat[16 * 8 * 8];
 #define ROWTIME_NOW() __builtin_readcyclecounter()
 #define ROWTIME_ADD(slot, v) do { rowtime_acc[(slot) & 3] += (unsigned long long)(v); rowtime_base = (slot) & 4; } while (0)
 #define ROWTIME_FLUSH() do { if (lane == 0 && rowtime_acc[3]) for (int k_ = 0; k_ < 4; ++k_) atomicAdd(&g_rowtime[s * 8 + rowtime_base + k_], rowtime_acc[k_]); } while (0)
@@ -368,6 +377,7 @@
   int adr_w;
   int adr_p;
   uint32_t Ip;
+  int f_min;
 };
 template <bool ALLV, bool WTAB, int J0, int J1, int STRIDE = 0>
 __device__ __forceinline__ void cell_batch(const RowLevel &A, const Luts &lut, const CellRow &C, int adr_c, int adr_c1, int adr_w, int adr_p, int g8,
@@ -384,7 +394,7 @@
   for (int k = 0; k < N; ++k) {
     const int j = J0 + k;
     const double q_disp = tap_disp(pa, (double)j, Gg);
-    const DispSplit d = ALLV ? split_disp_valid(q_disp) : split_disp(q_disp, A.Dm1, A.has_valid);
+    const DispSplit d = ALLV ? split_disp_valid(q_disp) : split_disp_in(q_disp, C.f_min, A.Dm1, true);
     fr[k] = d.fr;
     valid[k] = d.valid;
     int a0;
@@ -527,6 +537,9 @@
   const int s_len = SRC == kSrcVolume ? 0 : s_hi - s_lo + 1;
   const int o_lo = L.pad + cmin - A.half, o_len = cmax - cmin + 2 * A.half + 1;
   const bool staged = s_len <= ctx.cap && o_len <= ctx.ocap;
+  const int qual = CSPM_TABLE_QUALIFY & cd.qualify;
+  const bool abstain = (qual & 1) && dead_in && D >= 2;
+  if (abstain && !(SRC == kSrcGrd && CSPM_CELL_MODE && staged && D >= 2)) { a = 0.0; b = 0.0; c = 1.5; }
   RowSrc R;
   const int strip_a = lds_addr(ctx.strip), ostrip_a = lds_addr(ctx.ostrip);
   R.adr_o = strip_a + (L.pad + cx - A.half - s_lo) * 16 - ((VIEW == 0 && SRC != kSrcImg) ? 16 : 0);
@@ -566,82 +579,158 @@
     int nd_a = 0, b_lo = 0;
     bool lane_b = false;
     int tbuf = 2;
+    int f_min = 1, f_max = A.Dm1;
     const int p2 = (NQ * 4 + 15) / 16 * 16;
     if (CSPM_CELL_MODE && staged && D >= 2) {
       const bool full_fits = (NQ + D) * 16 + own_bytes + NQ * D * 8 + wtab_bytes <= lds_room;
       const bool have_cvol = CSPM_TABLE_DMA && L.cvol[VIEW] != nullptr;
-      bool range_ok = false;
-      int f_lo = 1, f_hi = 1;
-      int fl_lane = 1, fh_lane = 1;
-      if ((!full_fits || have_cvol) && CSPM_RANGE_MODE && D < 512 && dy_lo <= dy_hi) {
+      const bool range_test = (!full_fits || have_cvol) && CSPM_RANGE_MODE && D < 512 && dy_lo <= dy_hi;
+      bool safe = false, part_ok = false, all_inv = false;
+      int sl = 1, sh = 1;
+      if (range_test) {
         const int jl = (A.n - 1) % kRowMod;
         const double rt0 = b * (double)(cy - A.half + dy_lo) + c, rt1 = b * (double)(cy - A.half + dy_hi) + c;
         const double q00 = tap_disp(a, 0.0, group_disp(a, qx0_d, rt0)), q01 = tap_disp(a, (double)jl, group_disp(a, qx0_d + (double)(A.n - 1 - jl), rt0));
         const double q10 = tap_disp(a, 0.0, group_disp(a, qx0_d, rt1)), q11 = tap_disp(a, (double)jl, group_disp(a, qx0_d + (double)(A.n - 1 - jl), rt1));
         const double qmin = __builtin_fmin(__builtin_fmin(q00, q01), __builtin_fmin(q10, q11));
         const double qmax = __builtin_fmax(__builtin_fmax(q00, q01), __builtin_fmax(q10, q11));
-        const bool safe = (qmin >= 1.0 + 0x1p-20) & (qmax <= (double)D - 0x1p-20);
-        f_lo = fl_lane = safe ? (int)(qmin - 0x1p-20) : 1;
-        f_hi = fh_lane = safe ? min((int)(qmax + 0x1p-20) + 1, D) : 1;
-        f_lo = wave_min_i32(f_lo);
-        f_hi = wave_max_i32(f_hi);
-        range_ok = __builtin_amdgcn_ballot_w64(!safe) == 0ull;
+        safe = (qmin >= 1.0 + 0x1p-20) & (qmax <= (double)D - 0x1p-20);
+        sl = max(1, cvt_i32_sat(qmin - 0x1p-20));
+        sh = min(cvt_i32_sat(qmax + 0x1p-20) + 1, D);
+        if ((qual & 2) || kRowStats) {
+          const double mag = __builtin_fmax(__builtin_fmax(fabs(a) * (fabs(qx0_d) + (double)A.n), fabs(b) * (double)(abs(cy) + A.n)), fabs(c));
+          part_ok = !safe & (mag < 0x1p20);
+          all_inv = part_ok & ((qmax + 0x1p-20 < 1.0) | (qmin - 0x1p-20 >= (double)D));
+        }
       }
-      const int nd = f_hi - f_lo + 1;
-      if (have_cvol) {
-        const int NQE = (NQ + 3) & ~3, NQD = NQP > NQE ? NQP : NQE;
-        auto span32 = [&](int n_) { return (unsigned long long)n_ * (unsigned long long)L.H * (unsigned long long)L.cvW * 8ull < (1ull << 32); };
-        auto fits = [&](int nb, int n_, int pit, bool wt) { return nb * n_ * pit * 8 + 2 * p2 + (wt ? wtab_bytes : 0) <= lds_room && n_ * (pit / 2) <= 12 * kWave && span32(n_); };
-        for (int nb = 2; nb >= 1 && !tdma; --nb) {
-          if (range_ok) {
-            if (!CSPM_PREFER_WTAB && CSPM_CELL_PAD && !edge && ncent <= CSPM_WTAB_MAXC && fits(nb, nd, NQD, false)) { tdma = true; pitch = NQD; wtab = false; }
-            else if (!CSPM_PREFER_WTAB && !edge && ncent <= CSPM_WTAB_MAXC && fits(nb, nd, NQE, false)) { tdma = true; pitch = NQE; wtab = false; }
-            else if (CSPM_CELL_PAD && fits(nb, nd, NQD, true)) { tdma = true; pitch = NQD; }
-            else if (CSPM_CELL_PAD && !edge && fits(nb, nd, NQD, false)) { tdma = true; pitch = NQD; wtab = false; }
-            else if (fits(nb, nd, NQE, true)) { tdma = true; pitch = NQE; }
-            else if (!edge && fits(nb, nd, NQE, false)) { tdma = true; pitch = NQE; wtab = false; }
-            if (tdma) { cells_on = true; d_base = f_lo; ND = nd; allv_level = true; tbuf = nb; }
+      struct QIn {
+        bool ok;
+        int f_lo, f_hi;
+        int fl, fh;
+        bool neutral;
+        bool tol;
+      };
+      auto qualify = [&](int q) -> QIn {
+        QIn r;
+        const bool ab = (q & 1) && dead_in;
+        const bool adm = (q & 2) && part_ok;
+        const bool adds = !ab & (safe | (adm & !all_inv));
+        int lo = adds ? sl : 0x7fffffff, hi = adds ? sh : (int)0x80000000;
+        r.f_lo = wave_min_i32(lo);
+        r.f_hi = wave_max_i32(hi);
+        r.ok = __builtin_amdgcn_ballot_w64(!(ab | safe | adm)) == 0ull && r.f_lo <= r.f_hi;
+        if (!r.ok) r.f_lo = r.f_hi = 1;
+        r.neutral = !adds;
+        r.fl = adds ? lo : r.f_lo;
+        r.fh = adds ? hi : r.f_lo + 1;
+        r.tol = __builtin_amdgcn_ballot_w64(!ab & adm) != 0ull;
+        return r;
+      };
+      struct Sel {
+        int d_base, ND, pitch;
+        bool cells_on, wtab, allv_level, tdma, range;
+        int nd_a, b_lo;
+        bool lane_b;
+        int tbuf;
+      };
+      auto select = [&](const QIn &in) -> Sel {
+        Sel r{1, D, NQ, false, true, false, false, false, 0, 0, false, 2};
+        const int nd = in.f_hi - in.f_lo + 1;
+        if (have_cvol) {
+          const int NQE = (NQ + 3) & ~3, NQD = NQP > NQE ? NQP : NQE;
+          auto span32 = [&](int n_) { return (unsigned long long)n_ * (unsigned long long)L.H * (unsigned long long)L.cvW * 8ull < (1ull << 32); };
+          auto fits = [&](int nb, int n_, int pit, bool wt) { return nb * n_ * pit * 8 + 2 * p2 + (wt ? wtab_bytes : 0) <= lds_room && n_ * (pit / 2) <= 12 * kWave && span32(n_); };
+          for (int nb = 2; nb >= 1 && !r.tdma; --nb) {
+            if (in.ok) {
+              if (!CSPM_PREFER_WTAB && CSPM_CELL_PAD && !edge && ncent <= CSPM_WTAB_MAXC && fits(nb, nd, NQD, false)) { r.tdma = true; r.pitch = NQD; r.wtab = false; }
+              else if (!CSPM_PREFER_WTAB && !edge && ncent <= CSPM_WTAB_MAXC && fits(nb, nd, NQE, false)) { r.tdma = true; r.pitch = NQE; r.wtab = false; }
+              else if (CSPM_CELL_PAD && fits(nb, nd, NQD, true)) { r.tdma = true; r.pitch = NQD; }
+              else if (CSPM_CELL_PAD && !edge && fits(nb, nd, NQD, false)) { r.tdma = true; r.pitch = NQD; r.wtab = false; }
+              else if (fits(nb, nd, NQE, true)) { r.tdma = true; r.pitch = NQE; }
+              else if (!edge && fits(nb, nd, NQE, false)) { r.tdma = true; r.pitch = NQE; r.wtab = false; }
+              if (r.tdma) { r.cells_on = true; r.range = true; r.d_base = in.f_lo; r.ND = nd; r.allv_level = !in.tol; r.tbuf = nb; }
+            }
+            if (!r.tdma && full_fits) {
+              if (CSPM_CELL_PAD && fits(nb, D, NQD, true)) { r.tdma = true; r.pitch = NQD; }
+              else if (fits(nb, D, NQE, true)) { r.tdma = true; r.pitch = NQE; }
+              if (r.tdma) { r.cells_on = true; r.tbuf = nb; }
+            }
+            if (!CSPM_TABLE_DMA_SINGLE) break;
           }
-          if (!tdma && full_fits) {
-            if (CSPM_CELL_PAD && fits(nb, D, NQD, true)) { tdma = true; pitch = NQD; }
-            else if (fits(nb, D, NQE, true)) { tdma = true; pitch = NQE; }
-            if (tdma) { cells_on = true; tbuf = nb; }
-          }
-          if (!CSPM_TABLE_DMA_SINGLE) break;
-        }
-        if (CSPM_TABLE_CLUSTERS && !tdma && range_ok && nd > 2) {
-          const int cut = (f_lo + f_hi + 1) / 2;
-          const bool in_a = fh_lane < cut, in_b = fl_lane >= cut;
-          if (__builtin_amdgcn_ballot_w64(!(in_a | in_b)) == 0ull) {
-            int a_hi = in_a ? fh_lane : f_lo, bl = in_b ? fl_lane : f_hi;
-            a_hi = wave_max_i32(a_hi);
-            bl = wave_min_i32(bl);
-            const int na = a_hi - f_lo + 1, nb_ = f_hi - bl + 1, nt = na + nb_;
-            const bool span_ok = span32(f_hi - f_lo + 1);
-            if (nt < nd && span_ok) {
-              for (int nb = 2; nb >= 1 && !tdma; --nb) {
-                if (CSPM_CELL_PAD && fits(nb, nt, NQD, true)) { tdma = true; pitch = NQD; }
-                else if (CSPM_CELL_PAD && !edge && fits(nb, nt, NQD, false)) { tdma = true; pitch = NQD; wtab = false; }
-                else if (fits(nb, nt, NQE, true)) { tdma = true; pitch = NQE; }
-                else if (!edge && fits(nb, nt, NQE, false)) { tdma = true; pitch = NQE; wtab = false; }
-                if (tdma) { cells_on = true; d_base = f_lo; ND = nt; allv_level = true; tbuf = nb; nd_a = na; b_lo = bl; lane_b = in_b; }
-                if (!CSPM_TABLE_DMA_SINGLE) break;
+          if (CSPM_TABLE_CLUSTERS && !r.tdma && in.ok && !in.tol && nd > 2) {
+            const int cut = (in.f_lo + in.f_hi + 1) / 2;
+            const bool in_a = in.neutral | (in.fh < cut), in_b = !in.neutral & (in.fl >= cut);
+            if (__builtin_amdgcn_ballot_w64(!(in_a | in_b)) == 0ull) {
+              int a_hi = (in_a & !in.neutral) ? in.fh : in.f_lo, bl = in_b ? in.fl : in.f_hi;
+              a_hi = wave_max_i32(a_hi);
+              bl = wave_min_i32(bl);
+              const int na = a_hi - in.f_lo + 1, nb_ = in.f_hi - bl + 1, nt = na + nb_;
+              const bool span_ok = span32(in.f_hi - in.f_lo + 1);
+              if (nt < nd && span_ok && na >= 2) {
+                for (int nb = 2; nb >= 1 && !r.tdma; --nb) {
+                  if (CSPM_CELL_PAD && fits(nb, nt, NQD, true)) { r.tdma = true; r.pitch = NQD; }
+                  else if (CSPM_CELL_PAD && !edge && fits(nb, nt, NQD, false)) { r.tdma = true; r.pitch = NQD; r.wtab = false; }
+                  else if (fits(nb, nt, NQE, true)) { r.tdma = true; r.pitch = NQE; }
+                  else if (!edge && fits(nb, nt, NQE, false)) { r.tdma = true; r.pitch = NQE; r.wtab = false; }
+                  if (r.tdma) { r.cells_on = true; r.range = true; r.d_base = in.f_lo; r.ND = nt; r.allv_level = !in.tol; r.tbuf = nb; r.nd_a = na; r.b_lo = bl; r.lane_b = in_b; }
+                  if (!CSPM_TABLE_DMA_SINGLE) break;
+                }
               }
             }
           }
         }
+        if (!r.tdma) {
+          if (full_fits) {
+            r.cells_on = true;
+            if (CSPM_CELL_PAD && (NQ + D) * 16 + own_bytes + NQP * D * 8 + wtab_bytes <= lds_room) r.pitch = NQP;
+          } else if (in.ok && (NQ + nd) <= kStripRegs * kWave) {
+            const int strip_bytes = (NQ + nd) * 16 + own_bytes;
+            if (CSPM_CELL_PAD && strip_bytes + NQP * nd * 8 + wtab_bytes <= lds_room) { r.cells_on = true; r.pitch = NQP; }
+            else if (CSPM_CELL_PAD && !edge && strip_bytes + p2 + NQP * nd * 8 <= lds_room) { r.cells_on = true; r.wtab = false; r.pitch = NQP; }
+            else if (strip_bytes + NQ * nd * 8 + wtab_bytes <= lds_room) { r.cells_on = true; }
+            else if (!edge && strip_bytes + p2 + NQ * nd * 8 <= lds_room) { r.cells_on = true; r.wtab = false; }
+            if (r.cells_on) { r.range = true; r.d_base = in.f_lo; r.ND = nd; r.allv_level = !in.tol; }
+          }
+        }
+        return r;
+      };
+      const QIn in = range_test ? qualify(qual) : QIn{false, 1, 1, 1, 1, false, false};
+      const bool mattered = range_test && __builtin_amdgcn_ballot_w64(abstain & (!safe | (sl < in.f_lo) | (sh > in.f_hi))) != 0ull;
+      const Sel sel = select(in);
+#ifdef CSPM_ROW_STATS
+      if (range_test) {
+        const Sel s0 = qual == 0 ? sel : select(qualify(0));
+        bool m1 = false, m2 = false, m3 = false;
+        if (!s0.cells_on) { m1 = select(qualify(1)).range; m2 = select(qualify(2)).range; m3 = select(qualify(3)).range; }
+        if (lane == 0) {
+          unsigned long long *g = &g_qualstat[(ctx.stat_slot * 8 + s) * 8];
+          atomicAdd(&g[0], 1ull);
+          if (!s0.cells_on) { atomicAdd(&g[1], 1ull); atomicAdd(&g[7], (unsigned long long)(dy_hi - dy_lo + 1)); }
+          if (m1) atomicAdd(&g[2], 1ull);
+          if (m2) atomicAdd(&g[3], 1ull);
+          if (m3) atomicAdd(&g[4], 1ull);
+          if (sel.range) atomicAdd(&g[5], 1ull);
+          if (sel.range && !sel.allv_level) atomicAdd(&g[6], 1ull);
+        }
       }
-      if (!tdma) {
-        if (full_fits) {
-          cells_on = true;
-          if (CSPM_CELL_PAD && (NQ + D) * 16 + own_bytes + NQP * D * 8 + wtab_bytes <= lds_room) pitch = NQP;
-        } else if (range_ok && (NQ + nd) <= kStripRegs * kWave) {
-          const int strip_bytes = (NQ + nd) * 16 + own_bytes;
-          if (CSPM_CELL_PAD && strip_bytes + NQP * nd * 8 + wtab_bytes <= lds_room) { cells_on = true; pitch = NQP; }
-          else if (CSPM_CELL_PAD && !edge && strip_bytes + p2 + NQP * nd * 8 <= lds_room) { cells_on = true; wtab = false; pitch = NQP; }
-          else if (strip_bytes + NQ * nd * 8 + wtab_bytes <= lds_room) { cells_on = true; }
-          else if (!edge && strip_bytes + p2 + NQ * nd * 8 <= lds_room) { cells_on = true; wtab = false; }
-          if (cells_on) { d_base = f_lo; ND = nd; allv_level = true; }
+#endif
+      [[maybe_unused]] const bool range_ok = in.ok;
+      [[maybe_unused]] const int nd = in.f_hi - in.f_lo + 1;
+      [[maybe_unused]] const int fl_lane = in.fl, fh_lane = in.fh;
+      d_base = sel.d_base; ND = sel.ND; pitch = sel.pitch;
+      cells_on = sel.cells_on; wtab = sel.wtab; allv_level = sel.allv_level; tdma = sel.tdma;
+      nd_a = sel.nd_a; b_lo = sel.b_lo; lane_b = sel.lane_b; tbuf = sel.tbuf;
+      if (sel.range) {
+        f_min = d_base; f_max = d_base + ND - 2;
+      }
+      if (abstain) { a = 0.0; b = 0.0; c = sel.range ? (double)d_base + 0.5 : 1.5; }
+      if (cd.qcount) {
+        if (lane == 0) {
+          atomicAdd(&cd.qcount[0], 1ull);
+          if (sel.range) atomicAdd(&cd.qcount[1], 1ull);
+          if (sel.range && !sel.allv_level) atomicAdd(&cd.qcount[2], 1ull);
+          if (sel.range && mattered) atomicAdd(&cd.qcount[3], 1ull);
+          if (!sel.cells_on) atomicAdd(&cd.qcount[4], 1ull);
         }
       }
 #ifdef CSPM_ROW_STATS
@@ -655,7 +744,7 @@
       }
       if (lane == 0) {
         unsigned long long *g = &g_rangestat[(ctx.stat_slot * 8 + s) * 8];
-        if (cells_on && !allv_level) atomicAdd(&g[7], 1ull);
+        if (cells_on && !sel.range) atomicAdd(&g[7], 1ull);
         else {
           atomicAdd(&g[0], 1ull);
           if (!range_ok) atomicAdd(&g[1], 1ull);
@@ -732,6 +821,8 @@
       C.stride = pitch * 8;
       C.adr_w = strip_a + off_w + (cx - cmin) * A.n * 8;
       C.Ip = Ip;
+      C.f_min = f_min;
+      A.Dm1 = f_max;
       const int adr_c0 = strip_a + (cx - cmin) * 8 - (lane_b ? b_lo - nd_a : d_base) * C.stride;
       int par = 0;
       for (int dy = dy_lo; dy <= dy_hi; ++dy) {
@@ -748,19 +839,19 @@
         if (wtab) build_wtab(strip_a + off_p + par * p2, ipc_a, strip_a + off_w);
         const double rowterm = b * (double)qy + c;
         double Rsum;
+        bool allv = allv_level;
+        if (!allv_level) {
+          const int jl = (A.n - 1) % kRowMod;
+          const double q_first = tap_disp(a, 0.0, group_disp(a, qx0_d, rowterm));
+          const double q_last = tap_disp(a, (double)jl, group_disp(a, qx0_d + (double)(A.n - 1 - jl), rowterm));
+          const double lo = 1.0 + 0x1p-20, hi = (double)L.D - 0x1p-20;
+          const bool safe = (L.D < 512) & (q_first >= lo) & (q_first <= hi) & (q_last >= lo) & (q_last <= hi);
+          allv = __builtin_amdgcn_ballot_w64(!safe) == 0ull;
+        }
         if (wtab) {
-          bool allv = allv_level;
-          if (!allv_level) {
-            const int jl = (A.n - 1) % kRowMod;
-            const double q_first = tap_disp(a, 0.0, group_disp(a, qx0_d, rowterm));
-            const double q_last = tap_disp(a, (double)jl, group_disp(a, qx0_d + (double)(A.n - 1 - jl), rowterm));
-            const double lo = 1.0 + 0x1p-20, hi = (double)L.D - 0x1p-20;
-            const bool safe = (L.D < 512) & (q_first >= lo) & (q_first <= hi) & (q_last >= lo) & (q_last <= hi);
-            allv = __builtin_amdgcn_ballot_w64(!safe) == 0ull;
-          }
           Rsum = allv ? cell_row_taps<true, true, true>(A, lut, C, a, rowterm, qx0_d) : cell_row_taps<false, true, true>(A, lut, C, a, rowterm, qx0_d);
         } else {
-          Rsum = cell_row_taps<true, false, true>(A, lut, C, a, rowterm, qx0_d);
+          Rsum = allv ? cell_row_taps<true, false, true>(A, lut, C, a, rowterm, qx0_d) : cell_row_taps<false, false, true>(A, lut, C, a, rowterm, qx0_d);
         }
         tree.push(dy, Rsum);
 #ifdef CSPM_ROW_STATS
@@ -812,6 +903,8 @@
       C.adr_c = strip_a + off_c + (cx - cmin) * 8 - d_base * C.stride;
       C.adr_w = strip_a + off_w + (cx - cmin) * A.n * 8;
       C.Ip = Ip;
+      C.f_min = f_min;
+      A.Dm1 = f_max;
       for (int dy = dy_lo; dy <= dy_hi; ++dy) {
         const int qy = cy - A.half + dy;
         [[maybe_unused]] const unsigned long long rt0 = ROWTIME_NOW();
@@ -852,19 +945,19 @@
         C.adr_p = strip_a + off_p + par * p_bytes + (cx - cmin) * 4;
         if (!wtab) par ^= 1;
         if (dy < dy_hi) issue(par);
+        bool allv = allv_level;
+        if (!allv_level) {
+          const int jl = (A.n - 1) % kRowMod;
+          const double q_first = tap_disp(a, 0.0, group_disp(a, qx0_d, rowterm));
+          const double q_last = tap_disp(a, (double)jl, group_disp(a, qx0_d + (double)(A.n - 1 - jl), rowterm));
+          const double lo = 1.0 + 0x1p-20, hi = (double)L.D - 0x1p-20;
+          const bool safe = (L.D < 512) & (q_first >= lo) & (q_first <= hi) & (q_last >= lo) & (q_last <= hi);
+          allv = __builtin_amdgcn_ballot_w64(!safe) == 0ull;
+        }
         if (wtab) {
-          bool allv = allv_level;
-          if (!allv_level) {
-            const int jl = (A.n - 1) % kRowMod;
-            const double q_first = tap_disp(a, 0.0, group_disp(a, qx0_d, rowterm));
-            const double q_last = tap_disp(a, (double)jl, group_disp(a, qx0_d + (double)(A.n - 1 - jl), rowterm));
-            const double lo = 1.0 + 0x1p-20, hi = (double)L.D - 0x1p-20;
-            const bool safe = (L.D < 512) & (q_first >= lo) & (q_first <= hi) & (q_last >= lo) & (q_last <= hi);
-            allv = __builtin_amdgcn_ballot_w64(!safe) == 0ull;
-          }
           Rsum = allv ? cell_row_taps<true, true>(A, lut, C, a, rowterm, qx0_d) : cell_row_taps<false, true>(A, lut, C, a, rowterm, qx0_d);
         } else {
-          Rsum = cell_row_taps<true, false>(A, lut, C, a, rowterm, qx0_d);
+          Rsum = allv ? cell_row_taps<true, false>(A, lut, C, a, rowterm, qx0_d) : cell_row_taps<false, false>(A, lut, C, a, rowterm, qx0_d);
         }
         tree.push(dy, Rsum);
 #ifdef CSPM_ROW_STATS
diff --git a/crossscalepatchmatch_amd/csrc/cspm_tap.h b/crossscalepatchmatch_amd/csrc/cspm_tap.h
--- a/crossscalepatchmatch_amd/csrc/cspm_tap.h
+++ b/crossscalepatchmatch_amd/csrc/cspm_tap.h
@@ -134,6 +134,14 @@
   s.fr = __builtin_amdgcn_fract(q_disp);
   return s;
 }
+__device__ __forceinline__ DispSplit split_disp_in(double q_disp, int lo, int hi, bool level_has_valid) {
+  DispSplit s;
+  const int f0 = cvt_i32_sat(q_disp);
+  s.f = med3_i32(f0, lo, hi);
+  s.valid = (s.f == f0) & level_has_valid;
+  s.fr = __builtin_amdgcn_fract(q_disp);
+  return s;
+}
 __device__ __forceinline__ DispSplit split_disp_valid(double q_disp) {
   DispSplit s;
   s.f = cvt_i32_sat(q_disp);
diff --git a/include/cspm.h b/include/cspm.h
--- a/include/cspm.h
+++ b/include/cspm.h
@@ -58,6 +58,13 @@
 #define CSPM_OPT_VOLUME_RETRY_PAIRS 15
 #define CSPM_OPT_VIEW_SORT 17
 #define CSPM_OPT_SWEEP_FOLD 18
+#define CSPM_OPT_TABLE_QUALIFY 19
+#define CSPM_OPT_QUALIFY_COUNTS 20
+#define CSPM_OPT_QUALIFY_PASSES 21
+#define CSPM_OPT_QUALIFY_RANGE 22
+#define CSPM_OPT_QUALIFY_CLAMPED 23
+#define CSPM_OPT_QUALIFY_ABSTAINED 24
+#define CSPM_OPT_QUALIFY_GENERAL 25
 #define CSPM_OPT_FAULT_VOLUME_ALLOC 16
 #define CSPM_OPT_SWEEP_PACKED 10
 #define CSPM_OPT_SWEEP_PACKED_ACTIVE 11
```

Result: no change. 3.373 Mpix/s (median of 6 runs) (+0.3%).
